# MiniMax-AI/VTP

Measured on AMD Instinct MI355X. Metric: images/sec/node VTP-B f16d64 256x256 train step, higher is better.
Workload: dtype bf16

## Files before the change

include/vtp_hip.h:

```cpp
#ifndef VTP_HIP_H
#define VTP_HIP_H
#ifdef __cplusplus
extern "C" {
#endif

#define VTP_ABI_VERSION 1

int vtp_abi_version(void);
const char* vtp_last_error(void);

enum { VTP_EPI_BF16 = 0, VTP_EPI_F32 = 1, VTP_EPI_SWIGLU = 2, VTP_EPI_GELU = 3, VTP_EPI_F32_ATOMIC = 4, VTP_EPI_F32_SLAB = 5,
       VTP_EPI_QUICK_GELU = 8 };
int vtp_gemm_splits(int K, int splits);
int vtp_gemm_tn_splits(int M, int N, int K);
int vtp_gemm_tn(const void* A, int lda, const void* B, int ldb, void* C, int ldc, int ldc2, const float* resid, int M, int N,
                int K, int epilogue, int a_grp, int a_pre, int b_grp, int b_pre, int c_grp, int c_pre, int splits,
                float* a_colsum, void* stream);
int vtp_gemm_tn_grouped(const void* probs, int nprob, int ntiles, int K, int splits, void* part, void* ticket, void* stream);
int vtp_gemm_tn_grouped_items(const void* probs, int nprob, int ntiles, int K, const void* items, int nitems, int slots, void* part,
                              void* ticket, void* stream);
int vtp_set_gemm_tuning(int force_cfg, int xcd_swizzle);
int vtp_set_gemm_dynamic(int on);
int vtp_gemm_debug(void* timing, int grid_limit, int delay_ticks);
int vtp_cu_thief(int nwg, int ticks, void* out, void* stream);
int vtp_attn_debug(void* timing, int lds_pad, int waves_per_wg, int stagger_ticks);
int vtp_gemm_nt_config(int M, int N, int K, int epilogue);
int vtp_gemm_nt(const void* A, int lda, const void* B, int ldb, void* C, int ldc, void* C2, int ldc2,
                const float* bias, const float* gamma, const float* resid, int M, int N, int K, int epilogue,
                int a_grp, int a_pre, int c_grp, int c_pre, int splits, float alpha, void* stream);

int vtp_gemm_qkv_rope(const void* A, int lda, const void* W, int ldb, const float* bias, void* C, int ldc, int M, int N, int K,
                      const int* rope_pos, const void* rope_sin, const void* rope_cos, int rope_cols, void* stream);

int vtp_gather_image_rows(const float* src, const int* img_idx, float* dst, void* dst_bf16, int n_img, long N, int D, float scale,
                          void* stream);
int vtp_scatter_image_rows(const float* src, const int* img_idx, float* dst, int n_img, long N, int D, float alpha, int accumulate,
                           void* stream);
int vtp_layerscale_wgrad(const float* G, const float* W, const float* bias, const float* colsum, const float* gamma, float* dW,
                         float* db, float* dgamma, int N, int K, void* stream);
int vtp_scaled_transpose(const float* W, const float* gamma, void* dstT, int N, int K, void* stream);
int vtp_qk_norm_fwd(const void* qkv, const float* wq, const float* wk, void* out, float* inv, long M, int D, float eps, void* stream);
int vtp_qk_norm_bwd(void* dqkv, const void* qkv, const float* inv, const float* wq, const float* wk, float* dwq, float* dwk, long M, int D,
                    void* stream);

int vtp_norm_fwd(const float* x, const float* w, const float* b, void* y, float* stats, int M, int D, float eps,
                 int kind, void* stream);
int vtp_norm_bwd(const void* dy, const float* x, const float* w, const float* stats, const float* dres, float* dx,
                 void* dx_bf16, float* dw, float* db, float* dx_colsum, int M, int D, int kind, void* stream);
int vtp_norm_bwd_pvec(const void* dy, const float* x, const float* w, const float* stats, const float* dres, float* dx,
                      void* dx_bf16, float* dw, float* db, float* dx_colsum, const float* pvec, int prow0, int pB, int pN, int M,
                      int D, int kind, void* stream);
int vtp_pool_patch_rows(const void* x, float* out, int B, int N, int D, float scale, void* stream);

int vtp_rope_qk(void* qkv, const void* sin, const void* cos, int B, int N, int heads, int prefix, int inverse,
                void* stream);

int vtp_attn_fwd(const void* q, const void* k, const void* v, void* o, float* lse, int B, int N, int heads,
                 long sb_qkv, long sn_qkv, long sb_o, long sn_o, float scale, int causal, void* stream);
int vtp_attn_bwd(const void* q, const void* k, const void* v, const void* o, const void* d_o, const float* lse,
                 float* delta, void* dq, void* dk, void* dv, const void* rope_sin, const void* rope_cos, int rope_prefix,
                 int B, int N, int heads, long sb_qkv, long sn_qkv, long sb_o, long sn_o, float scale, int causal,
                 void* stream);

int vtp_im2col16(const float* img, void* patches, int B, int H, int W, void* stream);
int vtp_im2col16_rows(const float* img, void* rows, int B, int H, int W, int prefix, void* stream);
int vtp_col2im16(const float* dpatches, float* dimg, int B, int H, int W, void* stream);

int vtp_assemble_tokens(float* x, const float* cls, const float* mask_token, const unsigned char* masks, int B, int N,
                        int D, void* stream);

int vtp_transpose_bf16(const void* in, int ld_in, void* out, int ld_out, float* colsum, int colsum_swiglu_h, int in_grp,
                       int in_pre, int R, int C, void* stream);
int vtp_colsum_bf16(const void* in, int ld, float* out, int colsum_swiglu_h, int in_grp, int in_pre, int R, int C, void* stream);
int vtp_colsum_bf16_rows(const void* in, int ld, float* out, const int* n_rows_dev, int R_max, int C, void* stream);
int vtp_mask_rows_bwd(const float* dx, void* dx_bf16, const unsigned char* masks, float* d_mask_token, int B, int N, int D,
                      void* stream);
int vtp_token_rows_bwd(const float* dx, void* dx_bf16, const unsigned char* masks, float* d_mask_token, float* d_cls_token, int B, int N,
                       int D, void* stream);
int vtp_strided_rowsum(const float* in, long stride, float* out, int B, int D, void* stream);

int vtp_cast_f32_bf16(const float* in, void* out, long n, void* stream);
int vtp_cast_transpose_f32_bf16(const float* in, void* out, int R, int C, void* stream);
int vtp_prep_weights(const void* descs, int n, int total_tiles, void* stream);
int vtp_prep_weights_range(const void* descs, int n, int tile_base, int n_tiles, void* stream);

int vtp_swiglu_bwd(const void* dh, const void* x12, void* dx12, float* db12, int M, int H, void* stream);
int vtp_gemm_dgrad_swiglu(const void* A, int lda, const void* WT, int ldb, const void* x12, int ldx, void* dx12, int ldc, int M, int H,
                          int K, void* stream);
int vtp_gelu_bwd(const void* dy, const void* pre, void* dx, long n, void* stream);
int vtp_quick_gelu_bwd(const void* dy, const void* pre, void* dx, long n, void* stream);

int vtp_pixel_shuffle16(const void* t, float* img, int B, int h, int w, void* stream);
int vtp_pixel_unshuffle16(const float* d_img, void* dt, int B, int h, int w, void* stream);
int vtp_l1_loss_fwd_bwd(const void* t, const float* target, void* dt, float* loss_sum, int B, int h, int w,
                        float gscale, void* stream);

int vtp_adamw(float* p, const float* g, float* m, float* v, void* p_bf16, long n, float lr, float beta1, float beta2,
              float eps, float weight_decay, int step, float grad_scale, void* stream);
int vtp_adamw_dev(float* p, const float* g, float* m, float* v, void* p_bf16, long n, const float* hyper, void* stream);
int vtp_adamw_dev_masked(float* p, const float* g, float* m, float* v, void* p_bf16, const void* nodecay4, long n, const float* hyper,
                         void* stream);
int vtp_reduce_slabs(const float* slabs, long stride, int S, float* dst, long n, int accumulate, void* stream);
int vtp_ema(float* t, const float* s, long n, float momentum, void* stream);
int vtp_ema_dev(float* t, const float* s, long n, const float* momentum , void* stream);
int vtp_adamw_ema_dev(float* p, const float* g, float* m, float* v, float* teacher, const void* nodecay4, long n, const float* hyper,
                      void* stream);
int vtp_adamw_dev_grouped(float* p, const float* g, float* m, float* v, void* p_bf16, const void* group4, const float* group_tab,
                          int ngroups, long n, const float* hyper, void* stream);
int vtp_adamw_ema_dev_grouped(float* p, const float* g, float* m, float* v, float* teacher, const void* group4, const float* group_tab,
                              int ngroups, long n, const float* hyper, void* stream);
int vtp_sumsq_partials_count(long n);
int vtp_sumsq_partials(const float* g, long n, double* partials, void* stream);
int vtp_sum_partials(const double* partials, int count, double* sum, void* stream);
int vtp_grad_clip_finalize(const double* partials, int count, float* hyper, float* total_norm, float* coef, void* stream);
int vtp_grad_clip_finalize_guarded(const double* partials, int count, float* hyper, float* total_norm, float* coef, int* state,
                                   const double* betas, void* stream);
int vtp_adamw_dev_guarded(float* p, const float* g, float* m, float* v, void* p_bf16, const void* idx4, const float* group_tab,
                          int ngroups, long n, const float* hyper, const int* skip, void* stream);
int vtp_adamw_ema_dev_guarded(float* p, const float* g, float* m, float* v, float* teacher, const void* idx4, const float* group_tab,
                              int ngroups, long n, const float* hyper, const int* skip, void* stream);
int vtp_ema_dev_guarded(float* t, const float* s, long n, const float* momentum, const int* skip, void* stream);

int vtp_embed_tokens(const long* ids, const float* table, const float* pos, float* x, int* eot, int B, int T, int D,
                     void* stream);
int vtp_embed_tokens_bwd(const long* ids, const float* dx, float* d_table, float* d_pos, int B, int T, int D, void* stream);
int vtp_gather_rows(const float* x, const int* idx, float* out, int B, int T, int D, void* stream);
int vtp_scatter_rows(const float* dy, const int* idx, float* dx, void* dx_bf16, int B, int T, int D, void* stream);
int vtp_l2norm_fwd(const float* x, float* y, float* inv_norm, int B, int D, float eps, void* stream);
int vtp_l2norm_bwd(const float* dy, const float* y, const float* inv_norm, float* dx, int B, int D, void* stream);
int vtp_clip_loss(const float* img_local, const float* txt_local, const float* img_all, const float* txt_all,
                  const float* logit_scale, int B_local, int B_all, int D, int label_offset, float* loss_sum,
                  float* d_img_local, float* d_txt_local, float* d_img_all, float* d_txt_all, float* d_logit_scale,
                  float* scratch, void* stream);

// ... 52 lines not shown
```

vtp_amd/_lib.py:

```python
import ctypes
import os
from ctypes import c_char_p, c_float, c_int, c_long, c_void_p

_HERE = os.path.dirname(os.path.abspath(__file__))
LIB_PATH = os.environ.get("VTP_HIP_LIB") or os.path.join(_HERE, "lib", "libvtp_hip.so")

_P, _I, _L, _F = c_void_p, c_int, c_long, c_float

SIGNATURES = {
    "vtp_gemm_nt": [_P, _I, _P, _I, _P, _I, _P, _I, _P, _P, _P, _I, _I, _I, _I, _I, _I, _I, _I, _I, _F, _P],
    "vtp_norm_fwd": [_P, _P, _P, _P, _P, _I, _I, _F, _I, _P],
    "vtp_norm_bwd": [_P, _P, _P, _P, _P, _P, _P, _P, _P, _P, _I, _I, _I, _P],
    "vtp_norm_bwd_pvec": [_P, _P, _P, _P, _P, _P, _P, _P, _P, _P, _P, _I, _I, _I, _I, _I, _I, _P],
    "vtp_pool_patch_rows": [_P, _P, _I, _I, _I, _F, _P],
    "vtp_rope_qk": [_P, _P, _P, _I, _I, _I, _I, _I, _P],
    "vtp_attn_fwd": [_P, _P, _P, _P, _P, _I, _I, _I, _L, _L, _L, _L, _F, _I, _P],
    "vtp_attn_bwd": [_P, _P, _P, _P, _P, _P, _P, _P, _P, _P, _P, _P, _I, _I, _I, _I, _L, _L, _L, _L, _F, _I, _P],
    "vtp_im2col16": [_P, _P, _I, _I, _I, _P],
    "vtp_im2col16_rows": [_P, _P, _I, _I, _I, _I, _P],
    "vtp_col2im16": [_P, _P, _I, _I, _I, _P],
    "vtp_assemble_tokens": [_P, _P, _P, _P, _I, _I, _I, _P],
    "vtp_transpose_bf16": [_P, _I, _P, _I, _P, _I, _I, _I, _I, _I, _P],
    "vtp_strided_rowsum": [_P, _L, _P, _I, _I, _P],
    "vtp_mask_rows_bwd": [_P, _P, _P, _P, _I, _I, _I, _P],
    "vtp_token_rows_bwd": [_P, _P, _P, _P, _P, _I, _I, _I, _P],
    "vtp_cast_f32_bf16": [_P, _P, _L, _P],
    "vtp_cast_transpose_f32_bf16": [_P, _P, _I, _I, _P],
    "vtp_prep_weights": [_P, _I, _I, _P],
    "vtp_prep_weights_range": [_P, _I, _I, _I, _P],
    "vtp_swiglu_bwd": [_P, _P, _P, _P, _I, _I, _P],
    "vtp_gemm_dgrad_swiglu": [_P, _I, _P, _I, _P, _I, _P, _I, _I, _I, _I, _P],
    "vtp_gelu_bwd": [_P, _P, _P, _L, _P],
    "vtp_quick_gelu_bwd": [_P, _P, _P, _L, _P],
    "vtp_pixel_shuffle16": [_P, _P, _I, _I, _I, _P],
    "vtp_pixel_unshuffle16": [_P, _P, _I, _I, _I, _P],
    "vtp_l1_loss_fwd_bwd": [_P, _P, _P, _P, _I, _I, _I, _F, _P],
    "vtp_adamw": [_P, _P, _P, _P, _P, _L, _F, _F, _F, _F, _F, _I, _F, _P],
    "vtp_adamw_dev": [_P, _P, _P, _P, _P, _L, _P, _P],
    "vtp_adamw_dev_masked": [_P, _P, _P, _P, _P, _P, _L, _P, _P],
    "vtp_reduce_slabs": [_P, _L, _I, _P, _L, _I, _P],
    "vtp_gemm_splits": [_I, _I],
    "vtp_gemm_tn_splits": [_I, _I, _I],
    "vtp_gemm_qkv_rope": [_P, _I, _P, _I, _P, _P, _I, _I, _I, _I, _P, _P, _P, _I, _P],
    "vtp_gemm_tn": [_P, _I, _P, _I, _P, _I, _I, _P, _I, _I, _I, _I, _I, _I, _I, _I, _I, _I, _I, _P, _P],
    "vtp_gemm_tn_grouped": [_P, _I, _I, _I, _I, _P, _P, _P],
    "vtp_gemm_tn_grouped_items": [_P, _I, _I, _I, _P, _I, _I, _P, _P, _P],
    "vtp_colsum_bf16": [_P, _I, _P, _I, _I, _I, _I, _I, _P],
    "vtp_colsum_bf16_rows": [_P, _I, _P, _P, _I, _I, _P],
    "vtp_gather_image_rows": [_P, _P, _P, _P, _I, _L, _I, _F, _P],
    "vtp_scatter_image_rows": [_P, _P, _P, _I, _L, _I, _F, _I, _P],
    "vtp_layerscale_wgrad": [_P, _P, _P, _P, _P, _P, _P, _P, _I, _I, _P],
    "vtp_scaled_transpose": [_P, _P, _P, _I, _I, _P],
    "vtp_qk_norm_fwd": [_P, _P, _P, _P, _P, _L, _I, _F, _P],
    "vtp_qk_norm_bwd": [_P, _P, _P, _P, _P, _P, _P, _L, _I, _P],
    "vtp_set_gemm_tuning": [_I, _I],
    "vtp_gemm_nt_config": [_I, _I, _I, _I],
    "vtp_gemm_debug": [_P, _I, _I],
    "vtp_attn_debug": [_P, _I, _I, _I],
    "vtp_cu_thief": [_I, _I, _P, _P],
    "vtp_set_gemm_dynamic": [_I],
    "vtp_norm_fwd_e4m3": [_P, _P, _P, _P, _P, _P, _I, _I, _F, _I, _P],
    "vtp_quantize_e4m3": [_P, _I, _P, _L, _P, _F, _P],
    "vtp_amax": [_P, _I, _L, _P, _P],
    "vtp_dequantize_e4m3": [_P, _P, _L, _F, _P],
    "vtp_gemm_nt_fp8": [_P, _I, _P, _I, _P, _I, _P, _I, _P, _P, _I, _I, _I, _I, _F, _P, _P, _P, _I, _P],
    "vtp_u8_to_images": [_P, _P, _L, _I, _I, _P, _P, _I, _P],
    "vtp_images_to_u8": [_P, _P, _L, _I, _I, _P, _P, _P],
    "vtp_latent_channel_stats": [_P, _P, _L, _I, _I, _P],
    "vtp_ema": [_P, _P, _L, _F, _P],
    "vtp_gather_token_rows": [_P, _P, _P, _I, _I, _P],
    "vtp_scatter_token_rows": [_P, _P, _P, _I, _I, _P],
    "vtp_weight_norm_prep": [_P, _P, _P, _P, _P, _I, _I, _P],
    "vtp_weight_norm_bwd": [_P, _P, _P, _P, _P, _P, _I, _I, _P],
    "vtp_softmax_center": [_P, _P, _F, _P, _I, _I, _P],
    "vtp_softmax_center_dev": [_P, _P, _P, _P, _I, _I, _P],
    "vtp_dino_ce": [_P, _P, _P, _P, _P, _F, _P, _P, _I, _I, _P],
    "vtp_center_ema": [_P, _P, _F, _P, _F, _I, _P],
    "vtp_conv3x3": [_P, _P, _P, _P, _P, _I, _I, _I, _I, _I, _I, _I, _P],
    "vtp_lpips_unfold3": [_P, _P, _P, _I, _I, _I, _P, _P, _P],
    "vtp_lpips_fold3_bwd": [_P, _P, _I, _I, _I, _P, _P],
    "vtp_maxpool2_fwd": [_P, _P, _I, _I, _I, _I, _P],
    "vtp_maxpool2_bwd": [_P, _P, _P, _P, _I, _I, _I, _I, _P],
    "vtp_lpips_tap": [_P, _P, _P, _P, _P, _I, _I, _I, _I, _F, _P],
    "vtp_ema_dev": [_P, _P, _L, _P, _P],
    "vtp_adamw_ema_dev": [_P, _P, _P, _P, _P, _P, _L, _P, _P],
    "vtp_adamw_dev_grouped": [_P, _P, _P, _P, _P, _P, _P, _I, _L, _P, _P],
    "vtp_adamw_ema_dev_grouped": [_P, _P, _P, _P, _P, _P, _P, _I, _L, _P, _P],
    "vtp_sumsq_partials_count": [_L],
    "vtp_sumsq_partials": [_P, _L, _P, _P],
    "vtp_sum_partials": [_P, _I, _P, _P],
    "vtp_grad_clip_finalize": [_P, _I, _P, _P, _P, _P],
    "vtp_grad_clip_finalize_guarded": [_P, _I, _P, _P, _P, _P, _P, _P],
    "vtp_adamw_dev_guarded": [_P, _P, _P, _P, _P, _P, _P, _I, _L, _P, _P, _P],
    "vtp_adamw_ema_dev_guarded": [_P, _P, _P, _P, _P, _P, _P, _I, _L, _P, _P, _P],
    "vtp_ema_dev_guarded": [_P, _P, _L, _P, _P, _P],
    "vtp_embed_tokens": [_P, _P, _P, _P, _P, _I, _I, _I, _P],
    "vtp_embed_tokens_bwd": [_P, _P, _P, _P, _I, _I, _I, _P],
    "vtp_gather_rows": [_P, _P, _P, _I, _I, _I, _P],
    "vtp_scatter_rows": [_P, _P, _P, _P, _I, _I, _I, _P],
    "vtp_l2norm_fwd": [_P, _P, _P, _I, _I, _F, _P],
    "vtp_l2norm_bwd": [_P, _P, _P, _P, _I, _I, _P],
    "vtp_clip_logits": [_P, _P, _P, _P, _I, _I, _I, _P],
    "vtp_clip_grad_rows": [_P, _P, _P, _P, _I, _I, _I, _I, _P],
    "vtp_clip_grad_cols": [_P, _P, _P, _P, _I, _I, _I, _I, _P],
    "vtp_siglip_pairs": [_P, _P, _I, _I, _I, _F, _P, _P, _P, _P],
    "vtp_koleo": [_P, _P, _P, _P, _I, _I, _F, _F, _P],
    "vtp_sinkhorn_knopp": [_P, _F, _P, _P, _P, _P, _I, _I, _F, _P, _P, _I, _I, _P],
    "vtp_clip_loss": [_P, _P, _P, _P, _P, _I, _I, _I, _I, _P, _P, _P, _P, _P, _P, _P, _P],
}

_lib = None


def load():
    global _lib
    if _lib is not None:
        return _lib
    if not os.path.exists(LIB_PATH):
        raise RuntimeError(
            f"vtp_amd: {LIB_PATH} not found. The HIP library is mandatory (there is no fallback path): "
            "run `python -c 'import __graft_entry__ as g; g.build()'` or `python vtp_amd/build.py`.")
    try:
        import torch
        if torch.cuda.is_available():
            torch.cuda.init()
    except ImportError:
        pass
    lib = ctypes.CDLL(LIB_PATH)
    lib.vtp_abi_version.restype = c_int
    lib.vtp_last_error.restype = c_char_p
    for name, args in SIGNATURES.items():
        fn = getattr(lib, name)
        fn.argtypes = args
# ... 12 lines not shown
```

vtp_amd/csrc/block_extras.hip:

```cpp
#include "common.h"
#include "vtp_hip.h"

namespace vtp {

__global__ __launch_bounds__(256) void gather_image_rows_kernel(const float* __restrict__ src, const int* __restrict__ idx,
                                                                float* __restrict__ dst, bf16* __restrict__ dst_b, int n_img,
                                                                long N, int D, float scale) {
  const int d4 = D / 4;
  const long total = (long)n_img * N * d4;
  for (long i = blockIdx.x * 256L + threadIdx.x; i < total; i += (long)gridDim.x * 256L) {
    const int c = (int)(i % d4);
    const long row = i / d4;
    const int img = (int)(row / N);
    const long t = row - (long)img * N;
    const f32x4 v = *(const f32x4*)(src + ((long)idx[img] * N + t) * D + 4 * c);
    if (dst) *(f32x4*)(dst + row * D + 4 * c) = v;
    if (dst_b) *(bf16x4*)(dst_b + row * D + 4 * c) = __builtin_convertvector(v * scale, bf16x4);
  }
}

__global__ __launch_bounds__(256) void scatter_image_rows_kernel(const float* __restrict__ src, const int* __restrict__ idx,
                                                                 float* __restrict__ dst, int n_img, long N, int D, float alpha,
                                                                 int accumulate) {
  const int d4 = D / 4;
// ... 48 lines not shown
    const int k = k0 + c, n = n0 + tx;
    if (k < K && n < N) dstT[(size_t)k * N + n] = f2bf(tile[tx][c]);
  }
}

__global__ __launch_bounds__(256) void qk_norm_fwd_kernel(const bf16* __restrict__ qkv, const float* __restrict__ wq,
                                                          const float* __restrict__ wk, bf16* __restrict__ out, float* __restrict__ inv,
                                                          long M, int D, float eps) {
  const int cpr = 3 * D / 8, cpp = D / 8;
  const long total = M * cpr;
  for (long i = blockIdx.x * 256L + threadIdx.x; i < (total + 255) / 256 * 256; i += (long)gridDim.x * 256L) {
    const bool live = i < total;
    const long row = live ? i / cpr : 0;
    const int c = live ? (int)(i - row * cpr) : 0, part = c / cpp, d0 = (c % 8) * 8;
    bf16x8 v = live ? *(const bf16x8*)(qkv + row * 3 * D + (long)c * 8) : bf16x8{};
    float ss = 0.f;
#pragma unroll
    for (int e = 0; e < 8; ++e) ss += bf2f(v[e]) * bf2f(v[e]);
    ss += __shfl_xor(ss, 1, 64);
    ss += __shfl_xor(ss, 2, 64);
    ss += __shfl_xor(ss, 4, 64);
    if (!live) continue;
    if (part < 2) {
      const float r = rsqrtf(ss * (1.f / 64.f) + eps);
      const float* w = part == 0 ? wq : wk;
#pragma unroll
      for (int e = 0; e < 8; ++e) v[e] = f2bf(bf2f(f2bf(bf2f(v[e]) * r)) * w[d0 + e]);
      if ((c & 7) == 0) inv[row * (2 * D / 64) + (c / 8)] = r;
    }
    *(bf16x8*)(out + row * 3 * D + (long)c * 8) = v;
  }
}

__global__ __launch_bounds__(256) void qk_norm_bwd_kernel(bf16* __restrict__ dqkv, const bf16* __restrict__ qkv, const float* __restrict__ inv,
                                                          const float* __restrict__ wq, const float* __restrict__ wk, float* __restrict__ dwq,
                                                          float* __restrict__ dwk, long M, int D) {
  __shared__ float red[2][64];
  const int cpr = 2 * D / 8, cpp = D / 8;
  const long total = M * cpr;
  if (threadIdx.x < 128) red[threadIdx.x >> 6][threadIdx.x & 63] = 0.f;
  __syncthreads();
  float dw[2][8] = {};
  for (long i = blockIdx.x * 256L + threadIdx.x; i < (total + 255) / 256 * 256; i += (long)gridDim.x * 256L) {
    const bool live = i < total;
    const long row = live ? i / cpr : 0;
    const int c = live ? (int)(i - row * cpr) : 0, part = c / cpp, d0 = (c % 8) * 8;
    const long off = row * 3 * D + (long)c * 8;
    const bf16x8 x = live ? *(const bf16x8*)(qkv + off) : bf16x8{};
    const bf16x8 dy = live ? *(const bf16x8*)(dqkv + off) : bf16x8{};
    const float r = live ? inv[row * (2 * D / 64) + (c / 8)] : 0.f;
    const float* w = part == 0 ? wq : wk;
    float xh[8], g[8], dot = 0.f;
#pragma unroll
    for (int e = 0; e < 8; ++e) {
      xh[e] = bf2f(x[e]) * r;
      g[e] = bf2f(dy[e]) * w[d0 + e];
      dot += g[e] * xh[e];
    }
    dot += __shfl_xor(dot, 1, 64);
    dot += __shfl_xor(dot, 2, 64);
    dot += __shfl_xor(dot, 4, 64);
    if (!live) continue;
    dot *= 1.f / 64.f;
    bf16x8 o;
#pragma unroll
    for (int e = 0; e < 8; ++e) {
      o[e] = f2bf(r * (g[e] - xh[e] * dot));
      dw[part][e] += bf2f(dy[e]) * bf2f(f2bf(xh[e]));
    }
    *(bf16x8*)(dqkv + off) = o;
  }
  const int d0 = (threadIdx.x % 8) * 8;
#pragma unroll
  for (int pt = 0; pt < 2; ++pt)
#pragma unroll
    for (int e = 0; e < 8; ++e) atomicAdd(&red[pt][d0 + e], dw[pt][e]);
  __syncthreads();
  if (threadIdx.x < 128) {
    const float v = red[threadIdx.x >> 6][threadIdx.x & 63];
    if (v != 0.f) atomicAdd((threadIdx.x >> 6 ? dwk : dwq) + (threadIdx.x & 63), v);
  }
}

}
using namespace vtp;

static inline int extras_grid(long items) {
  long b = (items + 255) / 256;
  return (int)(b > 4096 ? 4096 : (b < 1 ? 1 : b));
}

extern "C" int vtp_gather_image_rows(const float* src, const int* img_idx, float* dst, void* dst_bf16, int n_img, long N, int D,
                                     float scale, void* stream) {
  VTP_REQUIRE(src && img_idx && (dst || dst_bf16) && n_img > 0 && N > 0 && D > 0 && D % 4 == 0, "vtp_gather_image_rows: bad argument");
  hipLaunchKernelGGL(gather_image_rows_kernel, dim3(extras_grid((long)n_img * N * D / 4)), dim3(256), 0, (hipStream_t)stream, src,
                     img_idx, dst, (bf16*)dst_bf16, n_img, N, D, scale);
  return check_launch("gather_image_rows");
}

extern "C" int vtp_scatter_image_rows(const float* src, const int* img_idx, float* dst, int n_img, long N, int D, float alpha,
                                      int accumulate, void* stream) {
  VTP_REQUIRE(src && img_idx && dst && n_img > 0 && N > 0 && D > 0 && D % 4 == 0, "vtp_scatter_image_rows: bad argument");
  hipLaunchKernelGGL(scatter_image_rows_kernel, dim3(extras_grid((long)n_img * N * D / 4)), dim3(256), 0, (hipStream_t)stream, src,
                     img_idx, dst, n_img, N, D, alpha, accumulate);
  return check_launch("scatter_image_rows");
}

extern "C" int vtp_layerscale_wgrad(const float* G, const float* W, const float* bias, const float* colsum, const float* gamma,
                                    float* dW, float* db, float* dgamma, int N, int K, void* stream) {
  VTP_REQUIRE(G && W && colsum && gamma && dW && dgamma && N > 0 && K > 0 && K % 4 == 0, "vtp_layerscale_wgrad: bad argument");
  hipLaunchKernelGGL(layerscale_wgrad_kernel, dim3(cdiv(N, 4)), dim3(256), 0, (hipStream_t)stream, G, W, bias, colsum, gamma, dW, db,
                     dgamma, N, K);
  return check_launch("layerscale_wgrad");
}

extern "C" int vtp_scaled_transpose(const float* W, const float* gamma, void* dstT, int N, int K, void* stream) {
  VTP_REQUIRE(W && gamma && dstT && N > 0 && K > 0, "vtp_scaled_transpose: bad argument");
  hipLaunchKernelGGL(scaled_transpose_kernel, dim3(cdiv(K, 64), cdiv(N, 64)), dim3(256), 0, (hipStream_t)stream, W, gamma,
                     (bf16*)dstT, N, K);
  return check_launch("scaled_transpose");
}

extern "C" int vtp_qk_norm_fwd(const void* qkv, const float* wq, const float* wk, void* out, float* inv, long M, int D, float eps,
                               void* stream) {
  VTP_REQUIRE(qkv && wq && wk && out && inv && M > 0 && D > 0 && D % 64 == 0, "vtp_qk_norm_fwd: bad argument (head_dim 64: D %% 64 == 0)");
  hipLaunchKernelGGL(qk_norm_fwd_kernel, dim3(extras_grid(M * (3 * D / 8))), dim3(256), 0, (hipStream_t)stream, (const bf16*)qkv, wq, wk,
                     (bf16*)out, inv, M, D, eps);
  return check_launch("qk_norm_fwd");
}

extern "C" int vtp_qk_norm_bwd(void* dqkv, const void* qkv, const float* inv, const float* wq, const float* wk, float* dwq, float* dwk,
                               long M, int D, void* stream) {
  VTP_REQUIRE(dqkv && qkv && inv && wq && wk && dwq && dwk && M > 0 && D > 0 && D % 64 == 0, "vtp_qk_norm_bwd: bad argument");
  long blocks = (M * (2 * D / 8) + 255) / 256;
  hipLaunchKernelGGL(qk_norm_bwd_kernel, dim3((int)(blocks > 1024 ? 1024 : blocks)), dim3(256), 0, (hipStream_t)stream, (bf16*)dqkv,
                     (const bf16*)qkv, inv, wq, wk, dwq, dwk, M, D);
  return check_launch("qk_norm_bwd");
}
```

vtp_amd/csrc/gemm4w_tn.hip:

```cpp
#include "gemm_common.h"
#include "gemm_group.h"
#include "gemm4w_tn_ktile.inc"

namespace vtp {

namespace {
constexpr int W4T_KT = 65536;
constexpr int W4T_RING = 2 * W4T_KT;
constexpr int W4T_LDS = W4T_RING + 32768;
}

__device__ __forceinline__ void w4t_glds16(const char* sbase, unsigned voff, unsigned lds_dst) {
  unsigned keep;
  asm volatile("s_mov_b32 %0, m0\n\ts_mov_b32 m0, %3\n\ts_nop 0\n\tglobal_load_lds_dwordx4 %1, %2\n\ts_mov_b32 m0, %0"
               : "=&s"(keep)
               : "v"(voff), "s"(sbase), "s"(lds_dst)
               : "memory");
}

__device__ __forceinline__ int w4t_uni(long v) { return __builtin_amdgcn_readfirstlane((int)v); }
template <class T>
__device__ __forceinline__ T* w4t_uni(T* v) {
  const unsigned long long u = (unsigned long long)v;
  const unsigned lo = __builtin_amdgcn_readfirstlane((unsigned)u), hi = __builtin_amdgcn_readfirstlane((unsigned)(u >> 32));
  return (T*)(((unsigned long long)hi << 32) | lo);
}

struct W4TStage {
  const char *mata, *matb, *zb;
  unsigned stepa, stepb, da[2], db[2];
};

__device__ __forceinline__ void w4t_kloop(bool csum, f32x16 (&acc)[4][4], float (&cs)[4], const unsigned (&aE)[2], const unsigned (&aO)[2],
                                          const unsigned (&bE)[2], const unsigned (&bO)[2], unsigned& pea, unsigned& peb, unsigned zoff,
                                          const W4TStage& st, int& kra, int& krb, unsigned nk2) {
  unsigned vt, sm, cnt = nk2;
  unsigned long long sb;
  const unsigned ones = 0x3F803F80u;
  const unsigned docs = __builtin_amdgcn_readfirstlane(csum ? 1u : 0u);
  asm volatile(W4T_TILE_ASM_BOTH
               : W4T_TILE_ACC, [cs0] "+v"(cs[0]), [cs1] "+v"(cs[1]), [cs2] "+v"(cs[2]), [cs3] "+v"(cs[3]), [pea] "+v"(pea), [peb] "+v"(peb),
                 [vt] "=&v"(vt), [kra] "+s"(kra), [krb] "+s"(krb), [cnt] "+s"(cnt), [sm] "=&s"(sm), [sb] "=&s"(sb)
               : [aE0] "v"(aE[0]), [aO0] "v"(aO[0]), [bE0] "v"(bE[0]), [bO0] "v"(bO[0]), [aE1] "v"(aE[1]), [aO1] "v"(aO[1]), [bE1] "v"(bE[1]),
                 [bO1] "v"(bO[1]), [zoff] "v"(zoff), [mata] "s"(st.mata), [matb] "s"(st.matb), [zb] "s"(st.zb), [stepa] "s"(st.stepa),
                 [stepb] "s"(st.stepb), [ones] "s"(ones), [docs] "s"(docs), [da0] "s"(st.da[0]), [da1] "s"(st.da[1]), [db0] "s"(st.db[0]),
                 [db1] "s"(st.db[1])
               : "memory", "scc", "vcc", W4T_TILE_CLOBBERS);
}

__device__ __forceinline__ void w4t_segment(const GroupArgs& ga, int tile, int kbeg, int kcount, int nparts, int part) {
  extern __shared__ __attribute__((aligned(16))) char smem[];
  const int tid = threadIdx.x;
  auto stamp = [&](int which) {
    if (__builtin_expect(ga.timing != nullptr, 0) && tid == 0) ga.timing[(size_t)blockIdx.x * 8 + which] = wall_clock64();
  };
  if (__builtin_expect(ga.timing != nullptr, 0) && tid == 0) {
    ga.timing[(size_t)blockIdx.x * 8 + 5] = (unsigned long long)tile;
    ga.timing[(size_t)blockIdx.x * 8 + 6] = (unsigned long long)part;
    unsigned xcc;
    asm volatile("s_getreg_b32 %0, hwreg(HW_REG_XCC_ID)" : "=s"(xcc));
    ga.timing[(size_t)blockIdx.x * 8 + 7] = (unsigned long long)(xcc & 15);
  }
  stamp(0);
  const int lane = tid & 63;
  const int wave = __builtin_amdgcn_readfirstlane(tid >> 6);
  const int wr = wave >> 1, wc = wave & 1;
  const int hi = lane >> 5;

  int g = 0;
  for (int i = 1; i < ga.nprob; ++i)
    if ((int)ga.probs[i].tile0 <= tile) g = i;
  const GroupProblem& pr = ga.probs[g];
  GemmArgs p{};
  p.A = w4t_uni(pr.A); p.B = w4t_uni(pr.B); p.C = w4t_uni(pr.C); p.resid = w4t_uni(pr.accumulate) ? (const float*)p.C : nullptr;
  p.colsum = w4t_uni(pr.colsum);
  p.M = w4t_uni(pr.M); p.N = w4t_uni(pr.N); p.K = ga.K; p.lda = w4t_uni(pr.lda); p.ldb = w4t_uni(pr.ldb); p.ldc = w4t_uni(pr.ldc);
  p.c_grp = w4t_uni(pr.c_grp); p.c_pre = w4t_uni(pr.c_pre); p.k_split = ga.k_split; p.alpha = 1.f;
  p.xcd_swizzle = 2;
  const int lt = tile - w4t_uni(pr.tile0), tiles_n = (p.N + 255) >> 8;
  const int n0 = (lt % tiles_n) << 8, m0 = (lt / tiles_n) << 8;
  const unsigned nk2 = (unsigned)((kcount + 127) >> 7);

  const int krow = lane >> 3, chunk = (lane & 7) ^ (4 * ((krow >> 1) & 1));
  const int cola = min(m0 + wave * 64 + chunk * 8, p.M - 8), colb = min(n0 + wave * 64 + chunk * 8, p.N - 8);
  unsigned pea = (unsigned)(((size_t)(kbeg + krow) * p.lda + cola) * 2), peb = (unsigned)(((size_t)(kbeg + krow) * p.ldb + colb) * 2);
  const unsigned zoff = (lane & 3) * 16;
  W4TStage st;
  st.mata = (const char*)p.A;
  st.matb = (const char*)p.B;
  st.zb = (const char*)g_zero_block;
  st.stepa = (unsigned)(8 * p.lda * 2);
  st.stepb = (unsigned)(8 * p.ldb * 2);
#pragma unroll
  for (int sl = 0; sl < 2; ++sl) {
    st.da[sl] = (unsigned)(size_t)smem + sl * W4T_KT + wave * 8192;
    st.db[sl] = st.da[sl] + 32768;
  }
#pragma unroll
  for (int kt = 0; kt < 2; ++kt)
#pragma unroll
    for (int i = 0; i < 8; ++i) {
      const bool valid = kt * 64 + 8 * i < kcount;
      w4t_glds16(valid ? st.mata : st.zb, valid ? pea : zoff, st.da[kt] + i * 1024);
      w4t_glds16(valid ? st.matb : st.zb, valid ? peb : zoff, st.db[kt] + i * 1024);
      pea += st.stepa;
      peb += st.stepb;
    }
  int kra = kcount - 128, krb = kcount - 128;

  unsigned aE[2], aO[2], bE[2], bO[2];
  {
    const int t_li = lane & 15, t_rq = t_li >> 2;
    const int cq = ((lane >> 4) & 1) * 2 + ((t_li & 3) >> 1), sz = 4 * ((t_rq >> 1) & 1);
    const unsigned rowb = (unsigned)((hi * 8 + t_rq) * 128 + (t_li & 1) * 8);
    const unsigned lb0 = rowb + (unsigned)(((0 + cq) ^ sz) << 4), lb1 = rowb + (unsigned)(((4 + cq) ^ sz) << 4);
#pragma unroll
    for (int sl = 0; sl < 2; ++sl) {
      const unsigned ba = (unsigned)(size_t)smem + sl * W4T_KT + (wr * 2) * 8192, bb = (unsigned)(size_t)smem + sl * W4T_KT + (4 + wc * 2) * 8192;
      aE[sl] = ba + lb0;
      aO[sl] = ba + lb1;
      bE[sl] = bb + lb0;
      bO[sl] = bb + lb1;
    }
  }
  f32x16 acc[4][4];
#pragma unroll
  for (int i = 0; i < 4; ++i)
#pragma unroll
    for (int j = 0; j < 4; ++j)
#pragma unroll
      for (int e = 0; e < 16; ++e) acc[i][j][e] = 0.f;
  float cs[4] = {0.f, 0.f, 0.f, 0.f};
  const bool do_csum = p.colsum != nullptr && n0 == 0;

  asm volatile("s_waitcnt vmcnt(0)" ::: "memory");
  __builtin_amdgcn_s_barrier();
  __builtin_amdgcn_sched_barrier(0);
  stamp(1);
  w4t_kloop(do_csum, acc, cs, aE, aO, bE, bO, pea, peb, zoff, st, kra, krb, nk2);
  asm volatile("s_nop 15\n\ts_nop 15\n\ts_nop 7\n\ts_waitcnt vmcnt(0)" ::: "memory");
  stamp(2);

  if (do_csum && wc == 0) {
#pragma unroll
    for (int j = 0; j < 4; ++j) {
      const float v = cs[j] + __shfl_xor(cs[j], 32, 64);
      const int m = m0 + wr * 128 + j * 32 + (lane & 31);
      if (hi == 0 && m < p.M) unsafeAtomicAdd(p.colsum + remap_row(m, p.c_grp, p.c_pre), v);
    }
  }
  if (nparts > 1) {
    typedef __attribute__((ext_vector_type(4))) unsigned int u32x4_t;
    const f32x4* mine = (const f32x4*)ga.part + (((size_t)tile * ga.splits + part) * 4 + wave) * 4096;
    const auto rsrc = __builtin_amdgcn_make_buffer_rsrc((void*)mine, 0, 4096 * 16, 0x00020000);
#pragma unroll
    for (int u = 0; u < 64; ++u) {
      f32x4 v;
#pragma unroll
      for (int e = 0; e < 4; ++e) v[e] = acc[u >> 4][(u >> 2) & 3][4 * (u & 3) + e];
      __builtin_amdgcn_raw_buffer_store_b128((u32x4_t)v, rsrc, lane * 16 + u * 1024, 0,  16);
    }
    asm volatile("s_waitcnt vmcnt(0)" ::: "memory");
    __syncthreads();
    int* flag = (int*)(smem + W4T_LDS - 16);
// ... 56 lines not shown
```

vtp_amd/csrc/gemm_group.h:

```cpp
#pragma once
#include "gemm_common.h"

namespace vtp {

struct GroupProblem {
  const bf16* A;
  const bf16* B;
  float* C;
  float* colsum;
  long lda, ldb, ldc;
  long M, N;
  long c_grp, c_pre;
  long tile0;
  long accumulate;
  long pad[3];
};
struct GroupItem {
  int tile;
  int kbeg, kcount;
  int nparts, part;
  int pad[3];
};
struct GroupArgs {
  const GroupProblem* probs;
  float* part;
  int* ticket;
  int nprob, ntiles, splits, K, k_split;
  unsigned long long* timing;
  const GroupItem* items;
};

}
```

vtp_amd/csrc/norm.hip:

```cpp
#include "common.h"
#include <cstdlib>
#include "vtp_hip.h"

namespace vtp {

constexpr int NORM_MAXC = 8;

template <int KIND, int NC>
__global__ __launch_bounds__(256) void norm_fwd_kernel(const float* __restrict__ x, const float* __restrict__ w,
                                                       const float* __restrict__ b, bf16* __restrict__ y,
                                                       float* __restrict__ stats, int M, int D, float eps,
                                                       uint8_t* __restrict__ y8 = nullptr, const float* __restrict__ q_scale = nullptr) {
  const int lane = threadIdx.x & 63;
  const int row = blockIdx.x * 4 + (threadIdx.x >> 6);
  if (row >= M) return;
  const float* xr = x + (size_t)row * D;
  f32x4 v[NC];
  float s = 0.f;
#pragma unroll
  for (int c = 0; c < NC; ++c) {
    const int col = (c * 64 + lane) * 4;
    if (col < D) {
      v[c] = *(const f32x4*)(xr + col);
      s += (KIND == 0) ? (v[c][0] * v[c][0] + v[c][1] * v[c][1] + v[c][2] * v[c][2] + v[c][3] * v[c][3])
                       : (v[c][0] + v[c][1] + v[c][2] + v[c][3]);
    }
  }
  s = wave_sum(s);
  float mean = 0.f, rstd;
  if (KIND == 0) {
    rstd = rsqrtf(s / D + eps);
  } else {
    mean = s / D;
    float q = 0.f;
#pragma unroll
    for (int c = 0; c < NC; ++c) {
      const int col = (c * 64 + lane) * 4;
      if (col < D) {
#pragma unroll
        for (int e = 0; e < 4; ++e) {
          const float d = v[c][e] - mean;
          q += d * d;
        }
      }
    }
    q = wave_sum(q);
    rstd = rsqrtf(q / D + eps);
  }
  bf16* yr = y + (size_t)row * D;
#pragma unroll
  for (int c = 0; c < NC; ++c) {
    const int col = (c * 64 + lane) * 4;
    if (col < D) {
      f32x4 wv = *(const f32x4*)(w + col);
      f32x4 o;
      if (KIND == 0) {
#pragma unroll
        for (int e = 0; e < 4; ++e) o[e] = v[c][e] * rstd * wv[e];
      } else {
        f32x4 bv = *(const f32x4*)(b + col);
#pragma unroll
        for (int e = 0; e < 4; ++e) o[e] = (v[c][e] - mean) * rstd * wv[e] + bv[e];
      }
      const bf16x4 ob = __builtin_convertvector(o, bf16x4);
      if (y8) {
        const float qs = *q_scale;
        float q[4];
#pragma unroll
        for (int e = 0; e < 4; ++e) q[e] = fminf(fmaxf(bf2f(ob[e]) * qs, -448.f), 448.f);
        uint32_t wq = __builtin_amdgcn_cvt_pk_fp8_f32(q[0], q[1], 0u, false);
        wq = __builtin_amdgcn_cvt_pk_fp8_f32(q[2], q[3], wq, true);
        *(uint32_t*)(y8 + (size_t)row * D + col) = wq;
      } else {
        *(bf16x4*)(yr + col) = ob;
      }
    }
  }
  if (lane == 0 && stats) {
    stats[2 * row] = mean;
    stats[2 * row + 1] = rstd;
  }
}

template <int KIND, int NC, bool PV = false>
__global__ __launch_bounds__(256, 2) void norm_bwd_kernel(const bf16* __restrict__ dy, const float* __restrict__ x,
                                                       const float* __restrict__ w, const float* __restrict__ stats,
                                                       const float* __restrict__ dres, float* __restrict__ dx,
                                                       bf16* __restrict__ dxb, float* __restrict__ dw, float* __restrict__ db,
                                                       float* __restrict__ dxsum, int M, int D,
                                                       const float* __restrict__ pvec = nullptr, int prow0 = 0, int pB = 0,
                                                       int pN = 1) {
  constexpr int R = NC <= 3 ? 2 : 1;
  const int lane = threadIdx.x & 63;
  const int wv_id = threadIdx.x >> 6;
  f32x4 wreg[NC], dwacc[NC], dbacc[NC], dsacc[KIND == 1 ? NC : 1];
#pragma unroll
  for (int c = 0; c < NC; ++c) {
    const int col = (c * 64 + lane) * 4;
    if (col < D) wreg[c] = *(const f32x4*)(w + col);
    dwacc[c] = (f32x4){0.f, 0.f, 0.f, 0.f};
    dbacc[c] = (f32x4){0.f, 0.f, 0.f, 0.f};
    if (KIND == 1) dsacc[c] = (f32x4){0.f, 0.f, 0.f, 0.f};
  }
  for (int row0 = (blockIdx.x * 4 + wv_id) * R; row0 < M; row0 += gridDim.x * 4 * R) {
    constexpr bool PRE = NC <= 3;
    f32x4 xv[R][NC], dr[PRE ? R : 1][PRE ? NC : 1];
    bf16x4 gy[R][NC];
    float mean[R], rstd[R];
#pragma unroll
    for (int r = 0; r < R; ++r) {
      const int row = min(row0 + r, M - 1);
      mean[r] = stats[2 * row];
      rstd[r] = stats[2 * row + 1];
#pragma unroll
      for (int c = 0; c < NC; ++c) {
        const int col = (c * 64 + lane) * 4;
        if (col < D) {
          xv[r][c] = *(const f32x4*)(x + (size_t)row * D + col);
          gy[r][c] = *(const bf16x4*)(dy + (size_t)row * D + col);
          if constexpr (PRE) {
            if (dres) dr[r][c] = *(const f32x4*)(dres + (size_t)row * D + col);
          }
        }
      }
    }
#pragma unroll
    for (int r = 0; r < R; ++r) {
      const int row = row0 + r;
      if (row >= M) break;
      f32x4 xh[NC], g[NC];
      float s1 = 0.f, s2 = 0.f;
      const float* pv = nullptr;
      if constexpr (PV) {
        const int loc = row - prow0;
        if (loc >= 0 && loc < pB * pN && loc % pN != 0) pv = pvec + (size_t)(loc / pN) * D;
      }
#pragma unroll
      for (int c = 0; c < NC; ++c) {
        const int col = (c * 64 + lane) * 4;
        if (col < D) {
          f32x4 gyf = __builtin_convertvector(gy[r][c], f32x4);
          if constexpr (PV) {
            if (pv) gyf += *(const f32x4*)(pv + col);
          }
#pragma unroll
          for (int e = 0; e < 4; ++e) {
            xh[c][e] = (xv[r][c][e] - mean[r]) * rstd[r];
            g[c][e] = gyf[e] * wreg[c][e];
            s1 += g[c][e];
            s2 += g[c][e] * xh[c][e];
            dwacc[c][e] += gyf[e] * xh[c][e];
            if (KIND == 1) dbacc[c][e] += gyf[e];
          }
        }
      }
      s2 = wave_sum(s2) / D;
      if (KIND == 1) s1 = wave_sum(s1) / D; else s1 = 0.f;
#pragma unroll
      for (int c = 0; c < NC; ++c) {
        const int col = (c * 64 + lane) * 4;
        if (col < D) {
          f32x4 o;
#pragma unroll
          for (int e = 0; e < 4; ++e) o[e] = rstd[r] * (g[c][e] - s1 - xh[c][e] * s2);
          if (dres) {
            if constexpr (PRE) o += dr[r][c];
            else o += *(const f32x4*)(dres + (size_t)row * D + col);
          }
          *(f32x4*)(dx + (size_t)row * D + col) = o;
          if (dxb) {
            const bf16x4 ob = __builtin_convertvector(o, bf16x4);
            *(bf16x4*)(dxb + (size_t)row * D + col) = ob;
            if (dxsum) {
              const f32x4 of = __builtin_convertvector(ob, f32x4);
              if (KIND == 1) dsacc[c] += of; else dbacc[c] += of;
            }
          }
        }
      }
    }
  }
  __shared__ float red[4][NC * 256];
  for (int pass = 0; pass < 3; ++pass) {
    if (pass == 0 && dw == nullptr) continue;
    if (pass == 1 && (KIND == 0 || db == nullptr)) continue;
    if (pass == 2 && (dxsum == nullptr || dxb == nullptr)) continue;
    __syncthreads();
#pragma unroll
    for (int c = 0; c < NC; ++c)
#pragma unroll
      for (int e = 0; e < 4; ++e)
        red[wv_id][(c * 64 + lane) * 4 + e] =
            pass == 0 ? dwacc[c][e] : (pass == 1 ? dbacc[c][e] : (KIND == 1 ? dsacc[KIND == 1 ? c : 0][e] : dbacc[c][e]));
    __syncthreads();
    float* out = pass == 0 ? dw : (pass == 1 ? db : dxsum);
    for (int col = threadIdx.x; col < D; col += 256)
      unsafeAtomicAdd(out + col, red[0][col] + red[1][col] + red[2][col] + red[3][col]);
  }
}

constexpr int POOL_WAVES = 8;

__global__ __launch_bounds__(POOL_WAVES * 64) void pool_patch_rows_kernel(const bf16* __restrict__ x, float* __restrict__ out, int N,
                                                                         int D, float scale) {
  const int lane = threadIdx.x & 63;
  const int wv = threadIdx.x >> 6;
  const int col = (blockIdx.x * 64 + lane) * 4;
  const int b = blockIdx.y;
  f32x4 acc = (f32x4){0.f, 0.f, 0.f, 0.f};
  if (col < D) {
    const bf16* xb = x + (size_t)b * N * D + col;
    int t = 1 + wv;
    for (; t + 3 * POOL_WAVES < N; t += 4 * POOL_WAVES) {
      bf16x4 v[4];
#pragma unroll
      for (int u = 0; u < 4; ++u) v[u] = *(const bf16x4*)(xb + (size_t)(t + u * POOL_WAVES) * D);
#pragma unroll
      for (int u = 0; u < 4; ++u) acc += __builtin_convertvector(v[u], f32x4);
    }
    for (; t < N; t += POOL_WAVES) acc += __builtin_convertvector(*(const bf16x4*)(xb + (size_t)t * D), f32x4);
  }
  __shared__ f32x4 red[POOL_WAVES][64];
  red[wv][lane] = acc;
  __syncthreads();
  if (wv == 0 && col < D) {
    f32x4 s = red[0][lane];
#pragma unroll
    for (int k = 1; k < POOL_WAVES; ++k) s += red[k][lane];
    *(f32x4*)(out + (size_t)b * D + col) = s * scale;
  }
}

}
using namespace vtp;

#define NORM_DISPATCH(KERNEL, KIND, ...)                                                            \
  do {                                                                                              \
    const int nc = cdiv(D, 256);                                                                    \
    if (nc <= 1) hipLaunchKernelGGL((KERNEL<KIND, 1>), grid, block, 0, (hipStream_t)stream, __VA_ARGS__);      \
    else if (nc == 2) hipLaunchKernelGGL((KERNEL<KIND, 2>), grid, block, 0, (hipStream_t)stream, __VA_ARGS__); \
    else if (nc == 3) hipLaunchKernelGGL((KERNEL<KIND, 3>), grid, block, 0, (hipStream_t)stream, __VA_ARGS__); \
    else if (nc == 4) hipLaunchKernelGGL((KERNEL<KIND, 4>), grid, block, 0, (hipStream_t)stream, __VA_ARGS__); \
    else hipLaunchKernelGGL((KERNEL<KIND, 8>), grid, block, 0, (hipStream_t)stream, __VA_ARGS__);              \
  } while (0)

extern "C" int vtp_norm_fwd(const float* x, const float* w, const float* b, void* y, float* stats, int M, int D,
                            float eps, int kind, void* stream) {
  VTP_REQUIRE(x && w && y, "vtp_norm_fwd: null pointer");
  VTP_REQUIRE(M > 0 && D > 0 && D % 4 == 0 && D <= NORM_MAXC * 256, "vtp_norm_fwd: need 0 < D <= 2048, D %% 4 == 0 (D=%d)", D);
  VTP_REQUIRE(kind == 0 || (kind == 1 && b), "vtp_norm_fwd: kind must be 0 (rms) or 1 (layernorm, needs bias)");
  dim3 grid(cdiv(M, 4)), block(256);
  if (kind == 0)
    NORM_DISPATCH(norm_fwd_kernel, 0, x, w, b, (bf16*)y, stats, M, D, eps);
  else
    NORM_DISPATCH(norm_fwd_kernel, 1, x, w, b, (bf16*)y, stats, M, D, eps);
  return check_launch("norm_fwd");
}

extern "C" int vtp_norm_fwd_e4m3(const float* x, const float* w, const float* b, void* y8, const float* q_scale, float* stats, int M,
                                 int D, float eps, int kind, void* stream) {
  VTP_REQUIRE(x && w && y8 && q_scale, "vtp_norm_fwd_e4m3: null pointer");
  VTP_REQUIRE(M > 0 && D > 0 && D % 4 == 0 && D <= NORM_MAXC * 256, "vtp_norm_fwd_e4m3: need 0 < D <= 2048, D %% 4 == 0 (D=%d)", D);
  VTP_REQUIRE(kind == 0 || (kind == 1 && b), "vtp_norm_fwd_e4m3: kind must be 0 (rms) or 1 (layernorm, needs bias)");
  dim3 grid(cdiv(M, 4)), block(256);
  if (kind == 0)
    NORM_DISPATCH(norm_fwd_kernel, 0, x, w, b, (bf16*)nullptr, stats, M, D, eps, (uint8_t*)y8, q_scale);
  else
    NORM_DISPATCH(norm_fwd_kernel, 1, x, w, b, (bf16*)nullptr, stats, M, D, eps, (uint8_t*)y8, q_scale);
  return check_launch("norm_fwd_e4m3");
}

static int norm_bwd_blocks(int M, int D) {
  int blocks = cdiv(M, D <= 768 ? 8 : 4);
  static int cap_env = -1;
  if (cap_env < 0) {
    const char* e = getenv("VTP_NORM_BWD_BLOCKS");
    cap_env = e && atoi(e) > 0 ? atoi(e) : 0;
  }
  const int cap = cap_env ? cap_env : (M >= 24576 ? 512 : (M >= 4096 ? 256 : 128));
  return blocks > cap ? cap : blocks;
}

extern "C" int vtp_norm_bwd(const void* dy, const float* x, const float* w, const float* stats, const float* dres,
                            float* dx, void* dx_bf16, float* dw, float* db, float* dx_colsum, int M, int D, int kind,
                            void* stream) {
  VTP_REQUIRE(dy && x && w && stats && dx, "vtp_norm_bwd: null pointer");
  VTP_REQUIRE(!dx_colsum || dx_bf16, "vtp_norm_bwd: dx_colsum sums the bf16 output and needs dx_bf16");
  VTP_REQUIRE(M > 0 && D > 0 && D % 4 == 0 && D <= NORM_MAXC * 256, "vtp_norm_bwd: need 0 < D <= 2048, D %% 4 == 0 (D=%d)", D);
  VTP_REQUIRE(kind == 0 || kind == 1, "vtp_norm_bwd: kind must be 0 or 1");
  dim3 grid(norm_bwd_blocks(M, D)), block(256);
  if (kind == 0)
    NORM_DISPATCH(norm_bwd_kernel, 0, (const bf16*)dy, x, w, stats, dres, dx, (bf16*)dx_bf16, dw, db, dx_colsum, M, D);
  else
    NORM_DISPATCH(norm_bwd_kernel, 1, (const bf16*)dy, x, w, stats, dres, dx, (bf16*)dx_bf16, dw, db, dx_colsum, M, D);
  return check_launch("norm_bwd");
}

template <int KIND>
static void launch_norm_bwd_pvec(dim3 grid, hipStream_t s, const bf16* dy, const float* x, const float* w, const float* stats,
                                 const float* dres, float* dx, bf16* dxb, float* dw, float* db, float* dxsum, int M, int D,
                                 const float* pvec, int prow0, int pB, int pN) {
  const int nc = cdiv(D, 256);
#define NORM_PV(NC) \
  hipLaunchKernelGGL((norm_bwd_kernel<KIND, NC, true>), grid, dim3(256), 0, s, dy, x, w, stats, dres, dx, dxb, dw, db, dxsum, M, D, \
                     pvec, prow0, pB, pN)
  if (nc <= 1) NORM_PV(1);
  else if (nc == 2) NORM_PV(2);
  else if (nc == 3) NORM_PV(3);
  else NORM_PV(4);
#undef NORM_PV
}

extern "C" int vtp_norm_bwd_pvec(const void* dy, const float* x, const float* w, const float* stats, const float* dres, float* dx,
                                 void* dx_bf16, float* dw, float* db, float* dx_colsum, const float* pvec, int prow0, int pB, int pN,
                                 int M, int D, int kind, void* stream) {
  VTP_REQUIRE(dy && x && w && stats && dx && pvec, "vtp_norm_bwd_pvec: null pointer");
  VTP_REQUIRE(!dx_colsum || dx_bf16, "vtp_norm_bwd_pvec: dx_colsum sums the bf16 output and needs dx_bf16");
  VTP_REQUIRE(M > 0 && D > 0 && D % 4 == 0 && D <= 1024, "vtp_norm_bwd_pvec: need 0 < D <= 1024, D %% 4 == 0 (D=%d)", D);
  VTP_REQUIRE(kind == 0 || kind == 1, "vtp_norm_bwd_pvec: kind must be 0 or 1");
  VTP_REQUIRE(pB > 0 && pN >= 2 && prow0 >= 0 && (long)prow0 + (long)pB * pN <= M,
              "vtp_norm_bwd_pvec: segment rows [%d, %d + %d*%d) must lie in [0, M=%d), N >= 2", prow0, prow0, pB, pN, M);
  dim3 grid(norm_bwd_blocks(M, D));
  if (kind == 0)
    launch_norm_bwd_pvec<0>(grid, (hipStream_t)stream, (const bf16*)dy, x, w, stats, dres, dx, (bf16*)dx_bf16, dw, db, dx_colsum, M, D,
                            pvec, prow0, pB, pN);
  else
    launch_norm_bwd_pvec<1>(grid, (hipStream_t)stream, (const bf16*)dy, x, w, stats, dres, dx, (bf16*)dx_bf16, dw, db, dx_colsum, M, D,
                            pvec, prow0, pB, pN);
  return check_launch("norm_bwd_pvec");
}

extern "C" int vtp_pool_patch_rows(const void* x, float* out, int B, int N, int D, float scale, void* stream) {
  VTP_REQUIRE(x && out, "vtp_pool_patch_rows: null pointer");
  VTP_REQUIRE(B > 0 && N >= 2 && D > 0 && D % 4 == 0, "vtp_pool_patch_rows: need B > 0, N >= 2, D %% 4 == 0 (B=%d N=%d D=%d)", B, N, D);
  VTP_REQUIRE((long)B * N * D < (1L << 40), "vtp_pool_patch_rows: matrix too large");
  hipLaunchKernelGGL(pool_patch_rows_kernel, dim3(cdiv(D, 256), B), dim3(POOL_WAVES * 64), 0, (hipStream_t)stream, (const bf16*)x, out,
                     N, D, scale);
  return check_launch("pool_patch_rows");
}
```

vtp_amd/engine.py:

```python
from __future__ import annotations

import math
import os
from typing import Dict, List, NamedTuple, Optional, Tuple

import torch

from . import ops
from .ops import EPI_BF16, EPI_F32, EPI_F32_SLAB, EPI_GELU, EPI_SWIGLU


class Lin:
    __slots__ = ("N", "K", "w", "wT", "bias", "gw", "gb", "w32", "wTs")


class SwiGLULin:
    __slots__ = ("H", "K", "w12", "w12T", "b12", "gw1", "gb1")


def _flat_order(names: List[str]) -> List[str]:
    out, seen = [], set()
    for n in names:
        if n in seen:
            continue
# ... 222 lines not shown

        @contextlib.contextmanager
        def ctx():
            prev, self._lane = self._lane, k
            try:
                yield
            finally:
                self._lane = prev
        return ctx()


OVERLAP = Overlap()


def linear_bwd(ws: Workspace, tag: str, L, dy_b, x_b, M: int, d_in, *, need_dx: bool = True, dy_remap=(0, 0),
               x_remap=(0, 0), dx_remap=(0, 0), gw=None, gb=None, N=None, K=None, wT=None, swiglu_h: int = 0,
               bias_grad_done: bool = False, ls=None, dgrad_swiglu=None, defer=None):
    if L is not None:
        N = L.N if N is None else N
        K = L.K if K is None else K
        gw = L.gw if gw is None else gw
        gb = L.gb if gb is None else gb
        wT = L.wT if wT is None else wT
    if ls is not None:
        gamma, g_gamma = ls
        assert L is not None and not swiglu_h and dy_remap == (0, 0) and x_remap == (0, 0)
        cs = ws.get("T.ls_cs", (N,), F32)
        cs.zero_()
        G = ws.get("T.ls_G", (N * K,), F32)

        def wgrad_ls():
            kw = dict(M=N, N=K, K=M, lda=dy_b.stride(0), ldb=x_b.stride(0), ldc=K, a_colsum=cs)
            St = ops.gemm_tn_splits(N, K, M)
            if St == 1:
                ops.gemm_tn(dy_b, x_b, G, epi=EPI_F32, **kw)
            else:
                slab = ws.get("T.slab", (St * N * K,), F32)
                ops.gemm_tn(dy_b, x_b, slab, ldc2=N * K // 4, epi=EPI_F32_SLAB, splits=St, **kw)
                ops.reduce_slabs(slab, N * K, St, G, N * K, accumulate=False)
            ops.layerscale_wgrad(G, L.w32, L.bias, cs, gamma, gw, gb, g_gamma, N, K)

        OVERLAP.join()
        wgrad_ls()
        if need_dx:
            ops.gemm_nt(dy_b, L.wTs, d_in, M=M, N=K, K=N, lda=dy_b.stride(0), ldb=N, ldc=d_in.stride(0), epi=EPI_BF16,
                        c_remap=dx_remap)
        return
    if bias_grad_done:
        gb = None
    c_remap = (-1, swiglu_h) if swiglu_h else (0, 0)

    def wgrad():
        if gb is not None:
            ops.colsum_bf16(dy_b, dy_b.stride(0), gb, M, N, swiglu_h=swiglu_h, in_remap=dy_remap)
        kw = dict(M=N, N=K, K=M, lda=dy_b.stride(0), ldb=x_b.stride(0), ldc=K, a_remap=dy_remap, b_remap=x_remap, c_remap=c_remap)
        St = ops.gemm_tn_splits(N, K, M)
        if St == 1:
            ops.gemm_tn(dy_b, x_b, gw, resid=gw, epi=EPI_F32, **kw)
        else:
            n_el = N * K
            slab = ws.get("T.slab", (St * n_el,), F32)
            ops.gemm_tn(dy_b, x_b, slab, ldc2=n_el // 4, epi=EPI_F32_SLAB, splits=St, **kw)
            ops.reduce_slabs(slab, n_el, St, gw, n_el, accumulate=True)

    if defer is not None:
        assert dy_remap == (0, 0) and x_remap == (0, 0)
        defer.append(dict(dy=dy_b, x=x_b, gw=gw, gb=gb, N=N, K=K, swiglu_h=swiglu_h))
    elif OVERLAP.enabled and need_dx:
        OVERLAP.join()
        OVERLAP.fork()
        with torch.cuda.stream(OVERLAP.side):
            wgrad()
    else:
        OVERLAP.join()
        wgrad()
    if need_dx and dgrad_swiglu is not None:
        assert dy_remap == (0, 0) and dx_remap == (0, 0)
        ops.gemm_dgrad_swiglu(dy_b, wT, dgrad_swiglu, d_in, M, K, N)
    elif need_dx:
        ops.gemm_nt(dy_b, wT, d_in, M=M, N=K, K=N, lda=dy_b.stride(0), ldb=N, ldc=d_in.stride(0), epi=EPI_BF16,
                    a_remap=dy_remap, c_remap=dx_remap)


class BlockW:
    pass


class BlockSaved(NamedTuple):
    attn_in: torch.Tensor
    xn1: torch.Tensor
    st1: torch.Tensor
    qkv: torch.Tensor
    o: torch.Tensor
    lse: torch.Tensor
    ffn_in: torch.Tensor
    xn2: torch.Tensor
    st2: torch.Tensor
    pre: torch.Tensor
    hid: torch.Tensor


ATTN_SCALE = 1.0 / math.sqrt(64.0)


_NAMES = {
    "vit": dict(n1="norm1", n2="norm2", qkv_w="attn.qkv.weight", qkv_b="attn.qkv.bias", proj_w="attn.proj.weight",
                proj_b="attn.proj.bias", ls1="ls1.gamma", ls2="ls2.gamma"),
    "text": dict(n1="ln_1", n2="ln_2", qkv_w="attn.in_proj_weight", qkv_b="attn.in_proj_bias",
                 proj_w="attn.out_proj.weight", proj_b="attn.out_proj.bias", ls1="ls_1.gamma", ls2="ls_2.gamma"),
}


class Stack:

    def __init__(self, store: ParamStore, prefix: str, depth: int, D: int, heads: int, H: int, norm: str,
                 style: str = "vit", ffn: str = "swiglu"):
        self.store, self.depth, self.D, self.heads, self.H, self.style = store, depth, D, heads, H, style
        self.swiglu = style == "vit" and ffn != "mlp"
        self.quick_gelu = False
        self.kind = ops.NORM_RMS if norm == "rmsnorm" else ops.NORM_LN
        if style == "text":
            self.eps = 1e-5
        else:
            self.eps = 1e-5 if norm == "rmsnorm" else 1e-6
        self.causal = style == "text"
        nm = _NAMES[style]
        self.blocks: List[BlockW] = []
        for i in range(depth):
            b = BlockW()
            pre = f"{prefix}{i}."
            b.n1w, b.gn1w = store.p(pre + nm["n1"] + ".weight"), store.g(pre + nm["n1"] + ".weight")
            b.n2w, b.gn2w = store.p(pre + nm["n2"] + ".weight"), store.g(pre + nm["n2"] + ".weight")
            if self.kind == ops.NORM_LN:
                b.n1b, b.gn1b = store.p(pre + nm["n1"] + ".bias"), store.g(pre + nm["n1"] + ".bias")
                b.n2b, b.gn2b = store.p(pre + nm["n2"] + ".bias"), store.g(pre + nm["n2"] + ".bias")
            else:
                b.n1b = b.gn1b = b.n2b = b.gn2b = None
            b.qkv = store.lin(pre + nm["qkv_w"], pre + nm["qkv_b"], 3 * D, D)
            b.proj = store.lin(pre + nm["proj_w"], pre + nm["proj_b"], D, D)
            if self.swiglu:
                b.w12 = store.swiglu(pre + "mlp.", H, D)
                b.w3 = store.lin(pre + "mlp.w3.weight", pre + "mlp.w3.bias", D, H)
            else:
                n1, n2 = ("fc1", "fc2") if style == "vit" else ("c_fc", "c_proj")
                b.fc = store.lin(f"{pre}mlp.{n1}.weight", f"{pre}mlp.{n1}.bias", H, D)
                b.w3 = store.lin(f"{pre}mlp.{n2}.weight", f"{pre}mlp.{n2}.bias", D, H)
            b.ls1 = store.p(pre + nm["ls1"]) if store.has(pre + nm["ls1"]) else None
            b.ls2 = store.p(pre + nm["ls2"]) if store.has(pre + nm["ls2"]) else None
            b.gls1 = store.g(pre + nm["ls1"]) if b.ls1 is not None else None
            b.gls2 = store.g(pre + nm["ls2"]) if b.ls2 is not None else None
            qn = pre + "attn.q_norm.weight"
            if store.has(qn):
                b.qn_w, b.kn_w = store.p(qn), store.p(pre + "attn.k_norm.weight")
                b.g_qn, b.g_kn = store.g(qn), store.g(pre + "attn.k_norm.weight")
            else:
                b.qn_w = b.kn_w = b.g_qn = b.g_kn = None
            for L, gam in ((b.proj, b.ls1), (b.w3, b.ls2)):
                if gam is not None:
                    L.wTs = torch.empty(L.K, L.N, dtype=BF, device=store.device)
                    if not hasattr(store, "prep_hooks"):
                        store.prep_hooks = []
                    store.prep_hooks.append(lambda L=L, gam=gam: ops.scaled_transpose(L.w32, gam, L.wTs, L.N, L.K))
            self.blocks.append(b)
        self.qk_norm = any(b.qn_w is not None for b in self.blocks)
        self.drop_plan = None
        self.wgrad_overwrite = False

    def _rope_plan(self, ws: Workspace, segs, prefix_tokens: int, M: int):
        if self.style != "vit" or all(rp is None for _, _, rp in segs) or (2 * self.D) % 128 or self.qk_norm:
            return None
        hit = getattr(ws, "_rope_plan", None)
        aug = [rp for _, _, rp in segs if isinstance(rp, RopeAugTabs)]
        key = tuple((b, n, None if rp is None else (rp.sin_all.data_ptr(), rp.off) if isinstance(rp, RopeAugTabs) else rp[0].data_ptr())
                    for b, n, rp in segs) + (prefix_tokens,)
        if hit is not None and hit[0] == key:
            return hit[1]
        pos, tabs_s, tabs_c, base = [], [], [], 0
        for Bs, Ns, rp in segs:
            if rp is None:
                pos.append(torch.full((Bs * Ns,), -1, dtype=torch.int32))
                continue
            hw = _rope_hw(rp)
# ... 53 lines not shown

    def set_drop_plan(self, plan, ws_key="drop"):
        if plan is not None and self.style != "vit":
            raise NotImplementedError("stochastic depth is a property of the ViT blocks (block.py:207-289); the text tower has none")
        if plan is None:
            if self.drop_plan is not None:
                self.last_drop_plan = self.drop_plan
            self.drop_plan = None
            return
        bufs = self.__dict__.setdefault("_drop_bufs", {})
        n = plan["idx"].numel()
        buf = bufs.get(n)
        if buf is None:
            buf = bufs[n] = torch.empty(n, dtype=torch.int32, device=self.store.device)
        buf.copy_(plan["idx"], non_blocking=True)
        cur = dict(plan)
        cur["idx_dev"] = buf
        self.drop_plan = cur

    @staticmethod
    def _check_drop_plan(p, segs):
        got = [B for B, _, _ in segs]
        if p.get("batches") != got:
            raise RuntimeError(f"stochastic-depth plan drawn for item batch sizes {p.get('batches')} used on a pass with {got}")

    def _drop_idx(self, i: int, branch: int, s: int):
        p = self.drop_plan
        o = (i * 2 + branch) * p["per"] + sum(p["keeps"][:s])
        return p["idx_dev"][o:o + p["keeps"][s]]

    def _drop_segs(self, segs):
        self._check_drop_plan(self.drop_plan, segs)
        csegs = [(k, N, rp) for (_, N, rp), k in zip(segs, self.drop_plan["keeps"])]
        return csegs, sum(k * N for k, N, _ in csegs)

    def _gather(self, x, segs, csegs, i, branch, dst, dst_b, scale_by_seg):
        D = self.D
        r_full, r_c = 0, 0
        for s, ((B, N, _), (k, _, _)) in enumerate(zip(segs, csegs)):
            sc = scale_by_seg[s] if isinstance(scale_by_seg, (list, tuple)) else scale_by_seg
            ops.gather_image_rows(x[r_full:], self._drop_idx(i, branch, s), None if dst is None else dst[r_c:],
                                  None if dst_b is None else dst_b[r_c:], k, N, D, sc)
            r_full += B * N
            r_c += k * N

    def _scatter(self, src, x, segs, csegs, i, branch, alpha_by_seg, accumulate):
        D = self.D
        r_full, r_c = 0, 0
        for s, ((B, N, _), (k, _, _)) in enumerate(zip(segs, csegs)):
            al = alpha_by_seg[s] if isinstance(alpha_by_seg, (list, tuple)) else alpha_by_seg
            ops.scatter_image_rows(src[r_c:], self._drop_idx(i, branch, s), x[r_full:], k, N, D, al, accumulate)
            r_full += B * N
            r_c += k * N

    @staticmethod
    def _rows(segs):
        r0 = 0
        for B, N, rope in segs:
            yield r0, B, N, rope
            r0 += B * N

    @staticmethod
    def _attn_rows(segs):
        out = []
        for r0, B, N, rope in Stack._rows(segs):
            same = out and (out[-1][3] is rope or (isinstance(out[-1][3], tuple) and isinstance(rope, tuple)
                                                   and out[-1][3][0] is rope[0] and out[-1][3][1] is rope[1]))
            if out and out[-1][2] == N and same:
                out[-1] = (out[-1][0], out[-1][1] + B, N, rope)
            else:
                out.append((r0, B, N, rope))
        return out

    def _attention(self, qkv, o, lse, rows, i: int, prefix_tokens: int, rope_qk: bool):
        D, heads = self.D, self.heads
        for r0, Bs, Ns, rp in rows:
            q_s, o_s = qkv[r0:r0 + Bs * Ns], o[r0:r0 + Bs * Ns]
            if rp is not None and rope_qk:
                rs, rc = rope_at(rp, i)
                ops.rope_qk(q_s, rs, rc, Bs, Ns, heads, prefix_tokens)
            ops.attn_fwd(q_s, q_s[:, D:], q_s[:, 2 * D:], o_s, lse[r0 * heads:], Bs, Ns, heads, Ns * 3 * D, 3 * D, Ns * D, D,
                         ATTN_SCALE, self.causal)

    def _attn_fwd(self, ws: Workspace, t: str, i: int, x, out, resid, M: int, rows, prefix_tokens: int, rope_plan):
        D, heads, b = self.D, self.heads, self.blocks[i]
        xn1, st1 = ws.get(t + "xn1", (M, D), BF), ws.get(t + "st1", (M, 2), F32)
        qkv, o = ws.get(t + "qkv", (M, 3 * D), BF), ws.get(t + "o", (M, D), BF)
        lse = ws.get(t + "lse", (M * heads,), F32)
        ops.norm_fwd(x, b.n1w, b.n1b, xn1, st1, M, D, self.eps, self.kind)
        if rope_plan is not None:
            ps, pc = self._plan_tabs(rope_plan, i)
            ops.gemm_qkv_rope(xn1, b.qkv.w, b.qkv.bias, qkv, M, 3 * D, D, rope_plan[0], ps, pc, 2 * D)
        elif b.qn_w is not None:
            qkv_pre = ws.get(t + "qkv_pre", (M, 3 * D), BF)
            qinv = ws.get(t + "qinv", (M, 2 * heads), F32)
            ops.gemm_nt(xn1, b.qkv.w, qkv_pre, M=M, N=3 * D, K=D, bias=b.qkv.bias, epi=EPI_BF16)
            ops.qk_norm_fwd(qkv_pre, b.qn_w, b.kn_w, qkv, qinv, M, D)
        else:
            ops.gemm_nt(xn1, b.qkv.w, qkv, M=M, N=3 * D, K=D, bias=b.qkv.bias, epi=EPI_BF16)
        self._attention(qkv, o, lse, rows, i, prefix_tokens, rope_plan is None)
        ops.gemm_nt(o, b.proj.w, out, M=M, N=D, K=D, bias=b.proj.bias, gamma=b.ls1, resid=resid, epi=EPI_F32)
        return xn1, st1, qkv, o, lse

    def _ffn_fwd(self, ws: Workspace, t: str, i: int, x, out, resid, M: int, train: bool):
        D, H, b = self.D, self.H, self.blocks[i]
        xn2, st2 = ws.get(t + "xn2", (M, D), BF), ws.get(t + "st2", (M, 2), F32)
        pre = ws.get(t + "x12", (M, 2 * H if self.swiglu else H), BF) if train else None
        hid = ws.get(t + "hid", (M, H), BF)
        ops.norm_fwd(x, b.n2w, b.n2b, xn2, st2, M, D, self.eps, self.kind)
        if self.swiglu:
            ops.gemm_nt(xn2, b.w12.w12, hid, M=M, N=2 * H, K=D, c2=pre, ldc2=2 * H, bias=b.w12.b12, epi=EPI_SWIGLU)
        else:
            ops.gemm_nt(xn2, b.fc.w, hid, M=M, N=H, K=D, c2=pre, ldc2=H, bias=b.fc.bias,
                        epi=ops.EPI_QUICK_GELU if self.quick_gelu else EPI_GELU)
        ops.gemm_nt(hid, b.w3.w, out, M=M, N=D, K=H, bias=b.w3.bias, gamma=b.ls2, resid=resid, epi=EPI_F32)
        return xn2, st2, pre, hid

    def _ffn_bwd(self, ws: Workspace, i: int, s: BlockSaved, dy, dy_b, dx, dx_b, M: int, bt: str, dpre, *, fused: bool,
                 bias_done: bool = False, probs=None, dx_colsum=None):
        D, H, b = self.D, self.H, self.blocks[i]
        dh, dxn = ws.get(bt + "dh", (M, H), BF), ws.get(bt + "dxn", (M, D), BF)
        linear_bwd(ws, "w3", b.w3, dy_b, s.hid, M, dpre if fused else dh, bias_grad_done=bias_done,
                   ls=(b.ls2, b.gls2) if b.ls2 is not None else None, dgrad_swiglu=s.pre if fused else None, defer=probs)
        OVERLAP.run_deferred()
        if self.swiglu:
            if not fused:
                ops.swiglu_bwd(dh, s.pre, dpre, M, H)
            linear_bwd(ws, "w12", None, dpre, s.xn2, M, dxn, N=2 * H, K=D, gw=b.w12.gw1, gb=b.w12.gb1, wT=b.w12.w12T, swiglu_h=H,
                       defer=probs)
        else:
            ops.gelu_bwd(dh, s.pre, dpre, M * H, quick=self.quick_gelu)
            linear_bwd(ws, "fc", b.fc, dpre, s.xn2, M, dxn, defer=probs)
        ops.norm_bwd(dxn, s.ffn_in, b.n2w, s.st2, dy, dx, dx_b, b.gn2w, b.gn2b, M, D, self.kind, dx_colsum=dx_colsum)

    def _attn_bwd(self, ws: Workspace, t: str, i: int, s: BlockSaved, dy, dy_b, dx, dx_b, M: int, bt: str, dqkv, rows,
                  prefix_tokens: int, *, bias_done: bool = False, probs=None, join: bool = False, dx_colsum=None):
        D, heads, b = self.D, self.heads, self.blocks[i]
        d_o, dxn = ws.get(bt + "do", (M, D), BF), ws.get(bt + "dxn", (M, D), BF)
        delta = ws.get(bt + "delta", (M * heads,), F32)
        linear_bwd(ws, "proj", b.proj, dy_b, s.o, M, d_o, bias_grad_done=bias_done, ls=(b.ls1, b.gls1) if b.ls1 is not None else None,
                   defer=probs)
        for r0, Bs, Ns, rp in rows:
            r1 = r0 + Bs * Ns
            q_s, dq_s = s.qkv[r0:r1], dqkv[r0:r1]
            ops.attn_bwd(q_s, q_s[:, D:], q_s[:, 2 * D:], s.o[r0:r1], d_o[r0:r1], s.lse[r0 * heads:], delta[r0 * heads:], dq_s,
                         dq_s[:, D:], dq_s[:, 2 * D:], Bs, Ns, heads, Ns * 3 * D, 3 * D, Ns * D, D, ATTN_SCALE, self.causal,
                         rope=None if rp is None else rope_at(rp, i), rope_prefix=prefix_tokens)
        if b.qn_w is not None:
            ops.qk_norm_bwd(dqkv, ws.get(t + "qkv_pre", (M, 3 * D), BF), ws.get(t + "qinv", (M, 2 * heads), F32), b.qn_w, b.kn_w,
                            b.g_qn, b.g_kn, M, D)
        linear_bwd(ws, "qkv", b.qkv, dqkv, s.xn1, M, dxn, defer=probs)
        if join:
            OVERLAP.join()
        ops.norm_bwd(dxn, s.attn_in, b.n1w, s.st1, dy, dx, dx_b, b.gn1w, b.gn1b, M, D, self.kind, dx_colsum=dx_colsum)

    def forward(self, ws: Workspace, x, segs, prefix_tokens: int, train: bool):
        D = self.D
        M = sum(b * n for b, n, _ in segs)
        fp8 = getattr(self, "fp8", None)
        if fp8 is not None and fp8["ready"] and not train:
            return self._forward_fp8(ws, x, segs, prefix_tokens, M)
        calib = fp8["amax"] if (fp8 is not None and not fp8["ready"] and not train) else None
        drop = train and self.drop_plan is not None
        if drop:
            csegs, Mb = self._drop_segs(segs)
            rows, scales = list(self._rows(csegs)), self.drop_plan["scales"]
        else:
            csegs, Mb, rows = segs, M, self._attn_rows(segs)
        rope_plan = self._rope_plan(ws, csegs, prefix_tokens, Mb)
        saved_all = []
        for i in range(self.depth):
            if drop:
                t = f"{i}.d."
                x1, x2 = ws.get(t + "xs1", (Mb, D), F32), ws.get(t + "xs2", (Mb, D), F32)
                delta = ws.get("d.delta", (Mb, D), F32)
                self._gather(x, segs, csegs, i, 0, x1, None, 1.0)
                a = self._attn_fwd(ws, t, i, x1, delta, None, Mb, rows, prefix_tokens, rope_plan)
                self._scatter(delta, x, segs, csegs, i, 0, scales, accumulate=True)
                self._gather(x, segs, csegs, i, 1, x2, None, 1.0)
                f = self._ffn_fwd(ws, t, i, x2, delta, None, Mb, True)
                self._scatter(delta, x, segs, csegs, i, 1, scales, accumulate=True)
            else:
                t = f"{i}." if train else ""
                x1, x2 = x, ws.get(t + "xmid", (M, D), F32)
                xout = ws.get((f"{i}.xout" if train else f"xout{i & 1}"), (M, D), F32)
                a = self._attn_fwd(ws, t, i, x1, x2, x1, M, rows, prefix_tokens, rope_plan)
                f = self._ffn_fwd(ws, t, i, x2, xout, x2, M, train)
                if calib is not None:
                    for j, tns in enumerate((a[0], a[3], f[0], f[3])):
                        ops.amax(tns, calib[i, j:j + 1])
                x = xout
            if train:
                saved_all.append(BlockSaved(x1, *a, x2, *f))
        self.last_saved = saved_all
        return x

    def fp8_begin_calibration(self):
        if not self.swiglu or self.D % 16 or self.H % 16 or any(b.ls1 is not None or b.ls2 is not None for b in self.blocks):
            raise NotImplementedError("fp8 forward: SwiGLU ViT blocks with D, H multiples of 16, no LayerScale")
        dev = self.store.device
        self.fp8 = {"ready": False, "amax": torch.zeros(self.depth, 4, dtype=F32, device=dev)}

    def fp8_finalize(self):
        f, dev = self.fp8, self.store.device
        amax = f["amax"].clamp_min(1e-12)
        f["act_scale"] = (ops.E4M3_MAX / amax).contiguous()
        act_inv = (amax / ops.E4M3_MAX).cpu().tolist()
        f["w"], f["alpha"] = [], []
        for i, b in enumerate(self.blocks):
            ws8, al = [], []
            for j, w in enumerate((b.qkv.w, b.proj.w, b.w12.w12, b.w3.w)):
                wa = float(w.float().abs().max().clamp_min(1e-12))
                q = torch.empty(w.shape, dtype=torch.uint8, device=dev)
                ops.quantize_e4m3(w.contiguous(), q, ops.E4M3_MAX / wa)
                ws8.append(q)
                al.append(act_inv[i][j] * wa / ops.E4M3_MAX)
            f["w"].append(ws8)
            f["alpha"].append(al)
        f["ready"] = True

    def _forward_fp8(self, ws: Workspace, x, segs, prefix_tokens: int, M: int):
        D, H, heads, f = self.D, self.H, self.heads, self.fp8
        a8 = ws.get("f8.a", (M, max(D, H)), torch.uint8)
        qkv = ws.get("qkv", (M, 3 * D), BF)
        o = ws.get("o", (M, D), BF)
        lse = ws.get("lse", (M * heads,), F32)
        xmid = ws.get("xmid", (M, D), F32)
        hid = ws.get("hid", (M, H), BF)
        rope_plan = self._rope_plan(ws, segs, prefix_tokens, M)
        rope_arg = None if rope_plan is None else (rope_plan[0], rope_plan[1], rope_plan[2], 2 * D)
        rows = self._attn_rows(segs)
        for i, b in enumerate(self.blocks):
            w8, al, sc = f["w"][i], f["alpha"][i], f["act_scale"][i]
            xout = ws.get(f"xout{i & 1}", (M, D), F32)
            ops.norm_fwd_e4m3(x, b.n1w, b.n1b, a8, sc[0:1], None, M, D, self.eps, self.kind)
            if b.qn_w is not None:
                qkv_pre = ws.get("f8.qkv_pre", (M, 3 * D), BF)
                ops.gemm_nt_fp8(a8, w8[0], qkv_pre, M=M, N=3 * D, K=D, alpha=al[0], bias=b.qkv.bias, epi=EPI_BF16)
                ops.qk_norm_fwd(qkv_pre, b.qn_w, b.kn_w, qkv, ws.get("f8.qinv", (M, 2 * heads), F32), M, D)
            else:
                ops.gemm_nt_fp8(a8, w8[0], qkv, M=M, N=3 * D, K=D, alpha=al[0], bias=b.qkv.bias, epi=EPI_BF16, rope=rope_arg)
            self._attention(qkv, o, lse, rows, i, prefix_tokens, rope_arg is None)
            ops.quantize_e4m3(o, a8, sc[1:2])
            ops.gemm_nt_fp8(a8, w8[1], xmid, M=M, N=D, K=D, alpha=al[1], bias=b.proj.bias, resid=x, epi=EPI_F32)
            ops.norm_fwd_e4m3(xmid, b.n2w, b.n2b, a8, sc[2:3], None, M, D, self.eps, self.kind)
            ops.gemm_nt_fp8(a8, w8[2], hid, M=M, N=2 * H, K=D, alpha=al[2], bias=b.w12.b12, epi=EPI_SWIGLU)
            ops.quantize_e4m3(hid, a8, sc[3:4])
            ops.gemm_nt_fp8(a8, w8[3], xout, M=M, N=D, K=H, alpha=al[3], bias=b.w3.bias, resid=xmid, epi=EPI_F32)
            x = xout
        return x

    def w3_colsum_target(self, i: int):
        b = self.blocks[i]
        return b.w3.gb if (b.ls2 is None and self.drop_plan is None) else None

    def backward(self, ws: Workspace, dy, dy_b, segs, prefix_tokens: int, saved=None, dy_colsum_done: bool = False,
                 hold_last: bool = False, extra_last=None):
        D, H = self.D, self.H
        M = sum(b * n for b, n, _ in segs)
        saved = self.last_saved if saved is None else saved
        drop = self.drop_plan is not None
        if drop:
            csegs, Mb = self._drop_segs(segs)
            rows, scales, bt = list(self._rows(csegs)), self.drop_plan["scales"], "b.d."
            gdy, gdy_b = ws.get(bt + "gdy", (Mb, D), F32), ws.get(bt + "gdy_b", (Mb, D), BF)
            dxc = ws.get(bt + "dxc", (Mb, D), F32)
        else:
            Mb, rows, bt = M, self._attn_rows(segs), "b."
            dmid = ws.get("b.dmid", (M, D), F32)
        grouped = not drop and M >= 256 and all(b.ls1 is None and b.ls2 is None for b in self.blocks) \
            and ops.wgrad_group_fits(M, max(3 * D, 2 * H if self.swiglu else H)) and D % 8 == 0 and H % 8 == 0
        par = (lambda i: f".{i & 1}") if grouped else (lambda i: "")
        groups = ws.__dict__.setdefault("_wgrad_groups", {})
        scratch = self.__dict__.setdefault("_wgrad_scratch", {})
        pending = None

        def launch_pending():
            if pending is None:
                return
            if OVERLAP.enabled:
                OVERLAP.fork()
                side, grp = OVERLAP.side, pending[1]

                def issue():
                    with torch.cuda.stream(side):
                        grp.launch()
                OVERLAP.defer(issue)
            else:
                pending[1].launch()

        for i in range(self.depth - 1, -1, -1):
            b, s = self.blocks[i], saved[i]
            t = f"{i}.d." if drop else f"{i}."
            dpre = ws.get(bt + "dx12" + par(i), (Mb, 2 * H if self.swiglu else H), BF)
            dqkv = ws.get(bt + "dqkv" + par(i), (Mb, 3 * D), BF)
            if drop:
                self._gather(dy, segs, csegs, i, 1, gdy, gdy_b, scales)
                self._ffn_bwd(ws, i, s, gdy, gdy_b, dxc, None, Mb, bt, dpre, fused=False)
                self._scatter(dxc, dy, segs, csegs, i, 1, 1.0, accumulate=False)
                self._gather(dy, segs, csegs, i, 0, gdy, gdy_b, scales)
                self._attn_bwd(ws, t, i, s, gdy, gdy_b, dxc, None, Mb, bt, dqkv, rows, prefix_tokens)
                self._scatter(dxc, dy, segs, csegs, i, 0, 1.0, accumulate=False)
                OVERLAP.join()
                yield ("block", i)
                continue
            dxo = ws.get(f"b.dx{i & 1}", (M, D), F32)
            dxo_b = ws.get(f"b.dx_b{i & 1}", (M, D), BF)
            dmid_b = ws.get("b.dmid_b" + par(i), (M, D), BF)
            probs = [] if grouped else None
            if grouped:
                launch_pending()
            self._ffn_bwd(ws, i, s, dy, dy_b, dmid, dmid_b, M, bt, dpre, fused=self.swiglu and b.ls2 is None,
                          bias_done=dy_colsum_done if i == self.depth - 1 else self.w3_colsum_target(i) is not None, probs=probs,
                          dx_colsum=b.proj.gb if b.ls1 is None else None)
            self._attn_bwd(ws, t, i, s, dmid, dmid_b, dxo, dxo_b, M, bt, dqkv, rows, prefix_tokens, bias_done=b.proj.gb is not None,
                           probs=probs, join=grouped, dx_colsum=self.w3_colsum_target(i - 1) if i > 0 else None)
            dy, dy_b = dxo, dxo_b
            if not grouped:
                OVERLAP.join()
                yield ("block", i)
                continue
            extra = [dict(pr, dy=dy_b) for pr in extra_last] if (i == 0 and hold_last and extra_last) else []
            gkey = (i, bool(self.wgrad_overwrite), len(extra))
            grp = groups.get(gkey)
            if grp is None:
                grp = ops.WgradGroup(M)
                for pr in probs + extra:
                    grp.add(pr["dy"], pr["x"], pr["gw"], pr["gb"], pr["N"], pr["K"], pr["swiglu_h"], accumulate=not self.wgrad_overwrite)
                groups[gkey] = grp.finalize(self.store.device, scratch)
            if pending is not None:
                yield ("block", pending[0])
            pending = (i, grp)
        self.held = None
        if drop:
            ops.cast_f32_bf16(dy, dy_b, M * D)
        elif pending is not None and hold_last:
            OVERLAP.run_deferred()
            self.held = pending
        elif pending is not None:
            pending[1].launch()
            yield ("block", pending[0])
        return dy, dy_b


_ROPE_CACHE: Dict[tuple, Tuple[torch.Tensor, torch.Tensor]] = {}


def _rope_host(per: torch.Tensor, H: int, W: int, aug=None) -> Tuple[torch.Tensor, torch.Tensor]:
    dd = {"dtype": per.dtype}
    ch = torch.arange(0.5, H, **dd) / H
    cw = torch.arange(0.5, W, **dd) / W
    coords = torch.stack(torch.meshgrid(ch, cw, indexing="ij"), dim=-1).flatten(0, 1)
    coords = 2.0 * coords - 1.0
    if aug is not None:
        if aug.get("shift") is not None:
            coords += aug["shift"][None, :]
        if aug.get("jitter") is not None:
            coords *= aug["jitter"][None, :]
        if aug.get("rescale") is not None:
            coords *= aug["rescale"]
    ang = 2 * math.pi * coords[:, :, None] / per[None, None, :]
    ang = ang.flatten(1, 2).tile(2)
    return torch.sin(ang).to(torch.bfloat16).contiguous(), torch.cos(ang).to(torch.bfloat16).contiguous()


def rope_tables(periods: torch.Tensor, H: int, W: int, device) -> Tuple[torch.Tensor, torch.Tensor]:
    per = periods.detach().to("cpu")
    key = (H, W, str(device), per.dtype, tuple(per.float().tolist()))
    hit = _ROPE_CACHE.get(key)
    if hit is not None:
        return hit
    sin, cos = _rope_host(per, H, W)
    sin, cos = sin.to(device), cos.to(device)
    _ROPE_CACHE[key] = (sin, cos)
    return sin, cos


class RopeAugTabs:
    __slots__ = ("sin_all", "cos_all", "off", "hw")

    def __init__(self, sin_all, cos_all, off, hw):
        self.sin_all, self.cos_all, self.off, self.hw = sin_all, cos_all, off, hw

    def at(self, i: int):
        i = min(i, self.sin_all.shape[0] - 1)
        return self.sin_all[i, self.off:self.off + self.hw], self.cos_all[i, self.off:self.off + self.hw]


def rope_at(rp, i: int):
    return rp.at(i) if isinstance(rp, RopeAugTabs) else rp


def _rope_hw(rp) -> int:
    return rp.hw if isinstance(rp, RopeAugTabs) else rp[0].shape[0]


class RopeAugmenter:

    def __init__(self, periods: torch.Tensor, depth: int, per_block: bool, shift, jitter, rescale, seed: int = 0):
        self.per, self.depth, self.per_block = periods.detach().to("cpu"), depth, per_block
        self.cfg = (shift, jitter, rescale)
        self.engine_id = int(seed)
        self.gen = torch.Generator().manual_seed(int(seed))
        self.records: Dict[tuple, dict] = {}
        self.touched = set()
        self.last_draws = None

    def reseed(self, base_seed: int, rank: int = 0):
        self.gen.manual_seed((int(base_seed) * 1000003 + int(rank)) * 8 + self.engine_id)

    def get_state(self) -> torch.Tensor:
        return self.gen.get_state().clone()
# ... 19 lines not shown
            rm = float(np.log(rescale))
            d["rescale"] = torch.empty(1, **dd).uniform_(-rm, rm, generator=self.gen).exp()
        return d

    def record(self, key, hws, device):
        rec = self.records.get(key)
        if rec is None:
            P = sum(h * w for h, w in hws)
            nb = self.depth if self.per_block else 1
            rec = dict(hws=list(hws), sin=torch.zeros(nb, P, 64, dtype=torch.bfloat16, device=device),
                       cos=torch.zeros(nb, P, 64, dtype=torch.bfloat16, device=device),
                       host=torch.zeros(2, nb, P, 64, dtype=torch.bfloat16).pin_memory(), event=None, fresh=False)
            self.records[key] = rec
        return rec

    def refresh(self, rec):
        if rec["event"] is not None:
            rec["event"].synchronize()
        nb = rec["sin"].shape[0]
        draws = []
        for i in range(nb):
            row, off = [], 0
            for h, w in rec["hws"]:
                d = self._draw()
                sin, cos = _rope_host(self.per, h, w, d)
                rec["host"][0, i, off:off + h * w].copy_(sin)
                rec["host"][1, i, off:off + h * w].copy_(cos)
                off += h * w
                row.append(d)
            draws.append(row)
        rec["sin"].copy_(rec["host"][0], non_blocking=True)
        rec["cos"].copy_(rec["host"][1], non_blocking=True)
        ev = torch.cuda.Event()
        ev.record()
        rec["event"], rec["fresh"] = ev, True
        self.last_draws = draws

    def tables(self, key, hws, device):
        rec = self.record(key, hws, device)
        self.touched.add(key)
        if torch.cuda.is_current_stream_capturing():
            if not rec["fresh"]:
                raise RuntimeError("RoPE augmentation tables must exist before stream capture (run the step eagerly once)")
        else:
            self.refresh(rec)
        return rec

    def refresh_all(self, keys=None):
        for k, rec in self.records.items():
            if keys is None or k in keys:
                self.refresh(rec)


class TrunkEngine:
    def __init__(self, store: ParamStore, cfg, periods: torch.Tensor, prefix: str = "trunk."):
        from .config import ffn_hidden
        self.store = store
        self.prefix = prefix
        self.D, self.heads, self.depth = cfg.vision_embed_dim, cfg.vision_num_heads, cfg.vision_depth
        self.H = ffn_hidden(self.D, cfg.vision_mlp_ratio, cfg.vision_ffn_layer)
        self.kind = ops.NORM_RMS if cfg.vision_norm_layer == "rmsnorm" else ops.NORM_LN
        self.eps = 1e-5 if self.kind == ops.NORM_RMS else 1e-6
        self.periods = periods.detach().to("cpu")
        self.pe = store.lin(self.prefix + "patch_embed.proj.weight", self.prefix + "patch_embed.proj.bias", self.D, 768)
        self.stack = Stack(store, self.prefix + "blocks.", self.depth, self.D, self.heads, self.H, cfg.vision_norm_layer,
                           ffn=cfg.vision_ffn_layer)
        self.bott_dim = cfg.vision_feature_bottleneck
        self.bott = store.lin(self.prefix + "feature_bottleneck.weight", None, self.bott_dim, self.D) \
            if store.has(self.prefix + "feature_bottleneck.weight") else None
        self.bott_wgrads: List[tuple] = []
        self.ws: Dict[tuple, Workspace] = {}
        self.rope_aug = RopeAugmenter(self.periods, self.depth, True, getattr(cfg, "vision_rope_shift_coords", None),
                                      getattr(cfg, "vision_rope_jitter_coords", None), getattr(cfg, "vision_rope_rescale_coords", None),
                                      seed=1 if prefix == "trunk." else 2)

    def workspace(self, key) -> Workspace:
        if key not in self.ws:
            self.ws[key] = Workspace(self.store.device)
        return self.ws[key]

    def forward(self, img: torch.Tensor, train: bool, masks: Optional[torch.Tensor] = None, tag: str = "", rope_aug: Optional[bool] = None):
        return self.forward_list([(img, masks)], train, tag, rope_aug=rope_aug)

    def forward_list(self, items, train: bool, tag: str = "", rope_aug: Optional[bool] = None):
        st = self.store
        D = self.D
        segs, r0, p0 = [], 0, 0
        for img, masks in items:
            B, _, Hh, Ww = img.shape
            h, w = Hh // 16, Ww // 16
            sg = TrunkSeg()
            sg.B, sg.h, sg.w, sg.hw, sg.N, sg.row0, sg.prow0, sg.masks, sg.img = B, h, w, h * w, h * w + 1, r0, p0, masks, img
            sg.rope = rope_tables(self.periods, h, w, st.device)
            segs.append(sg)
            r0 += B * sg.N
            p0 += B * sg.hw
        M, P = r0, p0
        ws = self.workspace((tuple((g.B, g.h, g.w) for g in segs), tag))
        if self.rope_aug.active and (train if rope_aug is None else rope_aug):
            rec = self.rope_aug.tables((tuple((g.B, g.h, g.w) for g in segs), tag), [(g.h, g.w) for g in segs], st.device)
            off = 0
            for g in segs:
                g.rope = RopeAugTabs(rec["sin"], rec["cos"], off, g.hw)
                off += g.hw
        patches = ws.get("patches_tok", (M, 768), BF, zero=True)
        x0 = ws.get("x0", (M, D), F32)
        for g in segs:
            pt, xs = patches[g.row0:g.row0 + g.B * g.N], x0[g.row0:g.row0 + g.B * g.N]
            ops.im2col16_rows(g.img, pt, g.B, g.h * 16, g.w * 16, 1)
            ops.gemm_nt(pt, self.pe.w, xs, M=g.B * g.hw, N=D, K=768, bias=self.pe.bias, epi=EPI_F32, a_remap=(g.hw, 1), c_remap=(g.hw, 1))
            ops.assemble_tokens(xs, st.p(self.prefix + "cls_token"), st.p(self.prefix + "mask_token"), g.masks, g.B, g.N, D)
        stack_segs = [(g.B, g.N, g.rope) for g in segs]
        xl = self.stack.forward(ws, x0, stack_segs, 1, train)
        xnf = ws.get("xnf", (M, D), BF)
        stf = ws.get("stf", (M, 2), F32)
        ops.norm_fwd(xl, st.p(self.prefix + "norm.weight"), st.p(self.prefix + "norm.bias") if self.kind == ops.NORM_LN else None, xnf, stf,
                     M, D, self.eps, self.kind)
        c = TrunkCtx()
        c.ws, c.segs, c.M, c.xl, c.xnf, c.stf, c.patches, c.stack_saved, c.x0, c.stack_segs = \
            ws, segs, M, xl, xnf, stf, patches, self.stack.last_saved, x0, stack_segs
        self._ctx = c
        return xnf

    def ctx(self):
        return self._ctx

    def latents(self, out_f32: bool = False, seg: int = 0) -> torch.Tensor:
        c = self._ctx
        g = c.segs[seg]
        lat = c.ws.get("lat32" if out_f32 else "lat", (g.B * g.hw, self.bott_dim), F32 if out_f32 else BF)
        ops.gemm_nt(c.xnf[g.row0:], self.bott.w, lat, M=g.B * g.hw, N=self.bott_dim, K=self.D,
                    epi=EPI_F32 if out_f32 else EPI_BF16, a_remap=(g.hw, 1))
        return lat

    def bott_rows(self, x: torch.Tensor, R: int, out: torch.Tensor, lda: Optional[int] = None) -> torch.Tensor:
        ops.gemm_nt(x, self.bott.w, out, M=R, N=self.bott_dim, K=self.D, lda=x.stride(0) if lda is None else lda, epi=EPI_BF16)
        return out

    def bott_rows_bwd(self, dz: torch.Tensor, x: torch.Tensor, R: int, dx: Optional[torch.Tensor], alpha: float = 1.0):
        if dx is not None:
            ops.gemm_nt(dz, self.bott.wT, dx, M=R, N=self.D, K=self.bott_dim, ldc=dx.stride(0),
                        epi=EPI_F32 if dx.dtype == F32 else EPI_BF16, alpha=alpha)
        self.bott_wgrads.append((dz, x, R))

    def d_xnf_buffer(self, ctx=None) -> torch.Tensor:
        c = self._ctx if ctx is None else ctx
        return c.ws.get("b.d_xnf", (c.M, self.D), BF, zero=True)

    def backward(self, d_lat: Optional[torch.Tensor], ctx=None, lat_seg: int = 0, want_dimg: bool = False, pool=None):
        st = self.store
        if ctx is not None:
            self._ctx = ctx
        c = self._ctx
        ws, M, D = c.ws, c.M, self.D
        d_xnf = ws.get("b.d_xnf", (M, D), BF, zero=True)
        wgrads, self.bott_wgrads = self.bott_wgrads, []
        for dz, x, R in wgrads:
            linear_bwd(ws, "bott", self.bott, dz, x, R, None, need_dx=False)
        if d_lat is not None:
            g = c.segs[lat_seg]
            linear_bwd(ws, "bott", self.bott, d_lat, c.xnf[g.row0:], g.B * g.hw, d_xnf[g.row0:], x_remap=(g.hw, 1),
                       dx_remap=(g.hw, 1))
        dx = ws.get("b.dxt", (M, D), F32)
        dx_b = ws.get("b.dxt_b", (M, D), BF)
        nw, nb = st.g(self.prefix + "norm.weight"), st.g(self.prefix + "norm.bias") if self.kind == ops.NORM_LN else None
        if pool is None:
            ops.norm_bwd(d_xnf, c.xl, st.p(self.prefix + "norm.weight"), c.stf, None, dx, dx_b, nw, nb, M, D, self.kind,
                         dx_colsum=self.stack.w3_colsum_target(self.depth - 1))
        else:
            g = c.segs[pool[0]]
            ops.norm_bwd_pvec(d_xnf, c.xl, st.p(self.prefix + "norm.weight"), c.stf, None, dx, dx_b, nw, nb, M, D, self.kind, pool[1],
                              g.row0, g.B, g.N, dx_colsum=self.stack.w3_colsum_target(self.depth - 1))
        OVERLAP.join()
        yield "tail"
        g_cls, g_mask = st.g(self.prefix + "cls_token"), st.g(self.prefix + "mask_token")
        extra = None
        if not want_dimg and D % 8 == 0:
            extra = [dict(x=c.patches, gw=self.pe.gw, gb=self.pe.gb, N=self.pe.N, K=self.pe.K, swiglu_h=0)]
        dx0, dx0_b = yield from self.stack.backward(ws, dx, dx_b, c.stack_segs, 1, c.stack_saved,
                                                    dy_colsum_done=self.stack.w3_colsum_target(self.depth - 1) is not None,
                                                    hold_last=extra is not None, extra_last=extra)
        held, self.stack.held = self.stack.held, None
        for g in c.segs:
            d_s, d_sb = dx0[g.row0:g.row0 + g.B * g.N], dx0_b[g.row0:g.row0 + g.B * g.N]
            ops.token_rows_bwd(d_s, d_sb, g.masks, g_mask if g.masks is not None else None, g_cls, g.B, g.N, D)
        if held is not None:
            held[1].launch()
            yield ("block", held[0])
        else:
            for item, g in enumerate(c.segs):
                d_sb = dx0_b[g.row0:g.row0 + g.B * g.N]
                linear_bwd(ws, "pe", self.pe, d_sb, c.patches[g.row0:g.row0 + g.B * g.N], g.B * g.hw, None, need_dx=False,
                           dy_remap=(g.hw, 1), x_remap=(g.hw, 1))
                if want_dimg:
                    dpt = ws.get(f"b.dpatch{g.prow0}", (g.B * g.hw, 768), F32)
                    ops.gemm_nt(d_sb, self.pe.wT, dpt, M=g.B * g.hw, N=768, K=D, epi=EPI_F32, a_remap=(g.hw, 1))
                    dimg = torch.empty(g.B, 3, g.h * 16, g.w * 16, dtype=F32, device=st.device)
                    ops.col2im16(dpt, dimg, g.B, g.h * 16, g.w * 16)
                    c.__dict__.setdefault("d_img", {})[item] = dimg
        OVERLAP.join()


class TrunkSeg:
    """One item of a list forward: B images of (16h x 16w) pixels -> rows [row0, row0 + B*N) of the token buffers."""


class TrunkCtx:

    def take_d_img(self, item: int = 0):
        return self.__dict__.get("d_img", {}).pop(item)


class DecoderEngine:
    def __init__(self, store: ParamStore, cfg, periods: torch.Tensor):
        from .config import ffn_hidden
        self.store = store
        self.D, self.heads, self.depth = cfg.decoder_embed_dim, cfg.decoder_num_heads, cfg.decoder_depth
        self.H = ffn_hidden(self.D, 4.0, cfg.decoder_ffn_layer)
        self.kind = ops.NORM_RMS if cfg.decoder_norm_layer == "rmsnorm" else ops.NORM_LN
        self.eps = 1e-5 if self.kind == ops.NORM_RMS else 1e-6
        self.periods = periods.detach().to("cpu")
        self.cin = cfg.vision_feature_bottleneck
        self.pin = store.lin("pixel_decoder.proj_in.weight", "pixel_decoder.proj_in.bias", self.D, self.cin)
        self.stack = Stack(store, "pixel_decoder.blocks.", self.depth, self.D, self.heads, self.H, cfg.decoder_norm_layer,
                           ffn=cfg.decoder_ffn_layer)
        self.pout = store.lin("pixel_decoder.proj_out.weight", "pixel_decoder.proj_out.bias", 768, self.D)
        self.ws: Dict[tuple, Workspace] = {}
        self.rope_aug = RopeAugmenter(self.periods, self.depth, False, getattr(cfg, "decoder_rope_shift_coords", None),
                                      getattr(cfg, "decoder_rope_jitter_coords", None), getattr(cfg, "decoder_rope_rescale_coords", None), seed=3)

    def workspace(self, B, h, w) -> Workspace:
        key = (B, h, w)
        if key not in self.ws:
            self.ws[key] = Workspace(self.store.device)
        return self.ws[key]

    def forward(self, lat: torch.Tensor, B: int, h: int, w: int, train: bool) -> torch.Tensor:
# ... 40 lines not shown
```

vtp_amd/ops.py:

```python
from __future__ import annotations

import torch

from . import _lib

EPI_BF16, EPI_F32, EPI_SWIGLU, EPI_GELU, EPI_F32_ATOMIC, EPI_F32_SLAB = 0, 1, 2, 3, 4, 5
EPI_QUICK_GELU = 8
NORM_RMS, NORM_LN = 0, 1


def _s():
    return torch.cuda.current_stream().cuda_stream


def _p(t):
    return 0 if t is None else t.data_ptr()


def _lib_():
    return _lib.load()


def pad8(n: int) -> int:
    return (n + 7) // 8 * 8


def gemm_nt(a, b, c, *, M=None, N=None, K=None, lda=None, ldb=None, ldc=None, c2=None, ldc2=0, bias=None, gamma=None,
            resid=None, epi=EPI_BF16, a_remap=(0, 0), c_remap=(0, 0), splits=1, alpha=1.0):
    M = a.shape[0] if M is None else M
    K = a.shape[1] if K is None else K
    N = b.shape[0] if N is None else N
    lda = a.stride(0) if lda is None else lda
    ldb = b.stride(0) if ldb is None else ldb
    ldc = c.stride(0) if ldc is None else ldc
    if c2 is not None and not ldc2:
        ldc2 = c2.stride(0)
    rc = _lib_().vtp_gemm_nt(_p(a), lda, _p(b), ldb, _p(c), ldc, _p(c2), ldc2, _p(bias), _p(gamma), _p(resid), M, N, K,
                             epi, a_remap[0], a_remap[1], c_remap[0], c_remap[1], splits, alpha, _s())
    _lib.check(rc, "vtp_gemm_nt")


def gemm_qkv_rope(a, w, bias, c, M, N, K, rope_pos, rope_sin, rope_cos, rope_cols):
    _lib.check(_lib_().vtp_gemm_qkv_rope(_p(a), a.stride(0), _p(w), w.stride(0), _p(bias), _p(c), c.stride(0), M, N, K,
                                         _p(rope_pos), _p(rope_sin), _p(rope_cos), rope_cols, _s()), "vtp_gemm_qkv_rope")


def norm_fwd(x, w, b, y, stats, M, D, eps, kind):
    _lib.check(_lib_().vtp_norm_fwd(_p(x), _p(w), _p(b), _p(y), _p(stats), M, D, eps, kind, _s()), "vtp_norm_fwd")


def norm_bwd(dy, x, w, stats, dres, dx, dxb, dw, db, M, D, kind, dx_colsum=None):
    _lib.check(_lib_().vtp_norm_bwd(_p(dy), _p(x), _p(w), _p(stats), _p(dres), _p(dx), _p(dxb), _p(dw), _p(db), _p(dx_colsum),
                                    M, D, kind, _s()), "vtp_norm_bwd")


def norm_bwd_pvec(dy, x, w, stats, dres, dx, dxb, dw, db, M, D, kind, pvec, row0, B, N, dx_colsum=None):
    _lib.check(_lib_().vtp_norm_bwd_pvec(_p(dy), _p(x), _p(w), _p(stats), _p(dres), _p(dx), _p(dxb), _p(dw), _p(db), _p(dx_colsum),
                                         _p(pvec), row0, B, N, M, D, kind, _s()), "vtp_norm_bwd_pvec")


def pool_patch_rows(x, out, B, N, D, scale=None):
    assert x.dtype == torch.bfloat16 and x.is_contiguous() and x.numel() >= B * N * D and out.dtype == torch.float32
    assert out.is_contiguous() and out.numel() >= B * D
    s = 1.0 / (N - 1) if scale is None else float(scale)
    _lib.check(_lib_().vtp_pool_patch_rows(_p(x), _p(out), B, N, D, s, _s()), "vtp_pool_patch_rows")


def rope_qk(qkv, sin, cos, B, N, heads, prefix, inverse=False):
    _lib.check(_lib_().vtp_rope_qk(_p(qkv), _p(sin), _p(cos), B, N, heads, prefix, int(inverse), _s()), "vtp_rope_qk")


def attn_fwd(q, k, v, o, lse, B, N, heads, sb, sn, sbo, sno, scale, causal=False):
    _lib.check(_lib_().vtp_attn_fwd(_p(q), _p(k), _p(v), _p(o), _p(lse), B, N, heads, sb, sn, sbo, sno, scale, int(causal),
                                    _s()), "vtp_attn_fwd")


def attn_bwd(q, k, v, o, d_o, lse, delta, dq, dk, dv, B, N, heads, sb, sn, sbo, sno, scale, causal=False, rope=None,
             rope_prefix=0):
    rs, rc = (rope[0], rope[1]) if rope is not None else (None, None)
    _lib.check(_lib_().vtp_attn_bwd(_p(q), _p(k), _p(v), _p(o), _p(d_o), _p(lse), _p(delta), _p(dq), _p(dk), _p(dv), _p(rs),
                                    _p(rc), rope_prefix, B, N, heads, sb, sn, sbo, sno, scale, int(causal), _s()), "vtp_attn_bwd")


def im2col16(img, patches, B, H, W):
    _lib.check(_lib_().vtp_im2col16(_p(img), _p(patches), B, H, W, _s()), "vtp_im2col16")


def im2col16_rows(img, rows, B, H, W, prefix=1):
    _lib.check(_lib_().vtp_im2col16_rows(_p(img), _p(rows), B, H, W, prefix, _s()), "vtp_im2col16_rows")


def col2im16(dpatches, dimg, B, H, W):
    _lib.check(_lib_().vtp_col2im16(_p(dpatches), _p(dimg), B, H, W, _s()), "vtp_col2im16")


def assemble_tokens(x, cls, mask_token, masks, B, N, D):
    _lib.check(_lib_().vtp_assemble_tokens(_p(x), _p(cls), _p(mask_token), _p(masks), B, N, D, _s()), "vtp_assemble_tokens")


def transpose_bf16(inp, ld_in, out, ld_out, R, C, colsum=None, swiglu_h=0, in_remap=(0, 0)):
    _lib.check(_lib_().vtp_transpose_bf16(_p(inp), ld_in, _p(out), ld_out, _p(colsum), swiglu_h, in_remap[0], in_remap[1],
                                          R, C, _s()), "vtp_transpose_bf16")


def strided_rowsum(inp, stride, out, B, D):
    _lib.check(_lib_().vtp_strided_rowsum(_p(inp), stride, _p(out), B, D, _s()), "vtp_strided_rowsum")


def token_rows_bwd(dx, dxb, masks, d_mask_token, d_cls_token, B, N, D):
    _lib.check(_lib_().vtp_token_rows_bwd(_p(dx), _p(dxb), _p(masks), None if masks is None else _p(d_mask_token), _p(d_cls_token), B, N, D,
                                          _s()), "vtp_token_rows_bwd")


def mask_rows_bwd(dx, dxb, masks, d_mask_token, B, N, D):
    _lib.check(_lib_().vtp_mask_rows_bwd(_p(dx), _p(dxb), _p(masks), _p(d_mask_token), B, N, D, _s()), "vtp_mask_rows_bwd")


def cast_f32_bf16(inp, out, n):
    _lib.check(_lib_().vtp_cast_f32_bf16(_p(inp), _p(out), n, _s()), "vtp_cast_f32_bf16")


def cast_transpose_f32_bf16(inp, out, R, C):
    _lib.check(_lib_().vtp_cast_transpose_f32_bf16(_p(inp), _p(out), R, C, _s()), "vtp_cast_transpose_f32_bf16")


def prep_weights(descs, n, total_tiles):
    _lib.check(_lib_().vtp_prep_weights(_p(descs), n, total_tiles, _s()), "vtp_prep_weights")


def prep_weights_range(descs_run, n, tile_base, n_tiles):
    _lib.check(_lib_().vtp_prep_weights_range(_p(descs_run), n, tile_base, n_tiles, _s()), "vtp_prep_weights_range")


def swiglu_bwd(dh, x12, dx12, M, H, db12=None):
    _lib.check(_lib_().vtp_swiglu_bwd(_p(dh), _p(x12), _p(dx12), _p(db12), M, H, _s()), "vtp_swiglu_bwd")


def gelu_bwd(dy, pre, dx, n, quick: bool = False):
    if quick:
        _lib.check(_lib_().vtp_quick_gelu_bwd(_p(dy), _p(pre), _p(dx), n, _s()), "vtp_quick_gelu_bwd")
    else:
        _lib.check(_lib_().vtp_gelu_bwd(_p(dy), _p(pre), _p(dx), n, _s()), "vtp_gelu_bwd")


def pixel_shuffle16(t, img, B, h, w):
    _lib.check(_lib_().vtp_pixel_shuffle16(_p(t), _p(img), B, h, w, _s()), "vtp_pixel_shuffle16")


def pixel_unshuffle16(d_img, dt, B, h, w):
    _lib.check(_lib_().vtp_pixel_unshuffle16(_p(d_img), _p(dt), B, h, w, _s()), "vtp_pixel_unshuffle16")


def l1_loss_fwd_bwd(t, target, dt, loss_sum, B, h, w, gscale):
    _lib.check(_lib_().vtp_l1_loss_fwd_bwd(_p(t), _p(target), _p(dt), _p(loss_sum), B, h, w, gscale, _s()),
               "vtp_l1_loss_fwd_bwd")


def adamw(p, g, m, v, p_bf16, n, lr, beta1, beta2, eps, wd, step, grad_scale=1.0):
    _lib.check(_lib_().vtp_adamw(_p(p), _p(g), _p(m), _p(v), _p(p_bf16), n, lr, beta1, beta2, eps, wd, step, grad_scale,
                                 _s()), "vtp_adamw")


def adamw_dev(p, g, m, v, p_bf16, n, hyper, nodecay4=None):
    if nodecay4 is None:
        _lib.check(_lib_().vtp_adamw_dev(_p(p), _p(g), _p(m), _p(v), _p(p_bf16), n, _p(hyper), _s()), "vtp_adamw_dev")
    else:
        _lib.check(_lib_().vtp_adamw_dev_masked(_p(p), _p(g), _p(m), _p(v), _p(p_bf16), _p(nodecay4), n, _p(hyper), _s()),
                   "vtp_adamw_dev_masked")


def gemm_tn(a, b, c, *, M, N, K, lda, ldb, ldc, ldc2=0, resid=None, epi=EPI_F32, a_remap=(0, 0), b_remap=(0, 0),
            c_remap=(0, 0), splits=1, a_colsum=None):
    rc = _lib_().vtp_gemm_tn(_p(a), lda, _p(b), ldb, _p(c), ldc, ldc2, _p(resid), M, N, K, epi, a_remap[0], a_remap[1],
                             b_remap[0], b_remap[1], c_remap[0], c_remap[1], splits, _p(a_colsum), _s())
    _lib.check(rc, "vtp_gemm_tn")


def wgrad_group_fits(Ktok: int, max_ld: int) -> bool:
    return int(Ktok) * int(max_ld) * 2 < (1 << 32)


def gemm_cus() -> int:
    import os
    try:
        v = int(os.environ.get("VTP_GEMM_CUS", "0") or 0)
    except ValueError:
        v = 0
    return v - v % 8 if 8 <= v < 256 else 256


def wgrad_group_splits(ntiles: int, Ktok: int):
    s = max(1, min(gemm_cus() // ntiles, Ktok // 1024))
    ks = ((Ktok + s - 1) // s + 63) // 64 * 64
    return ks, (Ktok + ks - 1) // ks


def wgrad_group_kernel(ntiles: int, splits: int, Ktok: int) -> int:
    import os
    e = os.environ.get("VTP_GEMM4W_TN")
    if Ktok % 8 != 0 or e == "0":
        return 0
    if e == "1":
        return 1
    return 1 if Ktok // max(splits, 1) >= W4_TN_MIN_SLICE else 0


def wgrad_k_cuts(Ktok: int, n: int):
    ks = ((Ktok + n - 1) // n + 63) // 64 * 64
    return [(b, min(Ktok, b + ks) - b) for b in range(0, Ktok, ks)]


def wgrad_group_items(rows, Ktok: int, base_splits: int, cus: int = None):
    cus = gemm_cus() if cus is None else cus
    tiles = []
    for pi, r in enumerate(rows):
        gb, N, K, tile0 = r[3], r[7], r[8], r[11]
        tn = (K + 255) // 256
        for lt in range(((N + 255) // 256) * tn):
            tiles.append((tile0 + lt, pi, gb != 0 and lt % tn == 0))
    ncs = sum(1 for t in tiles if t[2])
    more = ncs > 0 and len(tiles) * base_splits + ncs <= cus and Ktok // (base_splits + 1) >= 1024
    items, slots = [], 1
    for pi in range(len(rows)):
        for heavy in (True, False):
            grp = [t for t in tiles if t[1] == pi and t[2] == heavy]
            if not grp:
                continue
            cs = wgrad_k_cuts(Ktok, base_splits + 1 if (heavy and more) else base_splits)
            slots = max(slots, len(cs))
            for z, (kb, kc) in enumerate(cs):
                items += [[t[0], kb, kc, len(cs), z, 0, 0, 0] for t in grp]
    return items, slots


def wgrad_group_uniform_items(ntiles: int, Ktok: int, splits: int):
    cs = wgrad_k_cuts(Ktok, max(int(splits), 1))
    return [[t, kb, kc, len(cs), z, 0, 0, 0] for z, (kb, kc) in enumerate(cs) for t in range(ntiles)], len(cs)


W4_TN_MIN_SLICE = 4096


class WgradGroup:

    def __init__(self, Ktok: int):
        self.Ktok, self.rows, self.ntiles, self.keep = int(Ktok), [], 0, []
        self.table = self.part = self.ticket = None
        self._uniform = {}

    def add(self, dy, x, gw, gb, N: int, K: int, swiglu_h: int = 0, accumulate: bool = True):
        if N % 8 or K % 8 or dy.stride(0) % 8 or x.stride(0) % 8 or N < 8 or K < 8:
            raise ValueError(f"WgradGroup.add: N = {N}, K = {K} and the leading dimensions ({dy.stride(0)}, {x.stride(0)}) must be multiples "
                             "of 8 (use the per-layer weight-gradient path: linear_bwd without `defer`)")
        self.rows.append([dy.data_ptr(), x.data_ptr(), gw.data_ptr(), 0 if gb is None else gb.data_ptr(), dy.stride(0), x.stride(0), K,
                          N, K, -1 if swiglu_h else 0, swiglu_h, self.ntiles, int(accumulate), 0, 0, 0])
        self.ntiles += ((N + 255) // 256) * ((K + 255) // 256)
        self.keep += [dy, x, gw, gb]

    def finalize(self, device, scratch=None):
        import torch
        assert 1 <= len(self.rows) <= 8
        if not wgrad_group_fits(self.Ktok, max(max(r[4], r[5]) for r in self.rows)):
            raise ValueError("WgradGroup: token rows x leading dimension exceed the 32-bit staging offsets of vtp_gemm_tn_grouped; "
                             "use the per-layer weight-gradient path (linear_bwd without `defer`)")
        _, self.splits = wgrad_group_splits(self.ntiles, self.Ktok)
        self.table = torch.tensor(self.rows, dtype=torch.int64, device=device)
        self.kernel = wgrad_group_kernel(self.ntiles, self.splits, self.Ktok)
        self.items, self.nitems, self.slots = None, None, self.splits
        if self.kernel == 1:
            items, self.slots = wgrad_group_items(self.rows, self.Ktok, self.splits)
            self.nitems = len(items)
            self.items = torch.tensor(items, dtype=torch.int32, device=device)
        if self.slots > 1:
            scratch = {} if scratch is None else scratch
            need = self.ntiles * self.slots * 65536
            if scratch.get("part") is None or scratch["part"].numel() < need:
                scratch["part"] = torch.empty(need, dtype=torch.float32, device=device)
            if scratch.get("ticket") is None or scratch["ticket"].numel() < self.ntiles:
                scratch["ticket"] = torch.zeros(max(self.ntiles, 256), dtype=torch.int32, device=device)
            self.part, self.ticket = scratch["part"], scratch["ticket"]
        return self

    def launch(self, kernel=None):
        if kernel is None:
            kernel = self.kernel
        if kernel == 0:
            _lib.check(_lib_().vtp_gemm_tn_grouped(_p(self.table), len(self.rows), self.ntiles, self.Ktok, self.splits, _p(self.part),
                                                   _p(self.ticket), _s()), "vtp_gemm_tn_grouped")
            return
        if kernel != 1:
            raise ValueError(f"WgradGroup.launch: kernel must be 0, 1 or None, not {kernel!r}")
        items, nitems, slots = self.items, self.nitems, self.slots
        if items is None:
            if self.splits not in self._uniform:
                import torch
                rows, slots = wgrad_group_uniform_items(self.ntiles, self.Ktok, self.splits)
                self._uniform[self.splits] = (torch.tensor(rows, dtype=torch.int32, device=self.table.device), len(rows), slots)
            items, nitems, slots = self._uniform[self.splits]
        _lib.check(_lib_().vtp_gemm_tn_grouped_items(_p(self.table), len(self.rows), self.ntiles, self.Ktok, _p(items), nitems, slots,
                                                     _p(self.part), _p(self.ticket), _s()), "vtp_gemm_tn_grouped_items")


def colsum_bf16(inp, ld, out, R, C, swiglu_h=0, in_remap=(0, 0)):
    _lib.check(_lib_().vtp_colsum_bf16(_p(inp), ld, _p(out), swiglu_h, in_remap[0], in_remap[1], R, C, _s()), "vtp_colsum_bf16")


def colsum_bf16_rows(inp, ld, out, n_rows_dev, R_max, C):
    _lib.check(_lib_().vtp_colsum_bf16_rows(_p(inp), ld, _p(out), _p(n_rows_dev), R_max, C, _s()), "vtp_colsum_bf16_rows")


def gather_image_rows(src, idx, dst, dst_bf16, n_img, N, D, scale=1.0):
    _lib.check(_lib_().vtp_gather_image_rows(_p(src), _p(idx), _p(dst), _p(dst_bf16), n_img, N, D, scale, _s()), "vtp_gather_image_rows")


def scatter_image_rows(src, idx, dst, n_img, N, D, alpha=1.0, accumulate=True):
    _lib.check(_lib_().vtp_scatter_image_rows(_p(src), _p(idx), _p(dst), n_img, N, D, alpha, int(accumulate), _s()),
               "vtp_scatter_image_rows")


def layerscale_wgrad(G, W, bias, colsum, gamma, dW, db, dgamma, N, K):
    _lib.check(_lib_().vtp_layerscale_wgrad(_p(G), _p(W), _p(bias), _p(colsum), _p(gamma), _p(dW), _p(db), _p(dgamma), N, K, _s()),
               "vtp_layerscale_wgrad")


def scaled_transpose(W, gamma, dstT, N, K):
    _lib.check(_lib_().vtp_scaled_transpose(_p(W), _p(gamma), _p(dstT), N, K, _s()), "vtp_scaled_transpose")


def gemm_splits(K, splits):
    return _lib_().vtp_gemm_splits(K, splits)


def gemm_tn_splits(M, N, K):
    return _lib_().vtp_gemm_tn_splits(M, N, K)


def reduce_slabs(slabs, stride, S, dst, n, accumulate=True):
    _lib.check(_lib_().vtp_reduce_slabs(_p(slabs), stride, S, _p(dst), n, int(accumulate), _s()), "vtp_reduce_slabs")


def ema(t, s, n, momentum):
    _lib.check(_lib_().vtp_ema(_p(t), _p(s), n, momentum, _s()), "vtp_ema")


def embed_tokens(ids, table, pos, x, eot, B, T, D):
    _lib.check(_lib_().vtp_embed_tokens(_p(ids), _p(table), _p(pos), _p(x), _p(eot), B, T, D, _s()), "vtp_embed_tokens")


def embed_tokens_bwd(ids, dx, d_table, d_pos, B, T, D):
    _lib.check(_lib_().vtp_embed_tokens_bwd(_p(ids), _p(dx), _p(d_table), _p(d_pos), B, T, D, _s()), "vtp_embed_tokens_bwd")


def gather_rows(x, idx, out, B, T, D):
    _lib.check(_lib_().vtp_gather_rows(_p(x), _p(idx), _p(out), B, T, D, _s()), "vtp_gather_rows")


def scatter_rows(dy, idx, dx, dxb, B, T, D):
    _lib.check(_lib_().vtp_scatter_rows(_p(dy), _p(idx), _p(dx), _p(dxb), B, T, D, _s()), "vtp_scatter_rows")


def l2norm_fwd(x, y, inv, B, D, eps=1e-12):
    _lib.check(_lib_().vtp_l2norm_fwd(_p(x), _p(y), _p(inv), B, D, eps, _s()), "vtp_l2norm_fwd")


def l2norm_bwd(dy, y, inv, dx, B, D):
    _lib.check(_lib_().vtp_l2norm_bwd(_p(dy), _p(y), _p(inv), _p(dx), B, D, _s()), "vtp_l2norm_bwd")


def clip_loss(img_l, txt_l, img_all, txt_all, logit_scale, Bl, Bg, D, label_offset, loss_sum, d_img_l, d_txt_l, d_img_all,
              d_txt_all, d_logit_scale, scratch):
    _lib.check(_lib_().vtp_clip_loss(_p(img_l), _p(txt_l), _p(img_all), _p(txt_all), _p(logit_scale), Bl, Bg, D, label_offset,
                                     _p(loss_sum), _p(d_img_l), _p(d_txt_l), _p(d_img_all), _p(d_txt_all), _p(d_logit_scale),
                                     _p(scratch), _s()), "vtp_clip_loss")


def qk_norm_fwd(qkv, wq, wk, out, inv, M, D, eps=1e-5):
    _lib.check(_lib_().vtp_qk_norm_fwd(_p(qkv), _p(wq), _p(wk), _p(out), _p(inv), M, D, eps, _s()), "vtp_qk_norm_fwd")


def qk_norm_bwd(dqkv, qkv, inv, wq, wk, dwq, dwk, M, D):
    _lib.check(_lib_().vtp_qk_norm_bwd(_p(dqkv), _p(qkv), _p(inv), _p(wq), _p(wk), _p(dwq), _p(dwk), M, D, _s()), "vtp_qk_norm_bwd")


def gemm_dgrad_swiglu(dy, wT, x12, dx12, M, H, K):
    _lib.check(_lib_().vtp_gemm_dgrad_swiglu(_p(dy), dy.stride(0), _p(wT), wT.stride(0), _p(x12), x12.stride(0), _p(dx12), dx12.stride(0),
                                             M, H, K, _s()), "vtp_gemm_dgrad_swiglu")


def clip_logits(a, b, logit_scale, out, M, N, D):
    _lib.check(_lib_().vtp_clip_logits(_p(a), _p(b), _p(logit_scale), _p(out), M, N, D, _s()), "vtp_clip_logits")


def siglip_loss(img_l, txt_all, logit_scale, logit_bias, Bl, Bg, D, label_offset, loss_sum, d_img_l, d_txt_all, d_logit_scale,
                d_logit_bias, scratch):
    L, s = _lib_(), _s()
    _lib.check(L.vtp_clip_logits(_p(img_l), _p(txt_all), _p(logit_scale), _p(scratch), Bl, Bg, D, s), "vtp_clip_logits")
    _lib.check(L.vtp_siglip_pairs(_p(scratch), _p(logit_bias), Bl, Bg, label_offset, 1.0 / Bl, _p(loss_sum), _p(d_logit_scale),
                                  _p(d_logit_bias), s), "vtp_siglip_pairs")
    _lib.check(L.vtp_clip_grad_rows(_p(scratch), _p(txt_all), _p(logit_scale), _p(d_img_l), Bl, Bg, D, 0, s), "vtp_clip_grad_rows")
    _lib.check(L.vtp_clip_grad_cols(_p(scratch), _p(img_l), _p(logit_scale), _p(d_txt_all), Bl, Bg, D, 0, s), "vtp_clip_grad_cols")


# ... 179 lines not shown
```

vtp_amd/ssl_engine.py:

```python
from __future__ import annotations

from typing import Dict, Optional

import numpy as np
import torch

from . import ops
from .engine import BF, F32, OVERLAP, ParamStore, Workspace, linear_bwd
from .ops import EPI_BF16, EPI_F32, EPI_GELU

I32 = torch.int32


class DinoHeadEngine:

    def __init__(self, store: ParamStore, prefix: str, Din: int, hidden: int, bott: int, K: int):
        self.store, self.prefix, self.Din, self.hidden, self.bott, self.K = store, prefix, Din, hidden, bott, K
        self.l1 = store.lin(prefix + "mlp.0.weight", prefix + "mlp.0.bias", hidden, Din)
        self.l2 = store.lin(prefix + "mlp.2.weight", prefix + "mlp.2.bias", hidden, hidden)
        self.l3 = store.lin(prefix + "mlp.4.weight", prefix + "mlp.4.bias", bott, hidden)
        self.v, self.g = store.p(prefix + "last_layer.weight_v"), store.p(prefix + "last_layer.weight_g")
        self.gv, self.gg = store.g(prefix + "last_layer.weight_v"), store.g(prefix + "last_layer.weight_g")
        dev = store.device
        self.weff = torch.empty(K, bott, dtype=BF, device=dev)
# ... 22 lines not shown
        pre1, h1 = ws.get("pre1", (T, hid), BF), ws.get("h1", (T, hid), BF)
        pre2, h2 = ws.get("pre2", (T, hid), BF), ws.get("h2", (T, hid), BF)
        z, zn = ws.get("z", (T, bott), F32), ws.get("zn", (T, bott), F32)
        inv_z = ws.get("inv_z", (T,), F32)
        zn_b = ws.get("zn_b", (T, bott), BF)
        logits = ws.get("logits", (T, K), BF)
        ops.gemm_nt(X, self.l1.w, h1, M=T, N=hid, K=self.Din, c2=pre1, ldc2=hid, bias=self.l1.bias, epi=EPI_GELU)
        ops.gemm_nt(h1, self.l2.w, h2, M=T, N=hid, K=hid, c2=pre2, ldc2=hid, bias=self.l2.bias, epi=EPI_GELU)
        ops.gemm_nt(h2, self.l3.w, z, M=T, N=bott, K=hid, bias=self.l3.bias, epi=EPI_F32)
        ops.l2norm_fwd(z, zn, inv_z, T, bott, 1e-12)
        ops.cast_f32_bf16(zn, zn_b, T * bott)
        ops.gemm_nt(zn_b, self.weff, logits, M=T, N=K, K=bott, epi=EPI_BF16)
        return logits, (ws, X, T, pre1, h1, pre2, h2, zn, inv_z, zn_b)

    def backward(self, d_logits: torch.Tensor, ctx) -> torch.Tensor:
        ws, X, T, pre1, h1, pre2, h2, zn, inv_z, zn_b = ctx
        hid, bott, K = self.hidden, self.bott, self.K
        dWeff = ws.get("b.dWeff", (K, bott), F32)
        ops.gemm_tn(d_logits, zn_b, dWeff, M=K, N=bott, K=T, lda=K, ldb=bott, ldc=bott, epi=EPI_F32)
        ops.weight_norm_bwd(dWeff, self.v, self.g, self.inv_norm, self.gv, self.gg, K, bott)
        d_zn = ws.get("b.d_zn", (T, bott), F32)
        S = ops.gemm_splits(K, max(1, min(16, K // 2048)))
        if S == 1:
            ops.gemm_nt(d_logits, self.weffT, d_zn, M=T, N=bott, K=K, epi=EPI_F32)
        else:
            slab = ws.get("b.d_zn_slab", (S * T * bott,), F32)
            ops.gemm_nt(d_logits, self.weffT, slab, M=T, N=bott, K=K, ldc=bott, ldc2=T * bott // 4, epi=ops.EPI_F32_SLAB,
                        splits=S)
            ops.reduce_slabs(slab, T * bott, S, d_zn, T * bott, accumulate=False)
        dz = ws.get("b.dz", (T, bott), F32)
        ops.l2norm_bwd(d_zn, zn, inv_z, dz, T, bott)
        dz_b = ws.get("b.dz_b", (T, bott), BF)
        ops.cast_f32_bf16(dz, dz_b, T * bott)
        dh = ws.get("b.dh", (T, hid), BF)
        dpre2, dpre1 = ws.get("b.dpre2", (T, hid), BF), ws.get("b.dpre1", (T, hid), BF)
        linear_bwd(ws, "l3", self.l3, dz_b, h2, T, dh)
        ops.gelu_bwd(dh, pre2, dpre2, T * hid)
        linear_bwd(ws, "l2", self.l2, dpre2, h1, T, dh)
        ops.gelu_bwd(dh, pre1, dpre1, T * hid)
        dX = ws.get("b.dX", (T, self.Din), BF)
        linear_bwd(ws, "l1", self.l1, dpre1, X, T, dX)
        OVERLAP.join()
        return dX


def build_ssl_indices(masks: np.ndarray, B: int, hw: int, n_local: int, hw_local: int, dino_weight: float,
                      ibot_weight: float, pad_to: int = 64, upperbound: Optional[int] = None):
    N = hw + 1
    n_g = 2
    flat = np.flatnonzero(masks.reshape(-1))
    n_masked = int(flat.size)
    if upperbound is not None:
        if n_masked > upperbound:
            raise ValueError(f"{n_masked} masked patches exceed upperbound={upperbound}")
        pad_to, n_cap = 64, int(upperbound)
    else:
        n_cap = n_masked
    Tm = max(pad_to, (n_cap + pad_to - 1) // pad_to * pad_to)
    img_of = flat // hw
    masked_rows = (img_of * N + 1 + flat % hw).astype(np.int32)
    per_img = np.maximum(masks.sum(1), 1)
    mw = (1.0 / per_img[img_of]).astype(np.float32)
    pad = np.full(Tm - n_masked, -1, np.int32)
    t_cls = np.concatenate([np.arange(B, 2 * B), np.arange(0, B)]).astype(np.int32) * N
    teacher_src = np.concatenate([t_cls, masked_rows, pad])
    local_src = (np.arange(n_local * B) * (hw_local + 1)).astype(np.int32)
    terms = n_g * (n_g - 1) + n_local * n_g
    w_cls = dino_weight / (B * terms)
    Ts = n_local * B + 2 * B + Tm
    t0 = np.full(Ts, -1, np.int32)
    t1 = np.full(Ts, -1, np.int32)
    w = np.zeros(Ts, np.float32)
    b_idx = np.tile(np.arange(B), n_local)
    t0[:n_local * B] = b_idx
    t1[:n_local * B] = B + b_idx
    w[:n_local * B] = w_cls
    g0 = n_local * B
    t0[g0:g0 + 2 * B] = np.arange(2 * B)
    w[g0:g0 + 2 * B] = w_cls
    m0 = g0 + 2 * B
    t0[m0:m0 + n_masked] = 2 * B + np.arange(n_masked)
    w[m0:m0 + n_masked] = ibot_weight * mw / B
    student_global_src = np.concatenate([np.arange(2 * B, dtype=np.int32) * N, masked_rows, pad])
    return dict(n_masked=n_masked, Tm=Tm, Ts=Ts, teacher_src=teacher_src, student_local_src=local_src,
                student_global_src=student_global_src, t0=t0, t1=t1, w=w)
```

vtp_amd/train.py:

```python
from __future__ import annotations

import math
import os
from typing import List, Optional, Sequence, Tuple

import torch

from . import ops
from .engine import BF, F32, OVERLAP


class GradBucketer:

    def __init__(self, flat_g: torch.Tensor, group=None, shard: bool = False, grad_dtype: torch.dtype = torch.float32,
                 force: bool = False):
        import torch.distributed as dist
        self.dist = dist
        self.flat_g = flat_g
        self.group = group
        self.world = dist.get_world_size(group) if dist.is_available() and dist.is_initialized() else 1
        self.rank = dist.get_rank(group) if self.world > 1 else 0
        self.active = self.world > 1 or (bool(force) and dist.is_available() and dist.is_initialized())
        self.works = []
        self.reduced_elems = 0
# ... 423 lines not shown
        if self.text is not None and model.config.text_pool_type == "none":
            self._clip_unsupported = "the contrastive objective needs pooled text features (text_pool_type argmax | first | last)"
        elif self.text is not None and model.config.vision_clip_feat == "pooled" and model.config.vision_embed_dim > 1024:
            self._clip_unsupported = (f"vision_clip_feat='pooled' needs vision_embed_dim <= 1024 on the fused step "
                                      f"(got {model.config.vision_embed_dim}); the autograd path (model(...); loss.backward()) has no limit")
        else:
            self._clip_unsupported = None
        self.sync_replicas()

    @property
    def max_grad_norm(self) -> Optional[float]:
        return self._max_grad_norm

    @max_grad_norm.setter
    def max_grad_norm(self, value):
        if (value is None) != (self._max_grad_norm is None):
            raise ValueError("max_grad_norm: clipping cannot be switched on or off after construction; build the trainer with "
                             "max_grad_norm=None or with a number")
        self._max_grad_norm = None if value is None else _max_norm_value(value)

    @property
    def skip_nonfinite(self) -> bool:
        return self._skip

    def sync_replicas(self):
        if not self.collectives:
            return
        dist, st = self.bucketer.dist, self.store
        bufs = [st.flat_p, self.m, self.v]
        if self._skip:
            bufs.append(self._skip_state)
        if self.ssl_head is not None:
            bufs += [self.center_dino, self.center_ibot]
        for b in bufs:
            dist.broadcast(b, src=dist.get_global_rank(self.group, 0) if self.group is not None else 0, group=self.group)
        st.prep()
        self.model._pver = self.model._param_version()

    def _plan_buckets(self):
        off = self.store.offsets

        def rng(*prefixes):
            return param_ranges(off, prefixes)

        plan = {"dec_tail": rng("pixel_decoder.norm.", "pixel_decoder.proj_out."),
                "dec_head": rng("pixel_decoder.proj_in."),
                "trunk_tail": rng("trunk.norm.", "trunk.feature_bottleneck."),
                "trunk_head": rng("trunk.cls_token", "trunk.mask_token", "trunk.patch_embed."),
                "text_tail": rng("ln_final.", "text_projection"),
                "text_head": rng("token_embedding.", "positional_embedding"),
                "clip_head": rng("visual_proj.", "logit_scale", "logit_bias"), "dino_head": rng("dino_head.")}
        towers = [("dec", "pixel_decoder.blocks.", self.decoder.depth), ("trunk", "trunk.blocks.", self.trunk.depth)]
        if self.text is not None:
            towers.append(("text", "text_transformer.resblocks.", self.text.depth))
        for key, prefix, depth in towers:
            for i in range(depth):
                plan[f"{key}.{i}"] = rng(f"{prefix}{i}.")
        return plan

    def _reduce(self, keys: Sequence[str]):
        if not self.collectives or not keys:
            return
        rs = merge_ranges([r for k in keys for r in self._bucket_plan[k]])
        for lo, hi in rs:
            self.bucketer.reduce_range(lo, hi)

    def _tower_backward(self, tower: str, gen, depth: int):
        nb = self.bucket_blocks
        result = None
        try:
            while True:
                ev = next(gen)
                if ev == "tail":
                    yield [f"{tower}_tail"]
                elif ev[0] == "block" and ev[1] % nb == 0:
                    i = ev[1]
                    yield [f"{tower}.{j}" for j in range(i, min(i + nb, depth))]
        except StopIteration as stop:
            result = stop.value
        return result

    def _ssl_gen(self, P, lead_images=None):
        from .vtp import ssl_forward
        out = ssl_forward(self.model, P["global"], P["local"], P["masks"], P["plan"], P["dev"], train=True, lead_images=lead_images)
        self._zero_join()
        if not (self.head_overlap and not self.collectives and OVERLAP.enabled):
            yield from self._ssl_tail(out, P)
            return out
        main = torch.cuda.current_stream()
        self.trunk.d_xnf_buffer(out["ctx"]).zero_()
        if self._head_stream is None:
            self._head_stream = torch.cuda.Stream()
        self._head_stream.wait_stream(main)
        with torch.cuda.stream(self._head_stream), OVERLAP.lane(2):
            was, OVERLAP.enabled = OVERLAP.enabled, False
            try:
                for ev in self._ssl_tail(out, P, zero_dxnf=False):
                    if callable(ev):
                        raise RuntimeError("head stream: the SSL tail asked for a collective")
                    self._head_keys += ev
            finally:
                OVERLAP.enabled = was
        return out

    def _ssl_tail(self, out, P, zero_dxnf: bool = True):
        model, st, head = self.model, self.store, self.ssl_head
        dist = self.bucketer.dist
        K, D = head.K, self.trunk.D
        Tt, Ts, Tm, B2, nl = out["Tt"], out["Ts"], out["Tm"], out["B2"], out["nl"]
        ws = out["ws"]
        t_logits, s_logits = out["teacher_logits"], out["student_logits"]
        probs = ws.get("probs", (Tt, K), BF)
        if self.centering == "sinkhorn_knopp":
            yield from self._sinkhorn_targets(ws, t_logits, probs, P, B2, Tm, K)
        else:
            inv_tt = self.hyper[8:9]
            ops.softmax_center(t_logits, self.center_dino, inv_tt, probs, B2, K)
            ops.softmax_center(t_logits[B2:], self.center_ibot, inv_tt, probs[B2:], Tm, K)
            stats = self.center_stats
            stats.zero_()
            ops.colsum_bf16(t_logits, K, stats, B2, K)
            ops.colsum_bf16_rows(t_logits[B2:], K, stats[K:], P["dev"]["n_masked_i"], Tm, K)
            stats[2 * K:2 * K + 1].copy_(P["dev"]["n_masked_f"])

            def apply_centers():
                ops.center_ema(self.center_dino, stats, 1.0 / (B2 * self.world), self.center_momentum, K)
                ops.center_ema(self.center_ibot, stats[K:], 0.0, self.center_momentum, K, count=stats[2 * K:])
            if self.collectives:
                yield lambda: self.bucketer.works.append((dist.all_reduce(stats, group=self.group, async_op=True), None))
                self._deferred.append(apply_centers)
            else:
                apply_centers()
        d_logits = ws.get("d_logits", (Ts, K), BF)
        ops.dino_ce(s_logits, probs, P["dev"]["t0"], P["dev"]["t1"], P["dev"]["w"], 1.0 / self.student_temp, self.ssl_loss_sum,
                    d_logits, Ts, K)
        dX = head.backward(d_logits, out["head_ctx"])
        if self.koleo_weight > 0:
            self._koleo(ws, out["Hs"], dX, nl, B2, head.Din)
        yield ["dino_head"]
        from .vtp import ssl_head_input_bwd
        dX = ssl_head_input_bwd(model, out, dX)
        ctx = out["ctx"]
        d_xnf = self.trunk.d_xnf_buffer(ctx)
        if zero_dxnf:
            d_xnf.zero_()
        seg_g, seg_l = ctx.segs[-2], ctx.segs[-1]
        ops.scatter_token_rows(dX, P["dev"]["student_local_src"], d_xnf[seg_l.row0:], nl, D)
        ops.scatter_token_rows(dX[nl:], P["dev"]["student_global_src"], d_xnf[seg_g.row0:], Ts - nl, D)

    def _sinkhorn_targets(self, ws, t_logits, probs, P, B2, Tm, K):
        dist = self.bucketer.dist
        it = self.sk_iterations
        inv_t = 1.0 / self.teacher_temp
        for tag, lg, pr, T, cnt_dev, rows_dev, count in (("cls", t_logits, probs, B2, None, None, float(B2 * self.world)),
                                                         ("patch", t_logits[B2:], probs[B2:], Tm, P["dev"]["n_masked_f"],
                                                          P["dev"]["n_masked_i"], 0.0)):
            u, v = ws.get(f"sk.u.{tag}", (T,), F32), ws.get(f"sk.v.{tag}", (K,), F32)
            scr = ws.get(f"sk.s.{tag}", (8 + K + T,), F32)
            if not self.collectives:
                ops.sinkhorn_knopp(lg, inv_t, pr, u, v, scr, T, K, count, it, -1, cnt_dev, rows_dev)
                continue
            if cnt_dev is not None:
                gcnt = ws.get("sk.cnt", (1,), F32)
                gcnt.copy_(cnt_dev)
                yield lambda gcnt=gcnt: dist.all_reduce(gcnt, group=self.group)
                cnt_dev = gcnt
            ops.sinkhorn_knopp(lg, inv_t, pr, u, v, scr, T, K, count, 0, 0, cnt_dev, rows_dev)
            yield lambda scr=scr: dist.all_reduce(scr[:1], op=dist.ReduceOp.MAX, group=self.group)
            for i in range(it):
                ops.sinkhorn_knopp(lg, inv_t, pr, u, v, scr, T, K, count, i, 1, cnt_dev, rows_dev)
                yield lambda scr=scr: dist.all_reduce(scr[8:8 + K], group=self.group)
                ops.sinkhorn_knopp(lg, inv_t, pr, u, v, scr, T, K, count, i, 2, cnt_dev, rows_dev)
            ops.sinkhorn_knopp(lg, inv_t, pr, u, v, scr, T, K, count, it, 3, cnt_dev, rows_dev)

    def _koleo(self, ws, Xs, dX, nl, B2, D):
        B = B2 // 2
        self.koleo_loss_sum.zero_()
        x32 = ws.get("kl.x", (B2, D), F32)
        x32.copy_(Xs[nl:nl + B2])
        xn, inv = ws.get("kl.xn", (B2, D), F32), ws.get("kl.inv", (B2,), F32)
        ops.l2norm_fwd(x32, xn, inv, B2, D, 1e-8)
        d_xn = ws.get("kl.dxn", (B2, D), F32)
        d_xn.zero_()
        nn = ws.get("kl.nn", (B2,), torch.int32)
        for v in range(2):
            ops.koleo(xn[v * B:], nn[v * B:], d_xn[v * B:], self.koleo_loss_sum, B, D, self.koleo_weight / B)
        dx = ws.get("kl.dx", (B2, D), F32)
        ops.l2norm_bwd(d_xn, xn, inv, dx, B2, D)
        dxb = ws.get("kl.dxb", (B2, D), BF)
        dxb.copy_(dx)
        dX[nl:nl + B2].add_(dxb)

    def prepare_ssl(self, global_crops: torch.Tensor, local_crops: torch.Tensor, masks, pad_to: Optional[int] = None,
                    upperbound: Optional[int] = None) -> dict:
        from .ssl_engine import build_ssl_indices
        from .vtp import plan_to_device
        import numpy as np
        B = global_crops.shape[0] // 2
        hw = (global_crops.shape[-2] // 16) * (global_crops.shape[-1] // 16)
        hw_l = (local_crops.shape[-2] // 16) * (local_crops.shape[-1] // 16)
        n_local = local_crops.shape[0] // B
        m = masks.detach().cpu().numpy().astype(bool) if torch.is_tensor(masks) else np.asarray(masks, bool)
        plan = build_ssl_indices(m, B, hw, n_local, hw_l, self.dino_weight, self.ibot_weight,
                                 pad_to=int(pad_to or self.ssl_bucket), upperbound=upperbound)
        if self._stager is None:
            self._stager = HostStager(self.store.device)
        arrays = {k: plan[k].astype(np.int32, copy=False) for k in ("teacher_src", "student_local_src", "student_global_src", "t0", "t1")}
        arrays["w"] = plan["w"].astype(np.float32, copy=False)
        arrays["n_masked_i"] = np.array([plan["n_masked"]], np.int32)
        arrays["n_masked_f"] = np.array([float(plan["n_masked"])], np.float32)
        arrays["masks"] = m.astype(np.uint8)
        up = self._stager.upload(arrays)
        masks_dev = up.pop("masks")
        packed = up.pop("_packed")
        return dict(**{"global": global_crops, "local": local_crops}, masks=masks_dev, plan=plan, dev=up, packed=packed)

    def _step_gen(self, images: torch.Tensor, text: Optional[torch.Tensor], ssl: Optional[dict] = None, rec_images=None):
        self._reduced_ranges = []
        self._head_keys = []
        self._opt_queue, self._opt_done, self._hooks_done = [], [], set()
        self._clip_cursor, self._clip_keys = 0, []
        del OVERLAP._deferred[:]
        del self.trunk.bott_wgrads[:]
        self._opt_ema = ssl is not None
        lag = 2 if self.collectives else 1
        lazy_join = not self.collectives and (self.single_graph or not self.use_graphs)
        stacks = [e.stack for e in (self.trunk, self.decoder, getattr(self, "text", None)) if e is not None and hasattr(e, "stack")]
        if os.environ.get("VTP_WGRAD_OVERWRITE", "1") not in ("0", "false", "off"):
            for sk in stacks:
                sk.wgrad_overwrite = True
        try:
            for ev in self._step_body(images, text, ssl, rec_images):
                if not lazy_join or callable(ev) or "FINAL" in ev:
                    self._opt_join()
                if callable(ev):
                    yield ev
                    continue
                keys = [k for k in ev if k != "FINAL"]
                self._reduced_ranges += merge_ranges([r for k in keys for r in self._bucket_plan[k]])
                yield ev
                if self.overlap_opt and "FINAL" not in ev:
                    self._opt_queue.append(keys)
                    while len(self._opt_queue) >= lag:
                        self._opt_launch(self._opt_queue.pop(0))
                elif self.overlap_opt:
                    self._opt_queue.append(keys)
        finally:
            for sk in stacks:
                sk.wgrad_overwrite = False

    def _opt_plan(self, keys, ema: bool):
        ck = (tuple(keys), ema)
        plan = self._opt_plans.get(ck)
        if plan is None:
            st = self.store
            rs = merge_ranges([r for k in keys for r in self._bucket_plan[k]])
            pairs = []
            if ema:
                from .vtp import _range
                for t_pref, s_pref in self.model.ema_pairs():
                    (tlo, thi), (slo, shi) = _range(st, t_pref), _range(st, s_pref)
                    assert thi - tlo == shi - slo
                    pairs.append((tlo, slo, shi))
            pieces = lane_pieces(rs, pairs)
            runs = st.desc_runs(rs) + st.desc_runs([(tl, tl + b - a) for a, b, tl in pieces if tl is not None])
            plan = self._opt_plans[ck] = (pieces, runs)
        return plan

    def _opt_update(self, keys):
        st = self.store
        pieces, runs = self._opt_plan(keys, self._opt_ema)
        tab = self.group_tab
        for a, b, tl in pieces:
            teacher = None if tl is None else st.flat_p[tl:tl + b - a]
            if self._skip:
                idx4 = self._group4 if tab is not None else self.nodecay4
                ops.adamw_ema_dev_guarded(st.flat_p[a:b], st.flat_g[a:b], self.m[a:b], self.v[a:b], teacher, b - a, self.hyper,
                                          self.step_skipped, None if idx4 is None else idx4[a // 4:b // 4], tab,
                                          0 if tab is None else tab.shape[0])
            elif tab is not None:
                ops.adamw_ema_dev_grouped(st.flat_p[a:b], st.flat_g[a:b], self.m[a:b], self.v[a:b], teacher, b - a, self.hyper,
                                          self._group4[a // 4:b // 4], tab, tab.shape[0])
            else:
                ops.adamw_ema_dev(st.flat_p[a:b], st.flat_g[a:b], self.m[a:b], self.v[a:b], teacher,
                                  b - a, self.hyper, None if self.nodecay4 is None else self.nodecay4[a // 4:b // 4])
        st.prep_runs(runs)
        touched = [(a, b) for a, b, _ in pieces] + [(tl, tl + b - a) for a, b, tl in pieces if tl is not None]
        for hook, deps in getattr(st, "hook_deps", {}).items():
            if hook not in self._hooks_done and all(any(a <= lo and hi <= b for a, b in touched) for lo, hi in deps):
                hook()
# ... 640 lines not shown
```

vtp_amd/vtp.py:

```python
from __future__ import annotations

import copy
from typing import Dict, Optional

import numpy as np
import torch
from torch import nn

from . import autograd as ag
from . import ops
from .config import VTPConfig
from .engine import BF, F32, OVERLAP, TrunkEngine
from .model import VTPModel, _holder, _param
from .ssl_engine import DinoHeadEngine, build_ssl_indices

I32 = torch.int32


def _dino_head_tree(in_dim: int, hidden: int, bott: int, K: int) -> nn.Module:
    h = _holder()
    h.mlp = nn.ModuleList([_holder() for _ in range(5)])
    for i, (o, k) in zip((0, 2, 4), ((hidden, in_dim), (hidden, hidden), (bott, hidden))):
        h.mlp[i].weight = _param(o, k)
        h.mlp[i].bias = _param(o)
# ... 104 lines not shown
            scale = self.logit_scale.exp()
        if self.output_dict:
            out = {"image_features": image_features, "text_features": text_features, "logit_scale": scale}
            if self.logit_bias is not None:
                out["logit_bias"] = self.logit_bias
            return out
        if self.logit_bias is not None:
            return image_features, text_features, scale, self.logit_bias
        return image_features, text_features, scale

    def forward_reconstruction(self, reconstruction_image: torch.Tensor):
        if self.pixel_decoder is None:
            return {}
        lat = self.get_reconstruction_latents(reconstruction_image)
        return {"reconstructed_image": self.get_latents_decoded_images(lat), "target_image": reconstruction_image}

    def forward(self, image=None, text=None, ssl_dict: Optional[dict] = None, reconstruction_image=None,
                forward_type: str = "clip"):
        assert forward_type in ["clip", "ssl", "rec"], "Invalid forward type"
        if forward_type == "clip":
            return self.forward_clip(image, text)
        if forward_type == "ssl":
            return self.forward_ssl_learning(**ssl_dict)
        return self.forward_reconstruction(reconstruction_image)

    def forward_ssl_learning(self, global_crops, n_global_crops, mask_indices_list, n_masked_patches, upperbound,
                             local_crops, masks, masks_weight=None):
        if n_global_crops != 2:
            raise NotImplementedError("n_global_crops must be 2")
        if ag.grad_mode(self):
            return self._forward_ssl_autograd(global_crops, local_crops, masks, n_masked_patches, upperbound)
        return self._forward_ssl_nograd(global_crops, n_global_crops, mask_indices_list, n_masked_patches, upperbound, local_crops,
                                        masks)

    def _forward_ssl_autograd(self, global_crops, local_crops, masks, n_masked_patches, upperbound):
        self._fresh()
        B2 = global_crops.shape[0]
        B = B2 // 2
        hw = (global_crops.shape[-2] // 16) * (global_crops.shape[-1] // 16)
        hw_l = (local_crops.shape[-2] // 16) * (local_crops.shape[-1] // 16)
        n_local = local_crops.shape[0] // B
        plan = build_ssl_indices(masks.detach().cpu().numpy().astype(bool), B, hw, n_local, hw_l, 1.0, 1.0, pad_to=8)
        assert plan["n_masked"] == int(n_masked_patches) <= int(upperbound)
        m8 = masks.to(self._store.device).to(torch.uint8).contiguous()
        s_loc, s_glob, s_cls, s_patch, t_logits = ag.SSLStudent.apply(ag.anchor(self), self, self._img(global_crops),
                                                                      self._img(local_crops), m8, plan)
        nm = plan["n_masked"]
        teacher_outputs = {"teacher_cls_tokens_after_head": t_logits[:B2], "n_masked_patches": n_masked_patches,
                           "masked_teacher_patch_tokens_after_head": t_logits[B2:B2 + nm]}
        student_outputs = {"student_local_cls_tokens_after_head": s_loc, "student_global_cls_tokens_after_head": s_glob,
                           "student_global_cls_tokens": s_cls, "student_global_masked_patch_tokens_after_head": s_patch}
        return teacher_outputs, student_outputs

    @torch.no_grad()
    def _forward_ssl_nograd(self, global_crops, n_global_crops, mask_indices_list, n_masked_patches, upperbound, local_crops,
                            masks):
        self._fresh()
        B2 = global_crops.shape[0]
        B = B2 // 2
        hw = (global_crops.shape[-2] // 16) * (global_crops.shape[-1] // 16)
        hw_l = (local_crops.shape[-2] // 16) * (local_crops.shape[-1] // 16)
        n_local = local_crops.shape[0] // B
        plan = build_ssl_indices(masks.detach().cpu().numpy().astype(bool), B, hw, n_local, hw_l, 1.0, 1.0, pad_to=8)
        assert plan["n_masked"] == int(n_masked_patches) <= int(upperbound)
        out = ssl_forward(self, self._img(global_crops), self._img(local_crops), masks.to(self._store.device), plan, train=False)
        nm, nl = plan["n_masked"], n_local * B
        tl, sl = out["teacher_logits"].float(), out["student_logits"].float()
        teacher_outputs = {"teacher_cls_tokens_after_head": tl[:B2].clone(), "n_masked_patches": n_masked_patches,
                           "masked_teacher_patch_tokens_after_head": tl[B2:B2 + nm].clone()}
        student_outputs = {"student_local_cls_tokens_after_head": sl[:nl].clone(),
                           "student_global_cls_tokens_after_head": sl[nl:nl + B2].clone(),
                           "student_global_cls_tokens": out["student_global_cls"].float().clone(),
                           "student_global_masked_patch_tokens_after_head": sl[nl + B2:nl + B2 + nm].clone()}
        return teacher_outputs, student_outputs


def _range(st, prefix):
    offs = [(o, o + (k + 3) // 4 * 4) for n, (o, k) in st.offsets.items() if n.startswith(prefix)]
    lo, hi = min(o for o, _ in offs), max(h for _, h in offs)
    assert sum(h - o for o, h in offs) == hi - lo, f"{prefix} is not contiguous in the flat buffer"
    return lo, hi


def plan_to_device(plan, device):
    d = {k: torch.as_tensor(plan[k], device=device) for k in ("teacher_src", "student_local_src", "student_global_src", "t0", "t1")}
    d["w"] = torch.as_tensor(plan["w"], device=device)
    d["n_masked_i"] = torch.tensor([plan["n_masked"]], dtype=torch.int32, device=device)
    d["n_masked_f"] = torch.tensor([float(plan["n_masked"])], dtype=torch.float32, device=device)
    return d


def ssl_forward(model: "VTP", global_crops, local_crops, masks_u8, plan, dev_plan=None, train: bool = False,
                lead_images=None):
    st = model._store
    B2 = global_crops.shape[0]
    hw = (global_crops.shape[-2] // 16) * (global_crops.shape[-1] // 16)
    N = hw + 1
    D = model.config.vision_embed_dim
    idx = plan_to_device(plan, st.device) if dev_plan is None else dev_plan
    Tm, Ts = plan["Tm"], plan["Ts"]
    Tt = B2 + Tm
    if masks_u8.dtype != torch.uint8:
        masks_u8 = masks_u8.to(torch.uint8).contiguous()
    ws = model._head.workspace(Ts, "ssl_io")
    Xt = ws.get("Xt", (Tt, D), BF)

    Dh = model.dino_cfg["in_dim"]
    bott = Dh != D

    def teacher():
        xnf_t = model._t_trunk.forward(global_crops, train=False, tag="teacher", rope_aug=train)
        ops.gather_token_rows(xnf_t, idx["teacher_src"], Xt, Tt, D)
        Ht = model._t_trunk.bott_rows(Xt, Tt, ws.get("Zt", (Tt, Dh), BF)) if bott else Xt
        return model._t_head.forward(Ht, Tt, tag="teacher")[0]

    if OVERLAP.enabled:
        OVERLAP.join()
        OVERLAP.fork()
        with torch.cuda.stream(OVERLAP.side):
            t_logits = teacher()
    else:
        t_logits = teacher()
    leads = [] if lead_images is None else (list(lead_images) if isinstance(lead_images, (list, tuple)) else [lead_images])
    items = [(im, None) for im in leads] + [(global_crops, masks_u8), (local_crops, None)]
    xnf = model._trunk.forward_list(items, train=train, tag="ssl")
    ctx = model._trunk.ctx()
    seg_g, seg_l = ctx.segs[-2], ctx.segs[-1]
    nl = int(plan["student_local_src"].shape[0])
    Xs = ws.get("Xs", (Ts, D), BF)
    ops.gather_token_rows(xnf[seg_l.row0:], idx["student_local_src"], Xs, nl, D)
    ops.gather_token_rows(xnf[seg_g.row0:], idx["student_global_src"], Xs[nl:], Ts - nl, D)
    Hs = model._trunk.bott_rows(Xs, Ts, ws.get("Zs", (Ts, Dh), BF)) if bott else Xs
    s_logits, head_ctx = model._head.forward(Hs, Ts, tag="student")
    OVERLAP.join()
    return dict(teacher_logits=t_logits, student_logits=s_logits, head_ctx=head_ctx, ctx=ctx, xnf=xnf, idx=idx,
                Xs=Xs, Hs=Hs, bott=bott, student_global_cls=Hs[nl:nl + B2], Tt=Tt, Ts=Ts, Tm=Tm, nl=nl, B2=B2, N=N, ws=ws)


def ssl_head_input_bwd(model: "VTP", out, dH):
    if not out["bott"]:
        return dH
    Ts, D = out["Ts"], model._trunk.D
    dXs = out["ws"].get("b.dXs", (Ts, D), BF)
    model._trunk.bott_rows_bwd(dH, out["Xs"], Ts, dXs)
    return dXs
```

Measured before the change: 738.5.

## Compute last transformer block's proj/FFN only on rows consumed by SSL heads

In the final trunk block, the attention output projection, the residual and the FFN now run only on the token rows that the DINO/iBOT heads actually gather (cls plus masked patches), for both teacher and student. In the backward pass the proj wgrad/dgrad use the compacted rows and are expanded back through a row map, and a mapped norm-backward reads the residual gradient through that map. This removes full-sequence GEMM work in the last block at the cost of gather and expand kernels, plus a per-problem K field in the grouped wgrad GEMM.

```diff
diff --git a/include/vtp_hip.h b/include/vtp_hip.h
--- a/include/vtp_hip.h
+++ b/include/vtp_hip.h
@@ -36,6 +36,10 @@
                           void* stream);
 int vtp_scatter_image_rows(const float* src, const int* img_idx, float* dst, int n_img, long N, int D, float alpha, int accumulate,
                            void* stream);
+int vtp_gather_tail_rows(const void* o, const float* x, const int* idx, void* o_c, float* x_c, int T, int L, int M, int D,
+                         void* stream);
+int vtp_tail_row_map(const int* idx, int* map, int T, int L, int M, void* stream);
+int vtp_expand_rows_bf16(const void* src, const int* map, void* dst, int M, int Mc, int D, void* stream);
 int vtp_layerscale_wgrad(const float* G, const float* W, const float* bias, const float* colsum, const float* gamma, float* dW,
                          float* db, float* dgamma, int N, int K, void* stream);
 int vtp_scaled_transpose(const float* W, const float* gamma, void* dstT, int N, int K, void* stream);
@@ -50,6 +54,9 @@
 int vtp_norm_bwd_pvec(const void* dy, const float* x, const float* w, const float* stats, const float* dres, float* dx,
                       void* dx_bf16, float* dw, float* db, float* dx_colsum, const float* pvec, int prow0, int pB, int pN, int M,
                       int D, int kind, void* stream);
+int vtp_norm_bwd_rows(const void* dy, const float* x, const float* w, const float* stats, const float* dres, const int* dres_rows,
+                      int dres_M, float* dx, void* dx_bf16, float* dw, float* db, float* dx_colsum, int M, int D, int kind,
+                      void* stream);
 int vtp_pool_patch_rows(const void* x, float* out, int B, int N, int D, float scale, void* stream);
 
 int vtp_rope_qk(void* qkv, const void* sin, const void* cos, int B, int N, int heads, int prefix, int inverse,
diff --git a/vtp_amd/_lib.py b/vtp_amd/_lib.py
--- a/vtp_amd/_lib.py
+++ b/vtp_amd/_lib.py
@@ -12,6 +12,7 @@
     "vtp_norm_fwd": [_P, _P, _P, _P, _P, _I, _I, _F, _I, _P],
     "vtp_norm_bwd": [_P, _P, _P, _P, _P, _P, _P, _P, _P, _P, _I, _I, _I, _P],
     "vtp_norm_bwd_pvec": [_P, _P, _P, _P, _P, _P, _P, _P, _P, _P, _P, _I, _I, _I, _I, _I, _I, _P],
+    "vtp_norm_bwd_rows": [_P, _P, _P, _P, _P, _P, _I, _P, _P, _P, _P, _P, _I, _I, _I, _P],
     "vtp_pool_patch_rows": [_P, _P, _I, _I, _I, _F, _P],
     "vtp_rope_qk": [_P, _P, _P, _I, _I, _I, _I, _I, _P],
     "vtp_attn_fwd": [_P, _P, _P, _P, _P, _I, _I, _I, _L, _L, _L, _L, _F, _I, _P],
@@ -49,6 +50,9 @@
     "vtp_colsum_bf16_rows": [_P, _I, _P, _P, _I, _I, _P],
     "vtp_gather_image_rows": [_P, _P, _P, _P, _I, _L, _I, _F, _P],
     "vtp_scatter_image_rows": [_P, _P, _P, _I, _L, _I, _F, _I, _P],
+    "vtp_gather_tail_rows": [_P, _P, _P, _P, _P, _I, _I, _I, _I, _P],
+    "vtp_tail_row_map": [_P, _P, _I, _I, _I, _P],
+    "vtp_expand_rows_bf16": [_P, _P, _P, _I, _I, _I, _P],
     "vtp_layerscale_wgrad": [_P, _P, _P, _P, _P, _P, _P, _P, _I, _I, _P],
     "vtp_scaled_transpose": [_P, _P, _P, _I, _I, _P],
     "vtp_qk_norm_fwd": [_P, _P, _P, _P, _P, _L, _I, _F, _P],
diff --git a/vtp_amd/csrc/block_extras.hip b/vtp_amd/csrc/block_extras.hip
--- a/vtp_amd/csrc/block_extras.hip
+++ b/vtp_amd/csrc/block_extras.hip
@@ -154,6 +154,55 @@
   }
 }
 
+
+__global__ __launch_bounds__(256) void gather_tail_rows_kernel(const bf16* __restrict__ o, const float* __restrict__ x,
+                                                               const int* __restrict__ idx, bf16* __restrict__ o_c,
+                                                               float* __restrict__ x_c, int T, int L, int M, int D) {
+  const int cb = o ? D / 8 : 0, cpr = cb + (x ? D / 4 : 0);
+  const long total = (long)(L + T) * cpr;
+  for (long i = blockIdx.x * 256L + threadIdx.x; i < total; i += (long)gridDim.x * 256L) {
+    const int j = (int)(i / cpr), c = (int)(i - (long)j * cpr);
+    int r = j;
+    if (j >= L) {
+      r = idx[j - L];
+      r = (r >= 0 && r < M - L) ? r + L : -1;
+    }
+    if (c < cb) {
+      bf16x8 v = bf16x8{};
+      if (r >= 0) v = *(const bf16x8*)(o + (long)r * D + 8 * c);
+      *(bf16x8*)(o_c + (long)j * D + 8 * c) = v;
+    } else {
+      const int c4 = c - cb;
+      f32x4 v = (f32x4){0.f, 0.f, 0.f, 0.f};
+      if (r >= 0) v = *(const f32x4*)(x + (long)r * D + 4 * c4);
+      *(f32x4*)(x_c + (long)j * D + 4 * c4) = v;
+    }
+  }
+}
+
+__global__ __launch_bounds__(256) void tail_row_map_fill_kernel(int* __restrict__ map, int L, int M) {
+  for (int r = blockIdx.x * 256 + threadIdx.x; r < M; r += gridDim.x * 256) map[r] = r < L ? r : -1;
+}
+__global__ __launch_bounds__(256) void tail_row_map_set_kernel(const int* __restrict__ idx, int* __restrict__ map, int T, int L, int M) {
+  for (int t = blockIdx.x * 256 + threadIdx.x; t < T; t += gridDim.x * 256) {
+    const int r = idx[t];
+    if (r >= 0 && r < M - L) map[L + r] = L + t;
+  }
+}
+
+__global__ __launch_bounds__(256) void expand_rows_bf16_kernel(const bf16* __restrict__ src, const int* __restrict__ map,
+                                                               bf16* __restrict__ dst, int M, int Mc, int D) {
+  const int d8 = D / 8;
+  const long total = (long)M * d8;
+  for (long i = blockIdx.x * 256L + threadIdx.x; i < total; i += (long)gridDim.x * 256L) {
+    const int r = (int)(i / d8), c = (int)(i - (long)r * d8);
+    const int j = map[r];
+    bf16x8 v = bf16x8{};
+    if (j >= 0 && j < Mc) v = *(const bf16x8*)(src + (long)j * D + 8 * c);
+    *(bf16x8*)(dst + (long)r * D + 8 * c) = v;
+  }
+}
+
 }
 using namespace vtp;
 
@@ -209,3 +258,29 @@
                      (const bf16*)qkv, inv, wq, wk, dwq, dwk, M, D);
   return check_launch("qk_norm_bwd");
 }
+
+extern "C" int vtp_gather_tail_rows(const void* o, const float* x, const int* idx, void* o_c, float* x_c, int T, int L, int M, int D,
+                                    void* stream) {
+  VTP_REQUIRE((o || x) && (!o || o_c) && (!x || x_c) && (idx || T == 0), "vtp_gather_tail_rows: null pointer");
+  VTP_REQUIRE(T >= 0 && L >= 0 && L + T > 0 && L <= M && D > 0 && D % 8 == 0,
+              "vtp_gather_tail_rows: need L <= M, L + T > 0, D %% 8 == 0 (T=%d L=%d M=%d D=%d)", T, L, M, D);
+  const long items = (long)(L + T) * ((o ? D / 8 : 0) + (x ? D / 4 : 0));
+  hipLaunchKernelGGL(gather_tail_rows_kernel, dim3(extras_grid(items)), dim3(256), 0, (hipStream_t)stream, (const bf16*)o, x, idx,
+                     (bf16*)o_c, x_c, T, L, M, D);
+  return check_launch("gather_tail_rows");
+}
+
+extern "C" int vtp_tail_row_map(const int* idx, int* map, int T, int L, int M, void* stream) {
+  VTP_REQUIRE(map && (idx || T == 0) && T >= 0 && L >= 0 && L <= M && M > 0, "vtp_tail_row_map: bad argument (T=%d L=%d M=%d)", T, L, M);
+  hipLaunchKernelGGL(tail_row_map_fill_kernel, dim3(extras_grid(M)), dim3(256), 0, (hipStream_t)stream, map, L, M);
+  if (T > 0)
+    hipLaunchKernelGGL(tail_row_map_set_kernel, dim3(extras_grid(T)), dim3(256), 0, (hipStream_t)stream, idx, map, T, L, M);
+  return check_launch("tail_row_map");
+}
+
+extern "C" int vtp_expand_rows_bf16(const void* src, const int* map, void* dst, int M, int Mc, int D, void* stream) {
+  VTP_REQUIRE(src && map && dst && M > 0 && Mc > 0 && D > 0 && D % 8 == 0, "vtp_expand_rows_bf16: bad argument (D %% 8 == 0)");
+  hipLaunchKernelGGL(expand_rows_bf16_kernel, dim3(extras_grid((long)M * D / 8)), dim3(256), 0, (hipStream_t)stream, (const bf16*)src,
+                     map, (bf16*)dst, M, Mc, D);
+  return check_launch("expand_rows_bf16");
+}
diff --git a/vtp_amd/csrc/gemm4w_tn.hip b/vtp_amd/csrc/gemm4w_tn.hip
--- a/vtp_amd/csrc/gemm4w_tn.hip
+++ b/vtp_amd/csrc/gemm4w_tn.hip
@@ -74,12 +74,13 @@
   GemmArgs p{};
   p.A = w4t_uni(pr.A); p.B = w4t_uni(pr.B); p.C = w4t_uni(pr.C); p.resid = w4t_uni(pr.accumulate) ? (const float*)p.C : nullptr;
   p.colsum = w4t_uni(pr.colsum);
-  p.M = w4t_uni(pr.M); p.N = w4t_uni(pr.N); p.K = ga.K; p.lda = w4t_uni(pr.lda); p.ldb = w4t_uni(pr.ldb); p.ldc = w4t_uni(pr.ldc);
+  p.M = w4t_uni(pr.M); p.N = w4t_uni(pr.N); p.K = w4t_uni(pr.K) > 0 ? w4t_uni(pr.K) : ga.K; p.lda = w4t_uni(pr.lda); p.ldb = w4t_uni(pr.ldb); p.ldc = w4t_uni(pr.ldc);
   p.c_grp = w4t_uni(pr.c_grp); p.c_pre = w4t_uni(pr.c_pre); p.k_split = ga.k_split; p.alpha = 1.f;
   p.xcd_swizzle = 2;
   const int lt = tile - w4t_uni(pr.tile0), tiles_n = (p.N + 255) >> 8;
   const int n0 = (lt % tiles_n) << 8, m0 = (lt / tiles_n) << 8;
-  const unsigned nk2 = (unsigned)((kcount + 127) >> 7);
+  kcount = max(0, min(kcount, p.K - kbeg));
+  const unsigned nk2 = (unsigned)max(1, (kcount + 127) >> 7);
 
   const int krow = lane >> 3, chunk = (lane & 7) ^ (4 * ((krow >> 1) & 1));
   const int cola = min(m0 + wave * 64 + chunk * 8, p.M - 8), colb = min(n0 + wave * 64 + chunk * 8, p.N - 8);
diff --git a/vtp_amd/csrc/gemm_group.h b/vtp_amd/csrc/gemm_group.h
--- a/vtp_amd/csrc/gemm_group.h
+++ b/vtp_amd/csrc/gemm_group.h
@@ -13,7 +13,8 @@
   long c_grp, c_pre;
   long tile0;
   long accumulate;
-  long pad[3];
+  long K;
+  long pad[2];
 };
 struct GroupItem {
   int tile;
diff --git a/vtp_amd/csrc/norm.hip b/vtp_amd/csrc/norm.hip
--- a/vtp_amd/csrc/norm.hip
+++ b/vtp_amd/csrc/norm.hip
@@ -82,14 +82,14 @@
   }
 }
 
-template <int KIND, int NC, bool PV = false>
+template <int KIND, int NC, bool PV = false, bool MAPPED = false>
 __global__ __launch_bounds__(256, 2) void norm_bwd_kernel(const bf16* __restrict__ dy, const float* __restrict__ x,
                                                        const float* __restrict__ w, const float* __restrict__ stats,
                                                        const float* __restrict__ dres, float* __restrict__ dx,
                                                        bf16* __restrict__ dxb, float* __restrict__ dw, float* __restrict__ db,
                                                        float* __restrict__ dxsum, int M, int D,
                                                        const float* __restrict__ pvec = nullptr, int prow0 = 0, int pB = 0,
-                                                       int pN = 1) {
+                                                       int pN = 1, const int* __restrict__ dres_rows = nullptr, int dres_M = 0) {
   constexpr int R = NC <= 3 ? 2 : 1;
   const int lane = threadIdx.x & 63;
   const int wv_id = threadIdx.x >> 6;
@@ -112,6 +112,11 @@
       const int row = min(row0 + r, M - 1);
       mean[r] = stats[2 * row];
       rstd[r] = stats[2 * row + 1];
+      int drow = row;
+      if constexpr (MAPPED && PRE) {
+        drow = dres_rows[row];
+        if (drow >= dres_M) drow = -1;
+      }
 #pragma unroll
       for (int c = 0; c < NC; ++c) {
         const int col = (c * 64 + lane) * 4;
@@ -119,7 +124,8 @@
           xv[r][c] = *(const f32x4*)(x + (size_t)row * D + col);
           gy[r][c] = *(const bf16x4*)(dy + (size_t)row * D + col);
           if constexpr (PRE) {
-            if (dres) dr[r][c] = *(const f32x4*)(dres + (size_t)row * D + col);
+            if constexpr (MAPPED) dr[r][c] = drow >= 0 ? *(const f32x4*)(dres + (size_t)drow * D + col) : (f32x4){0.f, 0.f, 0.f, 0.f};
+            else if (dres) dr[r][c] = *(const f32x4*)(dres + (size_t)row * D + col);
           }
         }
       }
@@ -165,7 +171,10 @@
           for (int e = 0; e < 4; ++e) o[e] = rstd[r] * (g[c][e] - s1 - xh[c][e] * s2);
           if (dres) {
             if constexpr (PRE) o += dr[r][c];
-            else o += *(const f32x4*)(dres + (size_t)row * D + col);
+            else if constexpr (MAPPED) {
+              const int drow = dres_rows[row];
+              o += (drow >= 0 && drow < dres_M) ? *(const f32x4*)(dres + (size_t)drow * D + col) : (f32x4){0.f, 0.f, 0.f, 0.f};
+            } else o += *(const f32x4*)(dres + (size_t)row * D + col);
           }
           *(f32x4*)(dx + (size_t)row * D + col) = o;
           if (dxb) {
@@ -330,6 +339,37 @@
   return check_launch("norm_bwd_pvec");
 }
 
+extern "C" int vtp_norm_bwd_rows(const void* dy, const float* x, const float* w, const float* stats, const float* dres,
+                                 const int* dres_rows, int dres_M, float* dx, void* dx_bf16, float* dw, float* db, float* dx_colsum,
+                                 int M, int D, int kind, void* stream) {
+  if (!dres_rows)
+    return vtp_norm_bwd(dy, x, w, stats, dres, dx, dx_bf16, dw, db, dx_colsum, M, D, kind, stream);
+  VTP_REQUIRE(dy && x && w && stats && dx && dres, "vtp_norm_bwd_rows: null pointer (a row map needs dres)");
+  VTP_REQUIRE(!dx_colsum || dx_bf16, "vtp_norm_bwd_rows: dx_colsum sums the bf16 output and needs dx_bf16");
+  VTP_REQUIRE(M > 0 && dres_M > 0 && D > 0 && D % 4 == 0 && D <= 1024,
+              "vtp_norm_bwd_rows: need 0 < D <= 1024, D %% 4 == 0, dres_M > 0 (D=%d dres_M=%d)", D, dres_M);
+  VTP_REQUIRE(kind == 0 || kind == 1, "vtp_norm_bwd_rows: kind must be 0 or 1");
+  dim3 grid(norm_bwd_blocks(M, D)), block(256);
+  const bf16* dyb = (const bf16*)dy;
+  bf16* dxb = (bf16*)dx_bf16;
+  const int nc = cdiv(D, 256);
+#define NORM_ROWS(KIND, NC)                                                                                                         \
+  hipLaunchKernelGGL((norm_bwd_kernel<KIND, NC, false, true>), grid, block, 0, (hipStream_t)stream, dyb, x, w, stats, dres, dx, dxb, dw, \
+                     db, dx_colsum, M, D, (const float*)nullptr, 0, 0, 1, dres_rows, dres_M)
+#define NORM_ROWS_KIND(KIND)           \
+  do {                                 \
+    if (nc <= 1) NORM_ROWS(KIND, 1);   \
+    else if (nc == 2) NORM_ROWS(KIND, 2); \
+    else if (nc == 3) NORM_ROWS(KIND, 3); \
+    else NORM_ROWS(KIND, 4);           \
+  } while (0)
+  if (kind == 0) NORM_ROWS_KIND(0);
+  else NORM_ROWS_KIND(1);
+#undef NORM_ROWS_KIND
+#undef NORM_ROWS
+  return check_launch("norm_bwd_rows");
+}
+
 extern "C" int vtp_pool_patch_rows(const void* x, float* out, int B, int N, int D, float scale, void* stream) {
   VTP_REQUIRE(x && out, "vtp_pool_patch_rows: null pointer");
   VTP_REQUIRE(B > 0 && N >= 2 && D > 0 && D % 4 == 0, "vtp_pool_patch_rows: need B > 0, N >= 2, D %% 4 == 0 (B=%d N=%d D=%d)", B, N, D);
diff --git a/vtp_amd/engine.py b/vtp_amd/engine.py
--- a/vtp_amd/engine.py
+++ b/vtp_amd/engine.py
@@ -328,6 +328,16 @@
                     a_remap=dy_remap, c_remap=dx_remap)
 
 
+class WgradGroups:
+
+    def __init__(self, parts):
+        self.parts = parts
+
+    def launch(self):
+        for g in self.parts:
+            g.launch()
+
+
 class BlockW:
     pass
 
@@ -344,6 +354,8 @@
     st2: torch.Tensor
     pre: torch.Tensor
     hid: torch.Tensor
+    o_c: Optional[torch.Tensor] = None
+    row_map: Optional[torch.Tensor] = None
 
 
 ATTN_SCALE = 1.0 / math.sqrt(64.0)
@@ -563,7 +575,7 @@
             ops.attn_fwd(q_s, q_s[:, D:], q_s[:, 2 * D:], o_s, lse[r0 * heads:], Bs, Ns, heads, Ns * 3 * D, 3 * D, Ns * D, D,
                          ATTN_SCALE, self.causal)
 
-    def _attn_fwd(self, ws: Workspace, t: str, i: int, x, out, resid, M: int, rows, prefix_tokens: int, rope_plan):
+    def _attn_fwd(self, ws: Workspace, t: str, i: int, x, out, resid, M: int, rows, prefix_tokens: int, rope_plan, proj: bool = True):
         D, heads, b = self.D, self.heads, self.blocks[i]
         xn1, st1 = ws.get(t + "xn1", (M, D), BF), ws.get(t + "st1", (M, 2), F32)
         qkv, o = ws.get(t + "qkv", (M, 3 * D), BF), ws.get(t + "o", (M, D), BF)
@@ -580,7 +592,8 @@
         else:
             ops.gemm_nt(xn1, b.qkv.w, qkv, M=M, N=3 * D, K=D, bias=b.qkv.bias, epi=EPI_BF16)
         self._attention(qkv, o, lse, rows, i, prefix_tokens, rope_plan is None)
-        ops.gemm_nt(o, b.proj.w, out, M=M, N=D, K=D, bias=b.proj.bias, gamma=b.ls1, resid=resid, epi=EPI_F32)
+        if proj:
+            ops.gemm_nt(o, b.proj.w, out, M=M, N=D, K=D, bias=b.proj.bias, gamma=b.ls1, resid=resid, epi=EPI_F32)
         return xn1, st1, qkv, o, lse
 
     def _ffn_fwd(self, ws: Workspace, t: str, i: int, x, out, resid, M: int, train: bool):
@@ -619,8 +632,17 @@
         D, heads, b = self.D, self.heads, self.blocks[i]
         d_o, dxn = ws.get(bt + "do", (M, D), BF), ws.get(bt + "dxn", (M, D), BF)
         delta = ws.get(bt + "delta", (M * heads,), F32)
-        linear_bwd(ws, "proj", b.proj, dy_b, s.o, M, d_o, bias_grad_done=bias_done, ls=(b.ls1, b.gls1) if b.ls1 is not None else None,
-                   defer=probs)
+        if s.row_map is not None:
+            Mc = s.o_c.shape[0]
+            d_o_c = ws.get(bt + "do", (Mc, D), BF)
+            linear_bwd(ws, "proj", b.proj, dy_b, s.o_c, Mc, d_o_c, bias_grad_done=bias_done, defer=probs)
+            if probs is not None:
+                for pr in probs:
+                    pr["Ktok"] = Mc
+            ops.expand_rows_bf16(d_o_c, s.row_map, d_o, M, Mc, D)
+        else:
+            linear_bwd(ws, "proj", b.proj, dy_b, s.o, M, d_o, bias_grad_done=bias_done,
+                       ls=(b.ls1, b.gls1) if b.ls1 is not None else None, defer=probs)
         for r0, Bs, Ns, rp in rows:
             r1 = r0 + Bs * Ns
             q_s, dq_s = s.qkv[r0:r1], dqkv[r0:r1]
@@ -633,11 +655,21 @@
         linear_bwd(ws, "qkv", b.qkv, dqkv, s.xn1, M, dxn, defer=probs)
         if join:
             OVERLAP.join()
-        ops.norm_bwd(dxn, s.attn_in, b.n1w, s.st1, dy, dx, dx_b, b.gn1w, b.gn1b, M, D, self.kind, dx_colsum=dx_colsum)
-
-    def forward(self, ws: Workspace, x, segs, prefix_tokens: int, train: bool):
+        if s.row_map is not None:
+            ops.norm_bwd_rows(dxn, s.attn_in, b.n1w, s.st1, dy, s.row_map, dx, dx_b, b.gn1w, b.gn1b, M, D, self.kind, dx_colsum=dx_colsum)
+        else:
+            ops.norm_bwd(dxn, s.attn_in, b.n1w, s.st1, dy, dx, dx_b, b.gn1w, b.gn1b, M, D, self.kind, dx_colsum=dx_colsum)
+
+    def tail_rows_ok(self, train: bool) -> bool:
+        return (_env_flag("VTP_TAIL_ROWS") and self.style == "vit" and not (train and self.drop_plan is not None)
+                and getattr(self, "fp8", None) is None and self.D % 8 == 0 and self.D <= 1024
+                and self.blocks[-1].ls1 is None and self.blocks[-1].ls2 is None)
+
+    def forward(self, ws: Workspace, x, segs, prefix_tokens: int, train: bool, tail=None):
         D = self.D
         M = sum(b * n for b, n, _ in segs)
+        if tail is not None and not self.tail_rows_ok(train):
+            raise RuntimeError("Stack.forward: a tail row plan was passed to a pass that cannot take one (tail_rows_ok)")
         fp8 = getattr(self, "fp8", None)
         if fp8 is not None and fp8["ready"] and not train:
             return self._forward_fp8(ws, x, segs, prefix_tokens, M)
@@ -663,16 +695,28 @@
                 self._scatter(delta, x, segs, csegs, i, 1, scales, accumulate=True)
             else:
                 t = f"{i}." if train else ""
-                x1, x2 = x, ws.get(t + "xmid", (M, D), F32)
-                xout = ws.get((f"{i}.xout" if train else f"xout{i & 1}"), (M, D), F32)
-                a = self._attn_fwd(ws, t, i, x1, x2, x1, M, rows, prefix_tokens, rope_plan)
-                f = self._ffn_fwd(ws, t, i, x2, xout, x2, M, train)
+                tl = tail if i == self.depth - 1 else None
+                Mo = M if tl is None else tl[2] + tl[1]
+                x1, x2 = x, ws.get(t + "xmid", (Mo, D), F32)
+                xout = ws.get((f"{i}.xout" if train else f"xout{i & 1}"), (Mo, D), F32)
+                a = self._attn_fwd(ws, t, i, x1, x2, x1, M, rows, prefix_tokens, rope_plan, proj=tl is None)
+                if tl is not None:
+                    idx, T, L = tl
+                    o_c, x_c = ws.get(t + "o_c", (Mo, D), BF), ws.get(t + "x_c", (Mo, D), F32)
+                    ops.gather_tail_rows(a[3], x1, idx, o_c, x_c, T, L, M, D)
+                    b = self.blocks[i]
+                    ops.gemm_nt(o_c, b.proj.w, x2, M=Mo, N=D, K=D, bias=b.proj.bias, resid=x_c, epi=EPI_F32)
+                    if train:
+                        row_map = ws.get(t + "row_map", (M,), torch.int32)
+                        ops.tail_row_map(idx, row_map, T, L, M)
+                        extra_saved = (o_c, row_map)
+                f = self._ffn_fwd(ws, t, i, x2, xout, x2, Mo, train)
                 if calib is not None:
                     for j, tns in enumerate((a[0], a[3], f[0], f[3])):
                         ops.amax(tns, calib[i, j:j + 1])
                 x = xout
             if train:
-                saved_all.append(BlockSaved(x1, *a, x2, *f))
+                saved_all.append(BlockSaved(x1, *a, x2, *f, *(extra_saved if (not drop and tl is not None) else ())))
         self.last_saved = saved_all
         return x
 
@@ -740,6 +784,7 @@
         D, H = self.D, self.H
         M = sum(b * n for b, n, _ in segs)
         saved = self.last_saved if saved is None else saved
+        tail_Mc = saved[-1].o_c.shape[0] if saved and saved[-1].row_map is not None else None
         drop = self.drop_plan is not None
         if drop:
             csegs, Mb = self._drop_segs(segs)
@@ -787,11 +832,15 @@
                 continue
             dxo = ws.get(f"b.dx{i & 1}", (M, D), F32)
             dxo_b = ws.get(f"b.dx_b{i & 1}", (M, D), BF)
-            dmid_b = ws.get("b.dmid_b" + par(i), (M, D), BF)
+            Mf = tail_Mc if (tail_Mc is not None and i == self.depth - 1) else M
+            if Mf != M:
+                dpre = ws.get(bt + "dx12" + par(i), (Mf, 2 * H if self.swiglu else H), BF)
+            dmid = ws.get("b.dmid", (Mf, D), F32)
+            dmid_b = ws.get("b.dmid_b" + par(i), (Mf, D), BF)
             probs = [] if grouped else None
             if grouped:
                 launch_pending()
-            self._ffn_bwd(ws, i, s, dy, dy_b, dmid, dmid_b, M, bt, dpre, fused=self.swiglu and b.ls2 is None,
+            self._ffn_bwd(ws, i, s, dy, dy_b, dmid, dmid_b, Mf, bt, dpre, fused=self.swiglu and b.ls2 is None,
                           bias_done=dy_colsum_done if i == self.depth - 1 else self.w3_colsum_target(i) is not None, probs=probs,
                           dx_colsum=b.proj.gb if b.ls1 is None else None)
             self._attn_bwd(ws, t, i, s, dmid, dmid_b, dxo, dxo_b, M, bt, dqkv, rows, prefix_tokens, bias_done=b.proj.gb is not None,
@@ -802,13 +851,21 @@
                 yield ("block", i)
                 continue
             extra = [dict(pr, dy=dy_b) for pr in extra_last] if (i == 0 and hold_last and extra_last) else []
-            gkey = (i, bool(self.wgrad_overwrite), len(extra))
+            gkey = (i, bool(self.wgrad_overwrite), len(extra), Mf)
             grp = groups.get(gkey)
             if grp is None:
-                grp = ops.WgradGroup(M)
-                for pr in probs + extra:
-                    grp.add(pr["dy"], pr["x"], pr["gw"], pr["gb"], pr["N"], pr["K"], pr["swiglu_h"], accumulate=not self.wgrad_overwrite)
-                groups[gkey] = grp.finalize(self.store.device, scratch)
+                counts = sorted({pr.get("Ktok", M) for pr in probs + extra}, reverse=True)
+                if len(counts) > 1 and ops.wgrad_group_mixed_ok(counts):
+                    counts = [None]
+                parts = []
+                for kt in counts:
+                    g = ops.WgradGroup(M if kt is None else kt)
+                    for pr in probs + extra:
+                        if kt is None or pr.get("Ktok", M) == kt:
+                            g.add(pr["dy"], pr["x"], pr["gw"], pr["gb"], pr["N"], pr["K"], pr["swiglu_h"],
+                                  accumulate=not self.wgrad_overwrite, Ktok=pr.get("Ktok"))
+                    parts.append(g.finalize(self.store.device, scratch))
+                grp = groups[gkey] = parts[0] if len(parts) == 1 else WgradGroups(parts)
             if pending is not None:
                 yield ("block", pending[0])
             pending = (i, grp)
@@ -994,7 +1051,10 @@
     def forward(self, img: torch.Tensor, train: bool, masks: Optional[torch.Tensor] = None, tag: str = "", rope_aug: Optional[bool] = None):
         return self.forward_list([(img, masks)], train, tag, rope_aug=rope_aug)
 
-    def forward_list(self, items, train: bool, tag: str = "", rope_aug: Optional[bool] = None):
+    def tail_rows_ok(self, train: bool) -> bool:
+        return self.stack.tail_rows_ok(train)
+
+    def forward_list(self, items, train: bool, tag: str = "", rope_aug: Optional[bool] = None, tail=None):
         st = self.store
         D = self.D
         segs, r0, p0 = [], 0, 0
@@ -1023,12 +1083,14 @@
             ops.gemm_nt(pt, self.pe.w, xs, M=g.B * g.hw, N=D, K=768, bias=self.pe.bias, epi=EPI_F32, a_remap=(g.hw, 1), c_remap=(g.hw, 1))
             ops.assemble_tokens(xs, st.p(self.prefix + "cls_token"), st.p(self.prefix + "mask_token"), g.masks, g.B, g.N, D)
         stack_segs = [(g.B, g.N, g.rope) for g in segs]
-        xl = self.stack.forward(ws, x0, stack_segs, 1, train)
-        xnf = ws.get("xnf", (M, D), BF)
-        stf = ws.get("stf", (M, 2), F32)
+        xl = self.stack.forward(ws, x0, stack_segs, 1, train, tail=tail)
+        Mc = M if tail is None else tail[2] + tail[1]
+        xnf = ws.get("xnf", (Mc, D), BF)
+        stf = ws.get("stf", (Mc, 2), F32)
         ops.norm_fwd(xl, st.p(self.prefix + "norm.weight"), st.p(self.prefix + "norm.bias") if self.kind == ops.NORM_LN else None, xnf, stf,
-                     M, D, self.eps, self.kind)
+                     Mc, D, self.eps, self.kind)
         c = TrunkCtx()
+        c.Mc = Mc
         c.ws, c.segs, c.M, c.xl, c.xnf, c.stf, c.patches, c.stack_saved, c.x0, c.stack_segs = \
             ws, segs, M, xl, xnf, stf, patches, self.stack.last_saved, x0, stack_segs
         self._ctx = c
@@ -1057,14 +1119,14 @@
 
     def d_xnf_buffer(self, ctx=None) -> torch.Tensor:
         c = self._ctx if ctx is None else ctx
-        return c.ws.get("b.d_xnf", (c.M, self.D), BF, zero=True)
+        return c.ws.get("b.d_xnf", (c.Mc, self.D), BF, zero=True)
 
     def backward(self, d_lat: Optional[torch.Tensor], ctx=None, lat_seg: int = 0, want_dimg: bool = False, pool=None):
         st = self.store
         if ctx is not None:
             self._ctx = ctx
         c = self._ctx
-        ws, M, D = c.ws, c.M, self.D
+        ws, M, D = c.ws, c.Mc, self.D
         d_xnf = ws.get("b.d_xnf", (M, D), BF, zero=True)
         wgrads, self.bott_wgrads = self.bott_wgrads, []
         for dz, x, R in wgrads:
diff --git a/vtp_amd/ops.py b/vtp_amd/ops.py
--- a/vtp_amd/ops.py
+++ b/vtp_amd/ops.py
@@ -59,6 +59,11 @@
                                          _p(pvec), row0, B, N, M, D, kind, _s()), "vtp_norm_bwd_pvec")
 
 
+def norm_bwd_rows(dy, x, w, stats, dres, dres_rows, dx, dxb, dw, db, M, D, kind, dx_colsum=None):
+    _lib.check(_lib_().vtp_norm_bwd_rows(_p(dy), _p(x), _p(w), _p(stats), _p(dres), _p(dres_rows), dres.shape[0], _p(dx), _p(dxb), _p(dw),
+                                         _p(db), _p(dx_colsum), M, D, kind, _s()), "vtp_norm_bwd_rows")
+
+
 def pool_patch_rows(x, out, B, N, D, scale=None):
     assert x.dtype == torch.bfloat16 and x.is_contiguous() and x.numel() >= B * N * D and out.dtype == torch.float32
     assert out.is_contiguous() and out.numel() >= B * D
@@ -219,20 +224,48 @@
         for lt in range(((N + 255) // 256) * tn):
             tiles.append((tile0 + lt, pi, gb != 0 and lt % tn == 0))
     ncs = sum(1 for t in tiles if t[2])
-    more = ncs > 0 and len(tiles) * base_splits + ncs <= cus and Ktok // (base_splits + 1) >= 1024
+    Ks = [int(r[13]) or int(Ktok) for r in rows]
+    if len(set(Ks)) > 1:
+        per = wgrad_mixed_splits([sum(1 for t in tiles if t[1] == pi) for pi in range(len(rows))], Ks, cus)
+    else:
+        per = [base_splits] * len(rows)
+    n_items = sum(per[t[1]] for t in tiles)
     items, slots = [], 1
     for pi in range(len(rows)):
+        more = ncs > 0 and n_items + ncs <= cus and Ks[pi] // (per[pi] + 1) >= 1024
         for heavy in (True, False):
             grp = [t for t in tiles if t[1] == pi and t[2] == heavy]
             if not grp:
                 continue
-            cs = wgrad_k_cuts(Ktok, base_splits + 1 if (heavy and more) else base_splits)
+            cs = wgrad_k_cuts(Ks[pi], per[pi] + 1 if (heavy and more) else per[pi])
             slots = max(slots, len(cs))
             for z, (kb, kc) in enumerate(cs):
                 items += [[t[0], kb, kc, len(cs), z, 0, 0, 0] for t in grp]
     return items, slots
 
 
+def wgrad_mixed_splits(ntiles, Ks, cus: int):
+    n = len(Ks)
+    per = [1] * n
+    length = lambda p: ((Ks[p] + per[p] - 1) // per[p] + 63) // 64 * 64
+    while True:
+        top = max(length(p) for p in range(n))
+        grp = [p for p in range(n) if length(p) == top]
+        total = sum(per[p] * ntiles[p] for p in range(n))
+        if total + sum(ntiles[p] for p in grp) > cus or any(Ks[p] // (per[p] + 1) < 1024 for p in grp):
+            return per
+        for p in grp:
+            per[p] += 1
+
+
+def wgrad_group_mixed_ok(Ks) -> bool:
+    import os
+    e = os.environ.get("VTP_GEMM4W_TN")
+    if e == "0" or any(k % 8 for k in Ks):
+        return False
+    return e == "1" or min(Ks) >= W4_TN_MIN_SLICE
+
+
 def wgrad_group_uniform_items(ntiles: int, Ktok: int, splits: int):
     cs = wgrad_k_cuts(Ktok, max(int(splits), 1))
     return [[t, kb, kc, len(cs), z, 0, 0, 0] for z, (kb, kc) in enumerate(cs) for t in range(ntiles)], len(cs)
@@ -248,24 +281,34 @@
         self.table = self.part = self.ticket = None
         self._uniform = {}
 
-    def add(self, dy, x, gw, gb, N: int, K: int, swiglu_h: int = 0, accumulate: bool = True):
+    def add(self, dy, x, gw, gb, N: int, K: int, swiglu_h: int = 0, accumulate: bool = True, Ktok: int = None):
         if N % 8 or K % 8 or dy.stride(0) % 8 or x.stride(0) % 8 or N < 8 or K < 8:
             raise ValueError(f"WgradGroup.add: N = {N}, K = {K} and the leading dimensions ({dy.stride(0)}, {x.stride(0)}) must be multiples "
                              "of 8 (use the per-layer weight-gradient path: linear_bwd without `defer`)")
         self.rows.append([dy.data_ptr(), x.data_ptr(), gw.data_ptr(), 0 if gb is None else gb.data_ptr(), dy.stride(0), x.stride(0), K,
-                          N, K, -1 if swiglu_h else 0, swiglu_h, self.ntiles, int(accumulate), 0, 0, 0])
+                          N, K, -1 if swiglu_h else 0, swiglu_h, self.ntiles, int(accumulate), 0 if Ktok is None or int(Ktok) == self.Ktok else int(Ktok),
+                          0, 0])
         self.ntiles += ((N + 255) // 256) * ((K + 255) // 256)
         self.keep += [dy, x, gw, gb]
 
     def finalize(self, device, scratch=None):
         import torch
         assert 1 <= len(self.rows) <= 8
-        if not wgrad_group_fits(self.Ktok, max(max(r[4], r[5]) for r in self.rows)):
+        Ks = [r[13] or self.Ktok for r in self.rows]
+        self.mixed = len(set(Ks)) > 1
+        if not self.mixed and Ks[0] != self.Ktok:
+            self.Ktok = Ks[0]
+            for r in self.rows:
+                r[13] = 0
+        if self.mixed and any(k % 8 or k < 8 for k in Ks):
+            raise ValueError(f"WgradGroup: problems over different token counts {Ks} need multiples of 8 (the item-list kernel); "
+                             "launch one group per token count")
+        if not all(wgrad_group_fits(k, max(r[4], r[5])) for k, r in zip(Ks, self.rows)):
             raise ValueError("WgradGroup: token rows x leading dimension exceed the 32-bit staging offsets of vtp_gemm_tn_grouped; "
                              "use the per-layer weight-gradient path (linear_bwd without `defer`)")
         _, self.splits = wgrad_group_splits(self.ntiles, self.Ktok)
         self.table = torch.tensor(self.rows, dtype=torch.int64, device=device)
-        self.kernel = wgrad_group_kernel(self.ntiles, self.splits, self.Ktok)
+        self.kernel = 1 if self.mixed else wgrad_group_kernel(self.ntiles, self.splits, self.Ktok)
         self.items, self.nitems, self.slots = None, None, self.splits
         if self.kernel == 1:
             items, self.slots = wgrad_group_items(self.rows, self.Ktok, self.splits)
@@ -284,6 +327,8 @@
     def launch(self, kernel=None):
         if kernel is None:
             kernel = self.kernel
+        if kernel == 0 and self.mixed:
+            raise ValueError("WgradGroup.launch: the 8-phase kernel takes one token count for every problem")
         if kernel == 0:
             _lib.check(_lib_().vtp_gemm_tn_grouped(_p(self.table), len(self.rows), self.ntiles, self.Ktok, self.splits, _p(self.part),
                                                    _p(self.ticket), _s()), "vtp_gemm_tn_grouped")
@@ -318,6 +363,18 @@
                "vtp_scatter_image_rows")
 
 
+def gather_tail_rows(o, x, idx, o_c, x_c, T, L, M, D):
+    _lib.check(_lib_().vtp_gather_tail_rows(_p(o), _p(x), _p(idx), _p(o_c), _p(x_c), T, L, M, D, _s()), "vtp_gather_tail_rows")
+
+
+def tail_row_map(idx, row_map, T, L, M):
+    _lib.check(_lib_().vtp_tail_row_map(_p(idx), _p(row_map), T, L, M, _s()), "vtp_tail_row_map")
+
+
+def expand_rows_bf16(src, row_map, dst, M, Mc, D):
+    _lib.check(_lib_().vtp_expand_rows_bf16(_p(src), _p(row_map), _p(dst), M, Mc, D, _s()), "vtp_expand_rows_bf16")
+
+
 def layerscale_wgrad(G, W, bias, colsum, gamma, dW, db, dgamma, N, K):
     _lib.check(_lib_().vtp_layerscale_wgrad(_p(G), _p(W), _p(bias), _p(colsum), _p(gamma), _p(dW), _p(db), _p(dgamma), N, K, _s()),
                "vtp_layerscale_wgrad")
diff --git a/vtp_amd/ssl_engine.py b/vtp_amd/ssl_engine.py
--- a/vtp_amd/ssl_engine.py
+++ b/vtp_amd/ssl_engine.py
@@ -128,5 +128,22 @@
     t0[m0:m0 + n_masked] = 2 * B + np.arange(n_masked)
     w[m0:m0 + n_masked] = ibot_weight * mw / B
     student_global_src = np.concatenate([np.arange(2 * B, dtype=np.int32) * N, masked_rows, pad])
-    return dict(n_masked=n_masked, Tm=Tm, Ts=Ts, teacher_src=teacher_src, student_local_src=local_src,
-                student_global_src=student_global_src, t0=t0, t1=t1, w=w)
+    out = dict(n_masked=n_masked, Tm=Tm, Ts=Ts, teacher_src=teacher_src, student_local_src=local_src,
+               student_global_src=student_global_src, t0=t0, t1=t1, w=w)
+    out.update(tail_row_plan(out, 2 * B * N))
+    return out
+
+
+def tail_row_plan(plan, global_rows: int):
+    tail = np.concatenate([np.asarray(plan["student_local_src"], np.int32) + np.int32(global_rows),
+                           plan["student_global_src"]]).astype(np.int32)
+    keep = lambda src: np.where(src >= 0, np.arange(src.shape[0]), -1).astype(np.int32)
+    return dict(student_tail_src=tail, student_tail_keep=keep(tail), teacher_keep=keep(plan["teacher_src"]))
+
+
+def tail_row_map(tail_src, L: int, M: int):
+    m = np.full(M, -1, np.int32)
+    m[:L] = np.arange(L, dtype=np.int32)
+    t = np.flatnonzero(np.asarray(tail_src) >= 0)
+    m[L + np.asarray(tail_src)[t]] = L + t
+    return m
diff --git a/vtp_amd/train.py b/vtp_amd/train.py
--- a/vtp_amd/train.py
+++ b/vtp_amd/train.py
@@ -529,7 +529,8 @@
 
     def _ssl_gen(self, P, lead_images=None):
         from .vtp import ssl_forward
-        out = ssl_forward(self.model, P["global"], P["local"], P["masks"], P["plan"], P["dev"], train=True, lead_images=lead_images)
+        out = ssl_forward(self.model, P["global"], P["local"], P["masks"], P["plan"], P["dev"], train=True, lead_images=lead_images,
+                          tail_rows="student_tail_src" in P["dev"])
         self._zero_join()
         if not (self.head_overlap and not self.collectives and OVERLAP.enabled):
             yield from self._ssl_tail(out, P)
@@ -591,6 +592,9 @@
         d_xnf = self.trunk.d_xnf_buffer(ctx)
         if zero_dxnf:
             d_xnf.zero_()
+        if out["tail"] is not None:
+            ops.gather_token_rows(dX, P["dev"]["student_tail_keep"], d_xnf[out["tail"]:], Ts, D)
+            return
         seg_g, seg_l = ctx.segs[-2], ctx.segs[-1]
         ops.scatter_token_rows(dX, P["dev"]["student_local_src"], d_xnf[seg_l.row0:], nl, D)
         ops.scatter_token_rows(dX[nl:], P["dev"]["student_global_src"], d_xnf[seg_g.row0:], Ts - nl, D)
@@ -652,7 +656,9 @@
                                  pad_to=int(pad_to or self.ssl_bucket), upperbound=upperbound)
         if self._stager is None:
             self._stager = HostStager(self.store.device)
-        arrays = {k: plan[k].astype(np.int32, copy=False) for k in ("teacher_src", "student_local_src", "student_global_src", "t0", "t1")}
+        from .vtp import TAIL_KEYS
+        arrays = {k: plan[k].astype(np.int32, copy=False)
+                  for k in ("teacher_src", "student_local_src", "student_global_src", "t0", "t1") + TAIL_KEYS}
         arrays["w"] = plan["w"].astype(np.float32, copy=False)
         arrays["n_masked_i"] = np.array([plan["n_masked"]], np.int32)
         arrays["n_masked_f"] = np.array([float(plan["n_masked"])], np.float32)
diff --git a/vtp_amd/vtp.py b/vtp_amd/vtp.py
--- a/vtp_amd/vtp.py
+++ b/vtp_amd/vtp.py
@@ -210,8 +210,11 @@
     return lo, hi
 
 
+TAIL_KEYS = ("student_tail_src", "student_tail_keep", "teacher_keep")
+
+
 def plan_to_device(plan, device):
-    d = {k: torch.as_tensor(plan[k], device=device) for k in ("teacher_src", "student_local_src", "student_global_src", "t0", "t1")}
+    d = {k: torch.as_tensor(plan[k], device=device) for k in ("teacher_src", "student_local_src", "student_global_src", "t0", "t1") + TAIL_KEYS}
     d["w"] = torch.as_tensor(plan["w"], device=device)
     d["n_masked_i"] = torch.tensor([plan["n_masked"]], dtype=torch.int32, device=device)
     d["n_masked_f"] = torch.tensor([float(plan["n_masked"])], dtype=torch.float32, device=device)
@@ -219,7 +222,7 @@
 
 
 def ssl_forward(model: "VTP", global_crops, local_crops, masks_u8, plan, dev_plan=None, train: bool = False,
-                lead_images=None):
+                lead_images=None, tail_rows: bool = False):
     st = model._store
     B2 = global_crops.shape[0]
     hw = (global_crops.shape[-2] // 16) * (global_crops.shape[-1] // 16)
@@ -236,9 +239,17 @@
     Dh = model.dino_cfg["in_dim"]
     bott = Dh != D
 
+    t_tail = tail_rows and model._t_trunk.tail_rows_ok(False)
+    s_tail = tail_rows and model._trunk.tail_rows_ok(train)
+
     def teacher():
-        xnf_t = model._t_trunk.forward(global_crops, train=False, tag="teacher", rope_aug=train)
-        ops.gather_token_rows(xnf_t, idx["teacher_src"], Xt, Tt, D)
+        if t_tail:
+            xnf_t = model._t_trunk.forward_list([(global_crops, None)], train=False, tag="teacher", rope_aug=train,
+                                                tail=(idx["teacher_src"], Tt, 0))
+            ops.gather_token_rows(xnf_t, idx["teacher_keep"], Xt, Tt, D)
+        else:
+            xnf_t = model._t_trunk.forward(global_crops, train=False, tag="teacher", rope_aug=train)
+            ops.gather_token_rows(xnf_t, idx["teacher_src"], Xt, Tt, D)
         Ht = model._t_trunk.bott_rows(Xt, Tt, ws.get("Zt", (Tt, Dh), BF)) if bott else Xt
         return model._t_head.forward(Ht, Tt, tag="teacher")[0]
 
@@ -251,18 +262,24 @@
         t_logits = teacher()
     leads = [] if lead_images is None else (list(lead_images) if isinstance(lead_images, (list, tuple)) else [lead_images])
     items = [(im, None) for im in leads] + [(global_crops, masks_u8), (local_crops, None)]
-    xnf = model._trunk.forward_list(items, train=train, tag="ssl")
+    lead_rows = sum(im.shape[0] * ((im.shape[-2] // 16) * (im.shape[-1] // 16) + 1) for im in leads)
+    xnf = model._trunk.forward_list(items, train=train, tag="ssl", tail=(idx["student_tail_src"], Ts, lead_rows) if s_tail else None)
     ctx = model._trunk.ctx()
     seg_g, seg_l = ctx.segs[-2], ctx.segs[-1]
+    assert seg_g.row0 == lead_rows
     nl = int(plan["student_local_src"].shape[0])
     Xs = ws.get("Xs", (Ts, D), BF)
-    ops.gather_token_rows(xnf[seg_l.row0:], idx["student_local_src"], Xs, nl, D)
-    ops.gather_token_rows(xnf[seg_g.row0:], idx["student_global_src"], Xs[nl:], Ts - nl, D)
+    if s_tail:
+        ops.gather_token_rows(xnf[lead_rows:], idx["student_tail_keep"], Xs, Ts, D)
+    else:
+        ops.gather_token_rows(xnf[seg_l.row0:], idx["student_local_src"], Xs, nl, D)
+        ops.gather_token_rows(xnf[seg_g.row0:], idx["student_global_src"], Xs[nl:], Ts - nl, D)
     Hs = model._trunk.bott_rows(Xs, Ts, ws.get("Zs", (Ts, Dh), BF)) if bott else Xs
     s_logits, head_ctx = model._head.forward(Hs, Ts, tag="student")
     OVERLAP.join()
     return dict(teacher_logits=t_logits, student_logits=s_logits, head_ctx=head_ctx, ctx=ctx, xnf=xnf, idx=idx,
-                Xs=Xs, Hs=Hs, bott=bott, student_global_cls=Hs[nl:nl + B2], Tt=Tt, Ts=Ts, Tm=Tm, nl=nl, B2=B2, N=N, ws=ws)
+                Xs=Xs, Hs=Hs, bott=bott, student_global_cls=Hs[nl:nl + B2], Tt=Tt, Ts=Ts, Tm=Tm, nl=nl, B2=B2, N=N, ws=ws,
+                tail=lead_rows if s_tail else None)
 
 
 def ssl_head_input_bwd(model: "VTP", out, dH):
```

New measurement: 752.4, median of 6. +1.9%, better.
